# WPCLab/OpenSeg3D

Hardware: AMD Instinct MI355X
Metric: points/sec fwd+bwd, Waymo 1-sweep ~180k pts @0.1m voxel; logit parity (higher is better)
Workload: dtype f32 storage/accumulate, bf16x3 products; 1 GPU; waymo_one_sweep (BASELINE configs[1]): synthetic scene, 174633 pts/step/GPU, voxel [0.1, 0.1, 0.1], grid [1440, 1440, 64], fwd (attention dropout p=0.1, DropPath) + criterion (ohem_ce+lovasz on 3 heads) + bwd + SGD step; mode=fwdbwd, segmentor=segformer, voxels=108690, parallelism=dp1

## Files before the change

### include/seg3d_hip.h

```cpp
#ifndef SEG3D_HIP_H
#define SEG3D_HIP_H

#include <stddef.h>
#include <stdint.h>

#ifdef __cplusplus
extern "C" {
#endif

#define SEG3D_OK 0
#define SEG3D_EINVAL (-1)
#define SEG3D_EWORKSPACE (-2)
#define SEG3D_ELAUNCH (-3)

#define SEG3D_REDUCE_SUM 0
#define SEG3D_REDUCE_MEAN 1
#define SEG3D_REDUCE_MAX 2

int seg3d_abi_version(void);

const char* seg3d_last_error(void);

int seg3d_grid_size(const float* voxel_size, const float* range, int32_t* grid_xyz);

// ... 107 lines not shown
int seg3d_linear_fwd_f32(const float* x, int64_t m, const void* w_packed, const float* bias ,
                         int32_t cin, int32_t cout, float* y, void* stream);
size_t seg3d_linear_packed_bytes_x6(int32_t cin, int32_t cout);
int seg3d_linear_pack_weight_x6(const float* weight, int32_t cin, int32_t cout, int32_t transpose, void* w_packed,
                                void* stream);
int seg3d_linear_fwd_x6(const float* x, int64_t m, const void* w_packed, const float* bias ,
                        const float* scale , const float* shift , int32_t relu, int32_t cin,
                        int32_t cout, float* y, void* stream);

typedef struct {
  const float* src;
  void* dst;
  int32_t cin, cout;
  int32_t kk, transpose, flip, reserved;
  int64_t first_block;
} seg3d_pack_job;
int seg3d_pack_weights_batched(const void* jobs, int32_t n_jobs, int64_t total_blocks, void* stream);

size_t seg3d_linear_packed_bytes(int32_t cin, int32_t cout, int32_t transpose);
int seg3d_linear_pack_weight(const float* weight, int32_t cin, int32_t cout, int32_t transpose,
                             void* w_packed, void* stream);
int seg3d_linear_fwd(const float* x, int64_t m, const void* w_packed, const float* bias ,
                     const float* addend , int32_t cin, int32_t cout,
                     float* y, void* stream);
int seg3d_linear_fwd_sum(const float* x, const float* x_add, int64_t m, const void* w_packed, const float* bias,
                         int32_t cin, int32_t cout, float* y, void* stream);
int seg3d_linear_layernorm_fwd(const float* x, int64_t m, const void* w_packed, const float* bias, const float* res,
                               const float* gamma, const float* beta, float eps, int32_t cin, int32_t cout, float* y,
                               void* stream);
int seg3d_linear_fwd_mul(const float* x, int64_t m, const void* w_packed, const float* factor, int32_t cin, int32_t cout,
                         float* y, void* stream);

size_t seg3d_window_partition_workspace_bytes(int64_t m, int32_t batch_size, const int32_t* nwin_xyz);
int seg3d_window_partition(const int32_t* coords, int64_t m, int32_t batch_size,
                           const int32_t* win_xyz, const int32_t* nwin_xyz, const int32_t* shift_xyz,
                           int32_t n_levels, const int32_t* level_lo, const int32_t* level_hi,
                           const int32_t* level_cap, int32_t* win_id, int32_t* in_win, int32_t* rank,
                           int32_t* level, int32_t* slot, int32_t* tok, int32_t* win_start,
                           int32_t* win_count, int32_t* win_tile0, int32_t* tile_item,
                           int32_t* qg_item, int32_t* counts, void* workspace,
                           size_t workspace_bytes, void* stream);

int seg3d_pos_embed(const int32_t* in_win, int64_t m, const int32_t* win_xyz ,
                    const float* inv_freq, int32_t c, float* pos, void* stream);

int seg3d_window_attn_supported(int32_t heads, int32_t dh);
size_t seg3d_window_attn_workspace_bytes(int64_t m, int32_t n_tiles, int32_t heads, int32_t dh);
int seg3d_window_attn_schedule(int32_t n_tiles, int32_t n_chunks, int32_t heads, int32_t dh, float dropout_p, int32_t* out);
int seg3d_window_attn_fwd(const float* q, const float* k, const float* v, int32_t ldq, int32_t ldk,
                          int32_t ldv, const int32_t* tok, const int32_t* win_start,
                          const int32_t* win_count, const int32_t* win_tile0,
                          const int32_t* tile_item, int32_t n_tiles, const int32_t* qg_item,
                          int32_t n_qgroups, int64_t m, int32_t n_windows, int32_t heads, int32_t dh,
                          const float* tau, float tau_min, float dropout_p, uint64_t dropout_seed, float* out,
                          float* lse, void* workspace, size_t workspace_bytes, void* stream);
int seg3d_window_attn_bwd(const float* q, const float* k, const float* v, int32_t ldq, int32_t ldk,
                          int32_t ldv, const float* out, const float* dout, const float* lse,
                          const int32_t* tok, const int32_t* win_start, const int32_t* win_count,
                          const int32_t* win_tile0, const int32_t* tile_item, int32_t n_tiles,
                          const int32_t* qg_item, int32_t n_qgroups, int64_t m, int32_t n_windows,
                          int32_t heads, int32_t dh, const float* tau,
                          float tau_min, float dropout_p, uint64_t dropout_seed, float* dq, float* dk,
                          float* dv, int32_t lddq, int32_t lddk,
                          int32_t lddv, float* dtau, void* workspace, size_t workspace_bytes,
                          void* stream);

int seg3d_layernorm_fwd(const float* x, const float* res, const float* gamma, const float* beta,
                        const float* rowscale, float eps, int64_t m, int32_t c, float* y, float* mean,
                        float* rstd, void* stream);
size_t seg3d_layernorm_bwd_workspace_bytes(int64_t m, int32_t c);
int seg3d_layernorm_bwd(const float* dy, const float* x, const float* mean, const float* rstd,
                        const float* gamma, const float* rowscale, int64_t m, int32_t c, float* dx,
                        float* dgamma, float* dbeta, void* workspace, size_t workspace_bytes, void* stream);
int seg3d_layernorm_bwd_partials(const float* dy, const float* x, const float* mean, const float* rstd,
                                 const float* gamma, const float* rowscale, int64_t m, int32_t c, float* dx,
                                 void* workspace, size_t workspace_bytes, int32_t* nblocks, void* stream);
size_t seg3d_batchnorm_workspace_bytes(int64_t m, int32_t c);
int seg3d_colstats(const float* x, int64_t m, int32_t c, float* sums, void* workspace, size_t workspace_bytes,
                   void* stream);
int seg3d_batchnorm_stats(const float* x, int64_t m, int32_t c, float eps, const float* gamma, const float* beta,
                          float momentum, float* running_mean, float* running_var, float* stats, void* workspace,
                          size_t workspace_bytes, void* stream);
int seg3d_gelu_fwd(const float* h, int64_t n, float* g, float* gp, void* stream);
int seg3d_affine_act(const float* x, const float* res, const float* scale, const float* shift, int32_t relu,
                     int64_t m, int32_t c, float* y, void* stream);
int seg3d_batchnorm_bwd(const float* dy, const float* y, const float* x, const float* mean, const float* rstd,
                        const float* gamma, int32_t relu, int64_t m, int32_t c, float* dx, float* dres,
                        float* sums, void* workspace, size_t workspace_bytes, void* stream);
int seg3d_batchnorm_bwd_reduce(const float* dy, const float* y, const float* x, const float* mean,
                               const float* rstd, int32_t relu, int64_t m, int32_t c, float* sums,
                               void* workspace, size_t workspace_bytes, void* stream);
int seg3d_batchnorm_bwd_apply(const float* dy, const float* y, const float* x, const float* mean,
                              const float* rstd, const float* gamma, const float* sums, const float* inv_count,
                              int32_t relu, int64_t m, int32_t c, float* dx, float* dres, void* stream);

int seg3d_segment_reduce_fwd(const float* x, int32_t c, const int32_t* order, const int32_t* offsets,
                             int64_t n_seg, int32_t mode, float* out, int32_t* argmax, void* stream);
int seg3d_segment_reduce_bwd(const float* dout, int32_t c, const int32_t* seg_of_row, int64_t n,
                             const int32_t* offsets, const int32_t* argmax, int64_t n_seg,
                             int32_t mode, float* dx, void* stream);

int seg3d_knn_attention_fwd(const float* q, const float* k, const float* v, const int32_t* idx,
                            const uint8_t* invalid, const float* keep, int64_t n, int64_t n_src,
                            int32_t n_neighbors, int32_t d, float scale, float* out, float* prob, void* stream);
int seg3d_knn_attention_bwd(const float* q, const float* k, const float* v, const int32_t* idx, const float* keep,
                            const float* prob, const float* dout, const int32_t* pair_order,
                            const int32_t* pair_offsets, int64_t n, int64_t n_src, int32_t n_neighbors, int32_t d,
                            float scale, float* dq, float* dk, float* dv, float* scratch, void* stream);

int seg3d_class_context_fwd(const float* feats, const float* probs, const int32_t* offsets, const int32_t* chunks,
                            const int32_t* chunk_offsets, int32_t n_chunks, int32_t batch, int64_t m,
                            int32_t classes, int32_t c, float scale, float* weights, float* partials, float* stats,
                            float* context, void* stream);
int seg3d_class_context_bwd(const float* feats, const float* weights, const float* dcontext,
                            const int32_t* offsets, const int32_t* chunks, const int32_t* chunk_offsets,
                            int32_t n_chunks, int32_t batch, int64_t m, int32_t classes, int32_t c, float scale,
                            float* dfeats, float* dprobs, float* scratch, void* stream);

int seg3d_gather_rows(const float* feats, const int32_t* ids, int64_t n, int32_t c, float* out,
                      void* stream);

int seg3d_knn_query(const float* xyz, int64_t n, const float* new_xyz, int64_t m, const int32_t* offset,
                    const int32_t* new_offset, int32_t batch_size, int32_t k, int32_t* idx, float* dist2,
                    void* stream);

size_t seg3d_knn_level_workspace_bytes(int64_t n);
int seg3d_knn_level_build(const float* xyz, int64_t n, const int32_t* offset, int32_t batch_size, float cell,
                          float* sorted_xyz, int32_t* src_index, int32_t* cell_end, void* table_keys, int32_t* table_vals,
                          int64_t capacity, void* workspace, size_t workspace_bytes, void* stream);
int seg3d_knn_query_order(const float* new_xyz, int64_t m, const int32_t* new_offset, int32_t batch_size, float cell,
                          int32_t* order, void* workspace, size_t workspace_bytes, void* stream);
int seg3d_parity_order(const int32_t* coords, int64_t m, int32_t* order, void* workspace, size_t workspace_bytes,
                       void* stream);
typedef struct {
  const float* sorted_xyz;
  const int32_t* src_index;
  const int32_t* cell_end;
  const void* table_keys;
  const int32_t* table_vals;
  int64_t capacity;
  float cell;
  int32_t max_ring;
} seg3d_knn_level;
int seg3d_knn_grid_query(const seg3d_knn_level* levels, int32_t n_levels, const float* new_xyz,
                         const int32_t* query_order , int64_t m,
                         const int32_t* offset, const int32_t* new_offset, int32_t batch_size, int32_t k,
                         int32_t* idx, float* dist2, void* stream);

size_t seg3d_furthest_sampling_workspace_bytes(int64_t n);
int seg3d_furthest_sampling(const float* xyz, int64_t n, const int32_t* order, const int32_t* offset,
                            const int32_t* new_offset, int32_t n_segments, int32_t* idx, void* workspace,
                            size_t workspace_bytes, void* stream);
int seg3d_furthest_sampling_host(const float* xyz, int64_t n, const int32_t* order, const int32_t* offset,
                                 const int32_t* new_offset, int32_t n_segments, int32_t* idx);
int seg3d_sector_angles(const float* xyz, int64_t n, const int32_t* offset, int32_t batch_size, float* angle,
                        float* minmax, void* stream);
int seg3d_sector_angles_host(const float* xyz, int64_t n, const int32_t* offset, int32_t batch_size, float* angle,
                             float* minmax);
int seg3d_sector_assign(const float* angle, int64_t n, const int32_t* offset, int32_t batch_size, const float* edges,
                        const int32_t* sector_offset, int32_t* sector_id, void* stream);
int seg3d_sector_assign_host(const float* angle, int64_t n, const int32_t* offset, int32_t batch_size,
                             const float* edges, const int32_t* sector_offset, int32_t* sector_id);

#define SEG3D_POINTOPS_CHUNK 512
size_t seg3d_pointops_scratch_bytes(int64_t m, int32_t k, int32_t width);
int seg3d_group_points_fwd(const float* xyz, const float* new_xyz, const float* feat, const int32_t* idx, int64_t n,
// ... 218 lines not shown
```

### openseg3d_amd/_lib.py

```python
import ctypes
import os
import re

_HERE = os.path.dirname(os.path.abspath(__file__))
LIB_PATH = os.path.join(_HERE, "csrc", "libseg3d_hip.so")
HEADER_PATH = os.path.join(os.path.dirname(_HERE), "include", "seg3d_hip.h")

OK, EINVAL, EWORKSPACE, ELAUNCH = 0, -1, -2, -3
REDUCE_SUM, REDUCE_MEAN, REDUCE_MAX = 0, 1, 2
ABI_VERSION = 49

_p, _i32, _i64, _sz, _f = ctypes.c_void_p, ctypes.c_int32, ctypes.c_int64, ctypes.c_size_t, ctypes.c_float
_u64 = ctypes.c_uint64
_d = ctypes.c_double

SIGNATURES = {
    "seg3d_abi_version": (ctypes.c_int, []),
    "seg3d_last_error": (ctypes.c_char_p, []),
    "seg3d_grid_size": (ctypes.c_int, [_p, _p, _p]),
    "seg3d_voxelize_workspace_bytes": (_sz, [_i64]),
    "seg3d_voxelize_f32": (ctypes.c_int, [_p, _i64, _i32, _i32, _i32, _p, _p, _p, _p, _p, _p, _sz, _p]),
    "seg3d_voxelize_f64": (ctypes.c_int, [_p, _i64, _i32, _i32, _i32, _p, _p, _p, _p, _p, _p, _sz, _p]),
    "seg3d_voxelize_host_workspace_bytes": (_sz, [_i64]),
    "seg3d_voxelize_host_f32": (ctypes.c_int, [_p, _i64, _i32, _i32, _i32, _p, _p, _p, _p, _p, _p, _sz]),
    "seg3d_voxelize_host_f64": (ctypes.c_int, [_p, _i64, _i32, _i32, _i32, _p, _p, _p, _p, _p, _p, _sz]),
    "seg3d_cart2polar_f32": (ctypes.c_int, [_p, _i64, _i32, _i32, _p, _p]),
    "seg3d_cart2polar_f64": (ctypes.c_int, [_p, _i64, _i32, _i32, _p, _p]),
    "seg3d_group_index_workspace_bytes": (_sz, [_i64, _i64]),
    "seg3d_group_index": (ctypes.c_int, [_p, _i64, _i64, _p, _p, _p, _p, _sz, _p]),
    "seg3d_coord_hash_bytes": (_sz, [_i64]),
    "seg3d_coord_hash_build": (ctypes.c_int, [_p, _i64, _p, _p, _sz, _p]),
    "seg3d_rulebook_subm": (ctypes.c_int, [_p, _i64, _p, _p, _sz, _p, _p]),
    "seg3d_downsample_workspace_bytes": (_sz, [_i32, _p]),
    "seg3d_downsample_coords": (ctypes.c_int, [_p, _i64, _p, _i32, _p, _p, _i64, _p, _p, _sz, _p]),
    "seg3d_rulebook_strided": (ctypes.c_int, [_p, _i64, _i64, _p, _p, _sz, _p, _p, _p]),
    "seg3d_spconv_packed_bytes": (_sz, [_i32, _i32, _i32]),
    "seg3d_spconv_pack_weight": (ctypes.c_int, [_p, _i32, _i32, _i32, _p, _p]),
    "seg3d_spconv_fwd": (ctypes.c_int, [_p, _p, _i64, _i64, _p, _i32, _p, _i32, _i32, _p, _p, _p]),
    "seg3d_spconv_fwd_act": (ctypes.c_int, [_p, _p, _i64, _i64, _p, _i32, _p, _p, _i32, _i32, _i32, _p, _p, _p]),
    "seg3d_spconv_fwd_act_bf16": (ctypes.c_int, [_p, _i32, _p, _i64, _i64, _p, _i32, _p, _p, _i32, _i32, _i32, _p, _p, _p]),
    "seg3d_spconv_presplit_bytes": (_sz, [_i64, _i32]),
    "seg3d_spconv_presplit": (ctypes.c_int, [_p, _i64, _i32, _p, _p]),
    "seg3d_spconv_fwd_presplit": (ctypes.c_int, [_p, _p, _i64, _i64, _p, _i32, _p, _p, _i32, _i32, _i32, _p, _p, _p]),
    "seg3d_conv_plan_bytes": (_sz, [_i64]),
    "seg3d_conv_plan_workspace_bytes": (_sz, [_i64]),
    "seg3d_conv_plan_build": (ctypes.c_int, [_p, _p, _i64, _p, _p, _sz, _p]),
    "seg3d_spconv_tiled_supported": (_i32, [_i32, _i32]),
    "seg3d_spconv_fwd_tiled": (ctypes.c_int, [_p, _p, _p, _i64, _i64, _p, _i32, _p, _p, _i32, _i32, _i32, _p, _p]),
    "seg3d_spconv_fwd_tiled_bf16": (ctypes.c_int, [_p, _i32, _p, _p, _i64, _i64, _p, _i32, _p, _p, _i32, _i32, _i32, _p, _p]),
    "seg3d_debug_set_conv_nbt": (ctypes.c_int, [_i32]),
    "seg3d_debug_set_linear_stream": (ctypes.c_int, [_i32]),
    "seg3d_spconv_wgrad_workspace_bytes": (_sz, [_i64, _i32, _i32]),
    "seg3d_spconv_wgrad": (ctypes.c_int, [_p, _p, _p, _i64, _i64, _i32, _i32, _i32, _p, _p, _sz, _p]),
    "seg3d_spconv_wgrad_partials": (ctypes.c_int, [_p, _p, _p, _i64, _i64, _i32, _i32, _p, _sz, _p, _p]),
    "seg3d_spconv_wgrad_partials_xbf16": (ctypes.c_int, [_p, _p, _p, _i64, _i64, _i32, _i32, _p, _sz, _p, _p]),
    "seg3d_linear_wgrad_partials_xbf16": (ctypes.c_int, [_p, _p, _i64, _i32, _i32, _i32, _p, ctypes.c_size_t, _p, _p]),
    "seg3d_linear_packed_bytes_f32": (ctypes.c_size_t, [_i32, _i32]),
    "seg3d_linear_pack_weight_f32": (ctypes.c_int, [_p, _i32, _i32, _i32, _p, _p]),
    "seg3d_linear_fwd_f32": (ctypes.c_int, [_p, _i64, _p, _p, _i32, _i32, _p, _p]),
    "seg3d_debug_set_wgrad_lds": (ctypes.c_int, [_i32]),
    "seg3d_linear_packed_bytes_x6": (ctypes.c_size_t, [_i32, _i32]),
    "seg3d_linear_pack_weight_x6": (ctypes.c_int, [_p, _i32, _i32, _i32, _p, _p]),
    "seg3d_linear_fwd_x6": (ctypes.c_int, [_p, _i64, _p, _p, _p, _p, _i32, _i32, _i32, _p, _p]),
    "seg3d_pack_weights_batched": (ctypes.c_int, [_p, _i32, _i64, _p]),
    "seg3d_linear_wgrad_workspace_bytes": (ctypes.c_size_t, [_i64, _i32, _i32]),
    "seg3d_linear_wgrad": (ctypes.c_int, [_p, _p, _i64, _i32, _i32, _p, _p, _p, ctypes.c_size_t, _p]),
    "seg3d_linear_wgrad_partials": (ctypes.c_int, [_p, _p, _i64, _i32, _i32, _i32, _p, ctypes.c_size_t, _p, _p]),
    "seg3d_reduce_partials": (ctypes.c_int, [_p, _i32, _i64, _i64, _p, _p, _p]),
    "seg3d_reduce_partials_batched": (ctypes.c_int, [_p, _i32, _i64, _p]),
    "seg3d_linear_packed_bytes": (_sz, [_i32, _i32, _i32]),
    "seg3d_linear_pack_weight": (ctypes.c_int, [_p, _i32, _i32, _i32, _p, _p]),
    "seg3d_linear_fwd": (ctypes.c_int, [_p, _i64, _p, _p, _p, _i32, _i32, _p, _p]),
    "seg3d_linear_fwd_sum": (ctypes.c_int, [_p, _p, _i64, _p, _p, _i32, _i32, _p, _p]),
    "seg3d_linear_fwd_mul": (ctypes.c_int, [_p, _i64, _p, _p, _i32, _i32, _p, _p]),
    "seg3d_linear_layernorm_fwd": (ctypes.c_int, [_p, _i64, _p, _p, _p, _p, _p, ctypes.c_float, _i32, _i32, _p, _p]),
    "seg3d_window_partition_workspace_bytes": (_sz, [_i64, _i32, _p]),
    "seg3d_window_partition": (ctypes.c_int, [_p, _i64, _i32, _p, _p, _p, _i32, _p, _p, _p,
                                              _p, _p, _p, _p, _p, _p, _p, _p, _p, _p, _p, _p, _p, _sz, _p]),
    "seg3d_pos_embed": (ctypes.c_int, [_p, _i64, _p, _p, _i32, _p, _p]),
    "seg3d_window_attn_supported": (ctypes.c_int, [_i32, _i32]),
    "seg3d_window_attn_workspace_bytes": (_sz, [_i64, _i32, _i32, _i32]),
    "seg3d_window_attn_schedule": (ctypes.c_int, [_i32, _i32, _i32, _i32, _f, _p]),
    "seg3d_window_attn_fwd": (ctypes.c_int, [_p, _p, _p, _i32, _i32, _i32, _p, _p, _p, _p, _p, _i32, _p, _i32,
                                             _i64, _i32, _i32, _i32, _p, _f, _f, _u64, _p, _p, _p, _sz, _p]),
    "seg3d_window_attn_bwd": (ctypes.c_int, [_p, _p, _p, _i32, _i32, _i32, _p, _p, _p, _p, _p, _p, _p, _p, _i32, _p,
                                             _i32, _i64, _i32, _i32, _i32, _p, _f, _f, _u64, _p, _p, _p, _i32, _i32, _i32,
                                             _p, _p, _sz, _p]),
    "seg3d_layernorm_fwd": (ctypes.c_int, [_p, _p, _p, _p, _p, _f, _i64, _i32, _p, _p, _p, _p]),
    "seg3d_layernorm_bwd_workspace_bytes": (ctypes.c_size_t, [_i64, _i32]),
    "seg3d_layernorm_bwd": (ctypes.c_int, [_p, _p, _p, _p, _p, _p, _i64, _i32, _p, _p, _p, _p, ctypes.c_size_t, _p]),
    "seg3d_layernorm_bwd_partials": (ctypes.c_int, [_p, _p, _p, _p, _p, _p, _i64, _i32, _p, _p, ctypes.c_size_t, _p, _p]),
    "seg3d_batchnorm_workspace_bytes": (ctypes.c_size_t, [_i64, _i32]),
    "seg3d_colstats": (ctypes.c_int, [_p, _i64, _i32, _p, _p, ctypes.c_size_t, _p]),
    "seg3d_batchnorm_stats": (ctypes.c_int, [_p, _i64, _i32, _f, _p, _p, _f, _p, _p, _p, _p, ctypes.c_size_t, _p]),
    "seg3d_affine_act": (ctypes.c_int, [_p, _p, _p, _p, _i32, _i64, _i32, _p, _p]),
    "seg3d_gelu_fwd": (ctypes.c_int, [_p, _i64, _p, _p, _p]),
    "seg3d_batchnorm_bwd": (ctypes.c_int, [_p, _p, _p, _p, _p, _p, _i32, _i64, _i32, _p, _p, _p, _p, ctypes.c_size_t, _p]),
    "seg3d_batchnorm_bwd_reduce": (ctypes.c_int, [_p, _p, _p, _p, _p, _i32, _i64, _i32, _p, _p, ctypes.c_size_t, _p]),
    "seg3d_batchnorm_bwd_apply": (ctypes.c_int, [_p, _p, _p, _p, _p, _p, _p, _p, _i32, _i64, _i32, _p, _p, _p]),
    "seg3d_segment_reduce_fwd": (ctypes.c_int, [_p, _i32, _p, _p, _i64, _i32, _p, _p, _p]),
    "seg3d_segment_reduce_bwd": (ctypes.c_int, [_p, _i32, _p, _i64, _p, _p, _i64, _i32, _p, _p]),
    "seg3d_voxel_majority_labels": (ctypes.c_int, [_p, _p, _p, _i64, _i32, _p, _p]),
    "seg3d_cross_entropy_workspace_bytes": (ctypes.c_size_t, [_i64]),
    "seg3d_cross_entropy_fwd": (ctypes.c_int, [_p, _p, _i64, _i32, _i64, _f, _p, _p, _p, ctypes.c_size_t, _p]),
    "seg3d_cross_entropy_bwd": (ctypes.c_int, [_p, _p, _p, _p, _p, _i64, _i32, _p, _p]),
    "seg3d_lovasz_workspace_bytes": (ctypes.c_size_t, [_i64, _i32]),
    "seg3d_lovasz_softmax_fwd": (ctypes.c_int, [_p, _p, _i64, _i32, _i64, _i32, _p, _p, _p, _p, _p, ctypes.c_size_t, _p]),
    "seg3d_lovasz_softmax_bwd": (ctypes.c_int, [_p, _p, _p, _p, _i64, _i32, _p, _p]),
    "seg3d_pointwise_loss_workspace_bytes": (ctypes.c_size_t, [_i64]),
    "seg3d_focal_loss_fwd": (ctypes.c_int, [_p, _p, _i64, _i32, _i64, _f, _f, _p, _i32, _p, _p, ctypes.c_size_t, _p]),
    "seg3d_focal_loss_bwd": (ctypes.c_int, [_p, _p, _p, _p, _i64, _i32, _i64, _f, _f, _p, _i32, _p, _p]),
    "seg3d_dice_loss_fwd": (ctypes.c_int, [_p, _p, _i64, _i32, _i64, _f, _f, _p, _f, _f, _p, _p, ctypes.c_size_t, _p]),
    "seg3d_dice_loss_bwd": (ctypes.c_int, [_p, _p, _p, _i64, _i32, _i64, _f, _f, _p, _f, _f, _p, _p]),
    "seg3d_knn_level_workspace_bytes": (ctypes.c_size_t, [_i64]),
    "seg3d_knn_level_build": (ctypes.c_int, [_p, _i64, _p, _i32, _f, _p, _p, _p, _p, _p, _i64, _p, ctypes.c_size_t, _p]),
    "seg3d_parity_order": (ctypes.c_int, [_p, _i64, _p, _p, ctypes.c_size_t, _p]),
    "seg3d_knn_query_order": (ctypes.c_int, [_p, _i64, _p, _i32, _f, _p, _p, ctypes.c_size_t, _p]),
    "seg3d_knn_grid_query": (ctypes.c_int, [_p, _i32, _p, _p, _i64, _p, _p, _i32, _i32, _p, _p, _p]),
    "seg3d_knn_query": (ctypes.c_int, [_p, _i64, _p, _i64, _p, _p, _i32, _i32, _p, _p, _p]),
    "seg3d_furthest_sampling_workspace_bytes": (_sz, [_i64]),
    "seg3d_furthest_sampling": (ctypes.c_int, [_p, _i64, _p, _p, _p, _i32, _p, _p, _sz, _p]),
    "seg3d_furthest_sampling_host": (ctypes.c_int, [_p, _i64, _p, _p, _p, _i32, _p]),
    "seg3d_sector_angles": (ctypes.c_int, [_p, _i64, _p, _i32, _p, _p, _p]),
    "seg3d_sector_angles_host": (ctypes.c_int, [_p, _i64, _p, _i32, _p, _p]),
    "seg3d_sector_assign": (ctypes.c_int, [_p, _i64, _p, _i32, _p, _p, _p, _p]),
    "seg3d_sector_assign_host": (ctypes.c_int, [_p, _i64, _p, _i32, _p, _p, _p]),
    "seg3d_pointops_scratch_bytes": (_sz, [_i64, _i32, _i32]),
    "seg3d_group_points_fwd": (ctypes.c_int, [_p, _p, _p, _p, _i64, _i64, _i32, _i32, _p, _p]),
    "seg3d_group_points_fwd_host": (ctypes.c_int, [_p, _p, _p, _p, _i64, _i64, _i32, _i32, _p]),
    "seg3d_group_points_bwd": (ctypes.c_int, [_p, _p, _p, _p, _i64, _i64, _i32, _i32, _i32, _p, _p, _p, _p, _sz, _p]),
    "seg3d_group_points_bwd_host": (ctypes.c_int, [_p, _p, _p, _p, _i64, _i64, _i32, _i32, _i32, _p, _p, _p]),
    "seg3d_knn_interpolate_fwd": (ctypes.c_int, [_p, _p, _p, _i64, _i64, _i32, _i32, _p, _p, _p]),
    "seg3d_knn_interpolate_fwd_host": (ctypes.c_int, [_p, _p, _p, _i64, _i64, _i32, _i32, _p, _p]),
    "seg3d_knn_interpolate_bwd": (ctypes.c_int, [_p, _p, _p, _p, _p, _i64, _i64, _i32, _i32, _p, _p, _sz, _p]),
    "seg3d_knn_interpolate_bwd_host": (ctypes.c_int, [_p, _p, _p, _p, _p, _i64, _i64, _i32, _i32, _p]),
    "seg3d_gather_rows": (ctypes.c_int, [_p, _p, _i64, _i32, _p, _p]),
    "seg3d_class_context_fwd": (ctypes.c_int, [_p, _p, _p, _p, _p, _i32, _i32, _i64, _i32, _i32, _f, _p, _p, _p, _p, _p]),
    "seg3d_class_context_bwd": (ctypes.c_int, [_p, _p, _p, _p, _p, _p, _i32, _i32, _i64, _i32, _i32, _f, _p, _p, _p, _p]),
    "seg3d_knn_attention_fwd": (ctypes.c_int, [_p, _p, _p, _p, _p, _p, _i64, _i64, _i32, _i32, _f, _p, _p, _p]),
    "seg3d_knn_attention_bwd": (ctypes.c_int, [_p, _p, _p, _p, _p, _p, _p, _p, _p, _i64, _i64, _i32, _i32, _f, _p, _p, _p, _p, _p]),
    "seg3d_tta_views_f32": (ctypes.c_int, [_p, _i64, _i32, _p, _p, _p]),
    "seg3d_tta_views_host_f32": (ctypes.c_int, [_p, _i64, _i32, _p, _p]),
    "seg3d_softmax_accumulate_f32": (ctypes.c_int, [_p, _i64, _i32, _i32, _i32, _p, _p]),
    "seg3d_argmax_confusion": (ctypes.c_int, [_p, _p, _i64, _i32, _i32, _p, _i32, _p, _p, _p]),
    "seg3d_aug_polarmix_workspace_bytes": (_sz, [_i64, _i64]),
    "seg3d_aug_polarmix_map": (ctypes.c_int, [_p, _i64, _p, _i64, _i32, _i32, _p, _i32, _i32, _d, _d, _p, _i32, _i32, _i64,
                                              _p, _p, _p, _p, _sz, _p]),
    "seg3d_aug_polarmix_map_host": (ctypes.c_int, [_p, _i64, _p, _i64, _i32, _i32, _p, _i32, _i32, _d, _d, _p, _i32, _i32,
                                                   _i64, _p, _p, _p]),
    "seg3d_aug_far_near_workspace_bytes": (_sz, [_i64]),
    "seg3d_aug_far_near": (ctypes.c_int, [_p, _i64, _p, _i64, _i32, _i32, _p, _p, _i64, _p, _i64, _p, _f, _p, _p, _p, _p,
                                          _p, _sz, _p]),
    "seg3d_aug_far_near_host": (ctypes.c_int, [_p, _i64, _p, _i64, _i32, _i32, _p, _p, _i64, _p, _i64, _p, _f, _p, _p, _p,
                                               _p]),
    "seg3d_aug_sample_workspace_bytes": (_sz, [_i64]),
    "seg3d_aug_sample_device": (ctypes.c_int, [_p, _i64, _i64, _u64, _p, _p, _sz, _p]),
    "seg3d_aug_sample_host": (ctypes.c_int, [_p, _i64, _i64, _u64, _p]),
    "seg3d_aug_cur_map_workspace_bytes": (_sz, [_i64, _i64]),
    "seg3d_aug_cur_map": (ctypes.c_int, [_p, _i64, _p, _i64, _i64, _p, _p, _p, _p, _sz, _p]),
    "seg3d_aug_cur_map_host": (ctypes.c_int, [_p, _i64, _p, _i64, _i64, _p, _p, _p]),
    "seg3d_aug_apply_f32": (ctypes.c_int, [_p, _i64, _p, _i64, _i32, _p, _p, _i64, _p, _p, _p]),
    "seg3d_aug_apply_f64in": (ctypes.c_int, [_p, _i64, _p, _i64, _i32, _p, _p, _i64, _p, _p, _p]),
    "seg3d_aug_apply_host_f32": (ctypes.c_int, [_p, _i64, _p, _i64, _i32, _p, _p, _i64, _p, _p]),
    "seg3d_aug_apply_host_f64in": (ctypes.c_int, [_p, _i64, _p, _i64, _i32, _p, _p, _i64, _p, _p]),
    "seg3d_aug_gather": (ctypes.c_int, [_p, _i64, _p, _i64, _i64, _p, _i64, _p, _p]),
    "seg3d_aug_gather_host": (ctypes.c_int, [_p, _i64, _p, _i64, _i64, _p, _i64, _p]),
    "seg3d_aug_instance_workspace_bytes": (_sz, [_i64, _i64, _i32]),
    "seg3d_aug_instance_paste": (ctypes.c_int, [_p, _i64, _i32, _i32, _p, _i32, _p, _i32, _p, _i64, _p, _i32, _i64, _p, _p,
                                                _p, _p, _p, _sz, _p]),
    "seg3d_aug_instance_paste_host": (ctypes.c_int, [_p, _i64, _i32, _i32, _p, _i32, _p, _i32, _p, _i64, _p, _i32, _i64, _p,
                                                     _p, _p, _p]),
    "seg3d_instance_extract_workspace_bytes": (_sz, [_i64, _i32]),
    "seg3d_instance_extract": (ctypes.c_int, [_p, _i64, _i32, _i32, _p, _i32, _p, _p, _i32, _p, _i32, _d, _i32, _p, _p, _p, _p,
                                              _p, _sz, _p]),
    "seg3d_instance_extract_host": (ctypes.c_int, [_p, _i64, _i32, _i32, _p, _i32, _p, _p, _i32, _p, _i32, _d, _i32, _p, _p, _p,
                                                   _p]),
    "seg3d_frame_assemble": (ctypes.c_int, [_p, _i32, _i32, _p, _p, _p, _f, _p]),
    "seg3d_frame_assemble_host": (ctypes.c_int, [_p, _i32, _i32, _p, _p, _p, _f]),
    "seg3d_range_image_workspace_bytes": (_sz, [_i32, _i32]),
# ... 55 lines not shown
```

### openseg3d_amd/csrc/rownorm.hip

```cpp
#include "common.hpp"

namespace {

constexpr int kThreads = 256;
constexpr int kMaxBlocks = 2048;
constexpr int kLnBwdMaxBlocks = 1024;

struct RowMap {
    int quads;
    int p;
    int items;
};

inline RowMap row_map(int c) {
    RowMap m;
    m.quads = c / 4;
    m.items = (m.quads + 63) / 64;
    int need = (m.quads + m.items - 1) / m.items;
    m.p = 8;
    while (m.p < need) m.p <<= 1;
    return m;
}

__device__ __forceinline__ float group_sum(float v, int p) {
    for (int off = 1; off < p; off <<= 1) v += __shfl_xor(v, off, SEG3D_WAVE);
    return v;
}

template <int ITEMS>
__global__ __launch_bounds__(kThreads) void ln_fwd_kernel(const float* __restrict__ x, const float* __restrict__ res,
                                                          const float* __restrict__ gamma, const float* __restrict__ beta,
                                                          const float* __restrict__ rowscale, float eps, int64_t m, int c,
                                                          RowMap rm, float* __restrict__ y, float* __restrict__ mean,
                                                          float* __restrict__ rstd) {
    const int lane = threadIdx.x & 63, wave = threadIdx.x >> 6;
    const int rows_per_wave = 64 / rm.p;
    const int lr = lane / rm.p, lq = lane % rm.p;
    const float inv_c = 1.0f / (float)c;
    for (int64_t base = ((int64_t)blockIdx.x * 4 + wave) * rows_per_wave; base < m;
         base += (int64_t)gridDim.x * 4 * rows_per_wave) {
        const int64_t row = base + lr;
        const bool rok = row < m;
        float4 v[ITEMS];
        float s = 0.f;
#pragma unroll
        for (int i = 0; i < ITEMS; ++i) {
            const int q = lq + i * rm.p;
            v[i] = make_float4(0.f, 0.f, 0.f, 0.f);
            if (rok && q < rm.quads) v[i] = *reinterpret_cast<const float4*>(x + row * c + 4 * q);
            s += (v[i].x + v[i].y) + (v[i].z + v[i].w);
        }
        const float mu = group_sum(s, rm.p) * inv_c;
        float ss = 0.f;
#pragma unroll
        for (int i = 0; i < ITEMS; ++i) {
            const int q = lq + i * rm.p;
            if (q < rm.quads) {
                const float a = v[i].x - mu, b = v[i].y - mu, cc = v[i].z - mu, d = v[i].w - mu;
                ss += (a * a + b * b) + (cc * cc + d * d);
            }
        }
        const float rs = rsqrtf(group_sum(ss, rm.p) * inv_c + eps);
        const float sc = rowscale && rok ? rowscale[row] : 1.0f;
#pragma unroll
        for (int i = 0; i < ITEMS; ++i) {
            const int q = lq + i * rm.p;
            if (rok && q < rm.quads) {
                const float4 g = *reinterpret_cast<const float4*>(gamma + 4 * q);
                const float4 b = *reinterpret_cast<const float4*>(beta + 4 * q);
                float4 o;
                o.x = ((v[i].x - mu) * rs * g.x + b.x) * sc;
                o.y = ((v[i].y - mu) * rs * g.y + b.y) * sc;
                o.z = ((v[i].z - mu) * rs * g.z + b.z) * sc;
                o.w = ((v[i].w - mu) * rs * g.w + b.w) * sc;
                if (res) {
                    const float4 r4 = *reinterpret_cast<const float4*>(res + row * c + 4 * q);
                    o.x += r4.x; o.y += r4.y; o.z += r4.z; o.w += r4.w;
                }
                *reinterpret_cast<float4*>(y + row * c + 4 * q) = o;
            }
        }
        if (rok && lq == 0 && mean) {
            mean[row] = mu;
            rstd[row] = rs;
        }
    }
}

template <int ITEMS>
__global__ __launch_bounds__(kThreads) void ln_bwd_kernel(const float* __restrict__ dy, const float* __restrict__ x,
                                                          const float* __restrict__ mean, const float* __restrict__ rstd,
                                                          const float* __restrict__ gamma, const float* __restrict__ rowscale,
                                                          int64_t m, int c, RowMap rm, float* __restrict__ dx,
                                                          float* __restrict__ part ) {
    extern __shared__ float red[];
    const int lane = threadIdx.x & 63, wave = threadIdx.x >> 6;
    const int rows_per_wave = 64 / rm.p;
    const int lr = lane / rm.p, lq = lane % rm.p;
    const float inv_c = 1.0f / (float)c;
    float4 ag[ITEMS], ab[ITEMS];
#pragma unroll
    for (int i = 0; i < ITEMS; ++i) ag[i] = ab[i] = make_float4(0.f, 0.f, 0.f, 0.f);

    for (int64_t base = ((int64_t)blockIdx.x * 4 + wave) * rows_per_wave; base < m;
         base += (int64_t)gridDim.x * 4 * rows_per_wave) {
        const int64_t row = base + lr;
        const bool rok = row < m;
        const float mu = rok ? mean[row] : 0.f, rs = rok ? rstd[row] : 0.f;
        const float sc = rowscale && rok ? rowscale[row] : 1.0f;
        float4 xh[ITEMS], gy[ITEMS];
        float s1 = 0.f, s2 = 0.f;
#pragma unroll
        for (int i = 0; i < ITEMS; ++i) {
            const int q = lq + i * rm.p;
            xh[i] = gy[i] = make_float4(0.f, 0.f, 0.f, 0.f);
            if (rok && q < rm.quads) {
                const float4 xv = *reinterpret_cast<const float4*>(x + row * c + 4 * q);
                float4 dv = *reinterpret_cast<const float4*>(dy + row * c + 4 * q);
                dv.x *= sc; dv.y *= sc; dv.z *= sc; dv.w *= sc;
                const float4 g = *reinterpret_cast<const float4*>(gamma + 4 * q);
                xh[i] = make_float4((xv.x - mu) * rs, (xv.y - mu) * rs, (xv.z - mu) * rs, (xv.w - mu) * rs);
                gy[i] = make_float4(dv.x * g.x, dv.y * g.y, dv.z * g.z, dv.w * g.w);
                ag[i].x += dv.x * xh[i].x; ag[i].y += dv.y * xh[i].y; ag[i].z += dv.z * xh[i].z; ag[i].w += dv.w * xh[i].w;
                ab[i].x += dv.x; ab[i].y += dv.y; ab[i].z += dv.z; ab[i].w += dv.w;
                s1 += (gy[i].x + gy[i].y) + (gy[i].z + gy[i].w);
                s2 += (gy[i].x * xh[i].x + gy[i].y * xh[i].y) + (gy[i].z * xh[i].z + gy[i].w * xh[i].w);
            }
        }
        const float c1 = group_sum(s1, rm.p) * inv_c, c2 = group_sum(s2, rm.p) * inv_c;
#pragma unroll
        for (int i = 0; i < ITEMS; ++i) {
            const int q = lq + i * rm.p;
            if (rok && q < rm.quads) {
                float4 o;
                o.x = rs * (gy[i].x - c1 - xh[i].x * c2);
                o.y = rs * (gy[i].y - c1 - xh[i].y * c2);
                o.z = rs * (gy[i].z - c1 - xh[i].z * c2);
                o.w = rs * (gy[i].w - c1 - xh[i].w * c2);
                *reinterpret_cast<float4*>(dx + row * c + 4 * q) = o;
            }
        }
    }
    const int slots = 4 * rows_per_wave;
    float* mine = red + (size_t)(wave * rows_per_wave + lr) * 2 * c;
#pragma unroll
    for (int i = 0; i < ITEMS; ++i) {
        const int q = lq + i * rm.p;
        if (q < rm.quads) {
            *reinterpret_cast<float4*>(mine + 4 * q) = ag[i];
            *reinterpret_cast<float4*>(mine + c + 4 * q) = ab[i];
        }
    }
    __syncthreads();
    for (int i = threadIdx.x; i < 2 * c; i += kThreads) {
        float t = red[i];
        for (int l = 1; l < slots; ++l) t += red[(size_t)l * 2 * c + i];
        part[(int64_t)blockIdx.x * 2 * c + i] = t;
    }
}

__global__ __launch_bounds__(1024) void ln_bwd_reduce(const float* __restrict__ part, int nblocks, int c,
                                                      float* __restrict__ dgamma, float* __restrict__ dbeta) {
    __shared__ float red[32][33];
    const int col = threadIdx.x & 31, q = threadIdx.x >> 5;
    const int i = blockIdx.x * 32 + col;
    float s = 0.f;
    if (i < 2 * c) {
        float s0 = 0.f, s1 = 0.f, s2 = 0.f, s3 = 0.f;
        int b = q;
        for (; b + 96 < nblocks; b += 128) {
            s0 += part[(int64_t)b * 2 * c + i];
            s1 += part[(int64_t)(b + 32) * 2 * c + i];
            s2 += part[(int64_t)(b + 64) * 2 * c + i];
            s3 += part[(int64_t)(b + 96) * 2 * c + i];
        }
        for (; b < nblocks; b += 32) s0 += part[(int64_t)b * 2 * c + i];
        s = (s0 + s1) + (s2 + s3);
    }
    red[q][col] = s;
    __syncthreads();
    if (q == 0 && i < 2 * c) {
        float t = red[0][col];
#pragma unroll
        for (int k = 1; k < 32; ++k) t += red[k][col];
        if (i < c) dgamma[i] = t;
        else dbeta[i - c] = t;
    }
}

template <int MODE>
__global__ __launch_bounds__(kThreads) void col_reduce_kernel(const float* __restrict__ x, const float* __restrict__ dy,
                                                              const float* __restrict__ y, const float* __restrict__ mean,
                                                              const float* __restrict__ rstd, int relu, int64_t m, int c,
                                                              float* __restrict__ part ) {
    extern __shared__ float red[];
    const int quads = c / 4;
    const int lanes = kThreads / quads;
    const int q = threadIdx.x % quads, rl = threadIdx.x / quads;
    if (rl < lanes) {
        float4 a = make_float4(0.f, 0.f, 0.f, 0.f), b = a;
        float4 p0 = a, p1 = a;
        if (MODE == 0) p0 = *reinterpret_cast<const float4*>(x + 4 * q);
        if (MODE == 1) {
            p0 = *reinterpret_cast<const float4*>(mean + 4 * q);
            p1 = *reinterpret_cast<const float4*>(rstd + 4 * q);
        }
        for (int64_t row = (int64_t)blockIdx.x * lanes + rl; row < m; row += (int64_t)gridDim.x * lanes) {
            const float4 xv = *reinterpret_cast<const float4*>(x + row * c + 4 * q);
            if (MODE == 0) {
                const float dx_ = xv.x - p0.x, dy_ = xv.y - p0.y, dz_ = xv.z - p0.z, dw_ = xv.w - p0.w;
                a.x += dx_; a.y += dy_; a.z += dz_; a.w += dw_;
                b.x += dx_ * dx_; b.y += dy_ * dy_; b.z += dz_ * dz_; b.w += dw_ * dw_;
            } else {
                float4 g = *reinterpret_cast<const float4*>(dy + row * c + 4 * q);
                if (relu) {
                    const float4 yv = *reinterpret_cast<const float4*>(y + row * c + 4 * q);
                    g.x = yv.x > 0.f ? g.x : 0.f; g.y = yv.y > 0.f ? g.y : 0.f;
                    g.z = yv.z > 0.f ? g.z : 0.f; g.w = yv.w > 0.f ? g.w : 0.f;
                }
                a.x += g.x; a.y += g.y; a.z += g.z; a.w += g.w;
                b.x += g.x * (xv.x - p0.x) * p1.x; b.y += g.y * (xv.y - p0.y) * p1.y;
                b.z += g.z * (xv.z - p0.z) * p1.z; b.w += g.w * (xv.w - p0.w) * p1.w;
            }
        }
        *reinterpret_cast<float4*>(red + (size_t)rl * 2 * c + 4 * q) = a;
        *reinterpret_cast<float4*>(red + (size_t)rl * 2 * c + c + 4 * q) = b;
    }
    __syncthreads();
    for (int i = threadIdx.x; i < 2 * c; i += kThreads) {
        float t = red[i];
        for (int l = 1; l < lanes; ++l) t += red[(size_t)l * 2 * c + i];
        part[(size_t)blockIdx.x * 2 * c + i] = t;
    }
}

__device__ __forceinline__ float col_partial_sum(const float* __restrict__ part, int nblocks, int c2, int i, float (*red)[33]) {
    const int col = threadIdx.x & 31, q = threadIdx.x >> 5;
    float s = 0.f;
    if (i < c2) {
        float s0 = 0.f, s1 = 0.f, s2 = 0.f, s3 = 0.f;
        int b = q;
        for (; b + 96 < nblocks; b += 128) {
            s0 += part[(int64_t)b * c2 + i];
            s1 += part[(int64_t)(b + 32) * c2 + i];
            s2 += part[(int64_t)(b + 64) * c2 + i];
            s3 += part[(int64_t)(b + 96) * c2 + i];
        }
        for (; b < nblocks; b += 32) s0 += part[(int64_t)b * c2 + i];
        s = (s0 + s1) + (s2 + s3);
    }
    red[q][col] = s;
    __syncthreads();
    float t = red[0][col];
#pragma unroll
    for (int k = 1; k < 32; ++k) t += red[k][col];
    __syncthreads();
    return t;
}

__global__ __launch_bounds__(1024) void col_sums_finish(const float* __restrict__ part, int nblocks, int c,
                                                        float* __restrict__ sums ) {
    __shared__ float red[32][33];
    const int i = blockIdx.x * 32 + (threadIdx.x & 31);
    const float t = col_partial_sum(part, nblocks, 2 * c, i, red);
    if ((threadIdx.x >> 5) == 0 && i < 2 * c) sums[i] = t;
}

__global__ __launch_bounds__(kThreads) void gelu_fwd_kernel(const float* __restrict__ h, int64_t quads, float* __restrict__ g,
                                                            float* __restrict__ gp) {
    for (int64_t t = (int64_t)blockIdx.x * kThreads + threadIdx.x; t < quads; t += (int64_t)gridDim.x * kThreads) {
        const float4 v = reinterpret_cast<const float4*>(h)[t];
        const float in[4] = {v.x, v.y, v.z, v.w};
        float o[4], d[4];
#pragma unroll
        for (int i = 0; i < 4; ++i) {
            const float cdf = 0.5f * (1.0f + erff(in[i] * 0.70710678118654752440f));
            o[i] = in[i] * cdf;
            d[i] = cdf + in[i] * (0.39894228040143267794f * __expf(-0.5f * in[i] * in[i]));
        }
        reinterpret_cast<float4*>(g)[t] = make_float4(o[0], o[1], o[2], o[3]);
        if (gp) reinterpret_cast<float4*>(gp)[t] = make_float4(d[0], d[1], d[2], d[3]);
    }
}

__global__ __launch_bounds__(kThreads) void affine_act_kernel(const float* __restrict__ x, const float* __restrict__ res,
                                                              const float* __restrict__ scale, const float* __restrict__ shift,
                                                              int relu, int64_t total_quads, int quads, float* __restrict__ y) {
    for (int64_t t = (int64_t)blockIdx.x * kThreads + threadIdx.x; t < total_quads; t += (int64_t)gridDim.x * kThreads) {
        const int q = (int)(t % quads);
        const float4 xv = reinterpret_cast<const float4*>(x)[t];
        const float4 s = *reinterpret_cast<const float4*>(scale + 4 * q);
        const float4 b = *reinterpret_cast<const float4*>(shift + 4 * q);
        float4 o = make_float4(xv.x * s.x + b.x, xv.y * s.y + b.y, xv.z * s.z + b.z, xv.w * s.w + b.w);
        if (res) {
            const float4 r = reinterpret_cast<const float4*>(res)[t];
            o.x += r.x; o.y += r.y; o.z += r.z; o.w += r.w;
        }
        if (relu) {
            o.x = fmaxf(o.x, 0.f); o.y = fmaxf(o.y, 0.f); o.z = fmaxf(o.z, 0.f); o.w = fmaxf(o.w, 0.f);
        }
        reinterpret_cast<float4*>(y)[t] = o;
    }
}

__global__ __launch_bounds__(kThreads) void bn_bwd_apply_kernel(const float* __restrict__ dy, const float* __restrict__ y,
                                                                const float* __restrict__ x, const float* __restrict__ mean,
                                                                const float* __restrict__ rstd, const float* __restrict__ gamma,
                                                                const float* __restrict__ sums , int relu,
                                                                float inv_m, const float* __restrict__ inv_m_dev,
                                                                int64_t total_quads, int quads,
                                                                float* __restrict__ dx, float* __restrict__ dres) {
    const int c = quads * 4;
    if (inv_m_dev) inv_m = inv_m_dev[0];
    for (int64_t t = (int64_t)blockIdx.x * kThreads + threadIdx.x; t < total_quads; t += (int64_t)gridDim.x * kThreads) {
        const int q = (int)(t % quads);
        float4 g = reinterpret_cast<const float4*>(dy)[t];
        if (relu) {
            const float4 yv = reinterpret_cast<const float4*>(y)[t];
            g.x = yv.x > 0.f ? g.x : 0.f; g.y = yv.y > 0.f ? g.y : 0.f;
            g.z = yv.z > 0.f ? g.z : 0.f; g.w = yv.w > 0.f ? g.w : 0.f;
        }
        if (dres) reinterpret_cast<float4*>(dres)[t] = g;
        const float4 xv = reinterpret_cast<const float4*>(x)[t];
        const float4 mu = *reinterpret_cast<const float4*>(mean + 4 * q);
        const float4 rs = *reinterpret_cast<const float4*>(rstd + 4 * q);
        const float4 ga = *reinterpret_cast<const float4*>(gamma + 4 * q);
        const float4 s1 = *reinterpret_cast<const float4*>(sums + 4 * q);
        const float4 s2 = *reinterpret_cast<const float4*>(sums + c + 4 * q);
        float4 o;
        o.x = ga.x * rs.x * (g.x - s1.x * inv_m - (xv.x - mu.x) * rs.x * s2.x * inv_m);
        o.y = ga.y * rs.y * (g.y - s1.y * inv_m - (xv.y - mu.y) * rs.y * s2.y * inv_m);
        o.z = ga.z * rs.z * (g.z - s1.z * inv_m - (xv.z - mu.z) * rs.z * s2.z * inv_m);
        o.w = ga.w * rs.w * (g.w - s1.w * inv_m - (xv.w - mu.w) * rs.w * s2.w * inv_m);
        reinterpret_cast<float4*>(dx)[t] = o;
    }
}

__global__ __launch_bounds__(1024) void bn_finalize_kernel(const float* __restrict__ x, const float* __restrict__ part,
                                                           int nblocks, int64_t m, int c, float eps,
                                                           const float* __restrict__ gamma, const float* __restrict__ beta,
                                                           float momentum, float* __restrict__ running_mean,
                                                           float* __restrict__ running_var, float* __restrict__ stats) {
    __shared__ float red[32][33];
    const int i = blockIdx.x * 32 + (threadIdx.x & 31);
    const float s1 = col_partial_sum(part, nblocks, 2 * c, i < c ? i : 2 * c, red);
    const float s2 = col_partial_sum(part, nblocks, 2 * c, i < c ? c + i : 2 * c, red);
    if ((threadIdx.x >> 5) != 0 || i >= c) return;
    stats[i] = s1;
    stats[c + i] = s2;
    const float inv_m = 1.0f / (float)m;
    const float d = s1 * inv_m;
    const float mean = x[i] + d;
    const float var = fmaxf(s2 * inv_m - d * d, 0.0f);
    const float rstd = 1.0f / sqrtf(var + eps);
    const float scale = gamma[i] * rstd;
    stats[2 * c + i] = mean;
    stats[3 * c + i] = rstd;
    stats[4 * c + i] = scale;
    stats[5 * c + i] = beta[i] - mean * scale;
    if (running_mean) {
        running_mean[i] = running_mean[i] * (1.0f - momentum) + mean * momentum;
        const float unbiased = m > 1 ? var * ((float)m / (float)(m - 1)) : var;
        running_var[i] = running_var[i] * (1.0f - momentum) + unbiased * momentum;
    }
}

constexpr int kColMaxBlocks = 1024;
constexpr size_t kColSmem = 8192;

inline unsigned blocks_for(int64_t work_items, int per_block) {
    int64_t b = ceil_div64(work_items, per_block);
    if (b > kMaxBlocks) b = kMaxBlocks;
    if (b < 1) b = 1;
    return (unsigned)b;
}

inline bool bad_c(int c) { return c <= 0 || (c & 3) || c > 1024; }

}

extern "C" {

int seg3d_layernorm_fwd(const float* x, const float* res, const float* gamma, const float* beta, const float* rowscale,
                        float eps, int64_t m, int32_t c, float* y, float* mean, float* rstd, void* stream) {
    if (m < 0 || bad_c(c) || c > 512) return SEG3D_EINVAL;
    if (m == 0) return SEG3D_OK;
    if (!x || !gamma || !beta || !y) return SEG3D_EINVAL;
    const RowMap rm = row_map(c);
    const unsigned nb = blocks_for(m, 4 * (64 / rm.p));
    if (rm.items == 1)
        hipLaunchKernelGGL(ln_fwd_kernel<1>, dim3(nb), dim3(kThreads), 0, as_stream(stream), x, res, gamma, beta, rowscale,
                           eps, m, c, rm, y, mean, rstd);
    else
        hipLaunchKernelGGL(ln_fwd_kernel<2>, dim3(nb), dim3(kThreads), 0, as_stream(stream), x, res, gamma, beta, rowscale,
                           eps, m, c, rm, y, mean, rstd);
    SEG3D_CHECK_LAUNCH();
    return SEG3D_OK;
}

size_t seg3d_layernorm_bwd_workspace_bytes(int64_t m, int32_t c) {
    if (m < 0 || bad_c(c)) return 0;
    return (size_t)kLnBwdMaxBlocks * 2 * c * sizeof(float);
}

int seg3d_layernorm_bwd_partials(const float* dy, const float* x, const float* mean, const float* rstd, const float* gamma,
                                 const float* rowscale, int64_t m, int32_t c, float* dx, void* workspace,
                                 size_t workspace_bytes, int32_t* nblocks, void* stream) {
    if (m < 0 || bad_c(c) || c > 512 || !nblocks) return SEG3D_EINVAL;
    if (workspace_bytes < seg3d_layernorm_bwd_workspace_bytes(m, c) || !workspace) return SEG3D_EWORKSPACE;
    *nblocks = 0;
    if (m == 0) return SEG3D_OK;
    if (!dy || !x || !mean || !rstd || !gamma || !dx) return SEG3D_EINVAL;
    hipStream_t st = as_stream(stream);
    float* part = static_cast<float*>(workspace);
    const RowMap rm = row_map(c);
    unsigned nb = blocks_for(m, 4 * (64 / rm.p) * 4);
    if (nb > (unsigned)kLnBwdMaxBlocks) nb = kLnBwdMaxBlocks;
    const size_t smem = (size_t)4 * (64 / rm.p) * 2 * c * sizeof(float);
    if (rm.items == 1)
        hipLaunchKernelGGL(ln_bwd_kernel<1>, dim3(nb), dim3(kThreads), smem, st, dy, x, mean, rstd, gamma, rowscale, m, c, rm,
                           dx, part);
    else
        hipLaunchKernelGGL(ln_bwd_kernel<2>, dim3(nb), dim3(kThreads), smem, st, dy, x, mean, rstd, gamma, rowscale, m, c, rm,
                           dx, part);
    SEG3D_CHECK_LAUNCH();
    *nblocks = (int32_t)nb;
    return SEG3D_OK;
}

int seg3d_layernorm_bwd(const float* dy, const float* x, const float* mean, const float* rstd, const float* gamma,
                        const float* rowscale, int64_t m, int32_t c, float* dx, float* dgamma, float* dbeta,
                        void* workspace, size_t workspace_bytes, void* stream) {
    if (m < 0 || bad_c(c) || c > 512 || !dgamma || !dbeta) return SEG3D_EINVAL;
    if (workspace_bytes < seg3d_layernorm_bwd_workspace_bytes(m, c) || !workspace) return SEG3D_EWORKSPACE;
    hipStream_t st = as_stream(stream);
    float* part = static_cast<float*>(workspace);
    unsigned nb = 0;
    if (m > 0) {
        if (!dy || !x || !mean || !rstd || !gamma || !dx) return SEG3D_EINVAL;
        const RowMap rm = row_map(c);
        nb = blocks_for(m, 4 * (64 / rm.p) * 4);
        if (nb > (unsigned)kLnBwdMaxBlocks) nb = kLnBwdMaxBlocks;
        const size_t smem = (size_t)4 * (64 / rm.p) * 2 * c * sizeof(float);
        if (rm.items == 1)
            hipLaunchKernelGGL(ln_bwd_kernel<1>, dim3(nb), dim3(kThreads), smem, st, dy, x, mean, rstd, gamma, rowscale, m, c,
                               rm, dx, part);
        else
            hipLaunchKernelGGL(ln_bwd_kernel<2>, dim3(nb), dim3(kThreads), smem, st, dy, x, mean, rstd, gamma, rowscale, m, c,
                               rm, dx, part);
        SEG3D_CHECK_LAUNCH();
    }
    hipLaunchKernelGGL(ln_bwd_reduce, dim3((unsigned)((2 * c + 31) / 32)), dim3(1024), 0, st, part, (int)nb, c, dgamma,
                       dbeta);
    SEG3D_CHECK_LAUNCH();
    return SEG3D_OK;
}

size_t seg3d_batchnorm_workspace_bytes(int64_t m, int32_t c) {
    if (m < 0 || bad_c(c)) return 0;
    return (size_t)kColMaxBlocks * 2 * c * sizeof(float);
}

static unsigned col_blocks(int64_t m, int c) {
    const int lanes = kThreads / (c / 4);
    unsigned nb = blocks_for(m, lanes * 16);
    return nb > (unsigned)kColMaxBlocks ? (unsigned)kColMaxBlocks : nb;
}

int seg3d_colstats(const float* x, int64_t m, int32_t c, float* sums ,
                   void* workspace, size_t workspace_bytes, void* stream) {
    if (m <= 0 || bad_c(c) || !sums || !x) return SEG3D_EINVAL;
    if (!workspace || workspace_bytes < seg3d_batchnorm_workspace_bytes(m, c)) return SEG3D_EWORKSPACE;
    hipStream_t st = as_stream(stream);
    float* part = static_cast<float*>(workspace);
    const unsigned nb = col_blocks(m, c);
    hipLaunchKernelGGL(col_reduce_kernel<0>, dim3(nb), dim3(kThreads), kColSmem, st, x, nullptr, nullptr, nullptr, nullptr, 0, m,
                       c, part);
    SEG3D_CHECK_LAUNCH();
    hipLaunchKernelGGL(col_sums_finish, dim3((unsigned)((2 * c + 31) / 32)), dim3(1024), 0, st, part, (int)nb, c, sums);
    SEG3D_CHECK_LAUNCH();
    return SEG3D_OK;
}

int seg3d_batchnorm_stats(const float* x, int64_t m, int32_t c, float eps, const float* gamma, const float* beta,
                          float momentum, float* running_mean, float* running_var, float* stats ,
                          void* workspace, size_t workspace_bytes, void* stream) {
    if (m <= 0 || bad_c(c) || !x || !gamma || !beta || !stats || (running_mean && !running_var)) return SEG3D_EINVAL;
    if (!workspace || workspace_bytes < seg3d_batchnorm_workspace_bytes(m, c)) return SEG3D_EWORKSPACE;
    hipStream_t st = as_stream(stream);
    float* part = static_cast<float*>(workspace);
    const unsigned nb = col_blocks(m, c);
    hipLaunchKernelGGL(col_reduce_kernel<0>, dim3(nb), dim3(kThreads), kColSmem, st, x, nullptr, nullptr, nullptr, nullptr, 0, m,
                       c, part);
    SEG3D_CHECK_LAUNCH();
    hipLaunchKernelGGL(bn_finalize_kernel, dim3((unsigned)((c + 31) / 32)), dim3(1024), 0, st, x, part, (int)nb, m, c, eps, gamma,
                       beta, momentum, running_mean, running_var, stats);
    SEG3D_CHECK_LAUNCH();
    return SEG3D_OK;
}

int seg3d_gelu_fwd(const float* h, int64_t n, float* g, float* gp, void* stream) {
    if (n < 0 || (n & 3)) return SEG3D_EINVAL;
    if (n == 0) return SEG3D_OK;
    if (!h || !g) return SEG3D_EINVAL;
    hipLaunchKernelGGL(gelu_fwd_kernel, dim3(blocks_for(n / 4, kThreads * 4)), dim3(kThreads), 0, as_stream(stream), h, n / 4, g,
                       gp);
    SEG3D_CHECK_LAUNCH();
    return SEG3D_OK;
}

int seg3d_affine_act(const float* x, const float* res, const float* scale, const float* shift, int32_t relu, int64_t m,
                     int32_t c, float* y, void* stream) {
    if (m < 0 || bad_c(c)) return SEG3D_EINVAL;
    if (m == 0) return SEG3D_OK;
    if (!x || !scale || !shift || !y) return SEG3D_EINVAL;
    const int64_t tq = m * (c / 4);
    hipLaunchKernelGGL(affine_act_kernel, dim3(blocks_for(tq, kThreads * 4)), dim3(kThreads), 0, as_stream(stream), x, res,
                       scale, shift, relu, tq, c / 4, y);
    SEG3D_CHECK_LAUNCH();
    return SEG3D_OK;
}

int seg3d_batchnorm_bwd(const float* dy, const float* y, const float* x, const float* mean, const float* rstd,
                        const float* gamma, int32_t relu, int64_t m, int32_t c, float* dx, float* dres,
                        float* sums , void* workspace, size_t workspace_bytes, void* stream) {
    if (m <= 0 || bad_c(c) || !sums) return SEG3D_EINVAL;
    if (!workspace || workspace_bytes < seg3d_batchnorm_workspace_bytes(m, c)) return SEG3D_EWORKSPACE;
    if (!dy || !x || !mean || !rstd || !gamma || !dx || (relu && !y)) return SEG3D_EINVAL;
    hipStream_t st = as_stream(stream);
    float* part = static_cast<float*>(workspace);
    const unsigned nb = col_blocks(m, c);
    hipLaunchKernelGGL(col_reduce_kernel<1>, dim3(nb), dim3(kThreads), kColSmem, st, x, dy, y, mean, rstd, relu, m, c, part);
    SEG3D_CHECK_LAUNCH();
    hipLaunchKernelGGL(col_sums_finish, dim3((unsigned)((2 * c + 31) / 32)), dim3(1024), 0, st, part, (int)nb, c, sums);
    SEG3D_CHECK_LAUNCH();
    const int64_t tq = m * (c / 4);
    hipLaunchKernelGGL(bn_bwd_apply_kernel, dim3(blocks_for(tq, kThreads * 4)), dim3(kThreads), 0, st, dy, y, x, mean, rstd,
                       gamma, sums, relu, 1.0f / (float)m, nullptr, tq, c / 4, dx, dres);
    SEG3D_CHECK_LAUNCH();
    return SEG3D_OK;
}

int seg3d_batchnorm_bwd_reduce(const float* dy, const float* y, const float* x, const float* mean, const float* rstd,
                               int32_t relu, int64_t m, int32_t c, float* sums, void* workspace, size_t workspace_bytes,
                               void* stream) {
    if (m <= 0 || bad_c(c) || !sums) return SEG3D_EINVAL;
    if (!workspace || workspace_bytes < seg3d_batchnorm_workspace_bytes(m, c)) return SEG3D_EWORKSPACE;
    if (!dy || !x || !mean || !rstd || (relu && !y)) return SEG3D_EINVAL;
    hipStream_t st = as_stream(stream);
    float* part = static_cast<float*>(workspace);
    const unsigned nb = col_blocks(m, c);
    hipLaunchKernelGGL(col_reduce_kernel<1>, dim3(nb), dim3(kThreads), kColSmem, st, x, dy, y, mean, rstd, relu, m, c, part);
    SEG3D_CHECK_LAUNCH();
    hipLaunchKernelGGL(col_sums_finish, dim3((unsigned)((2 * c + 31) / 32)), dim3(1024), 0, st, part, (int)nb, c, sums);
    SEG3D_CHECK_LAUNCH();
    return SEG3D_OK;
}

int seg3d_batchnorm_bwd_apply(const float* dy, const float* y, const float* x, const float* mean, const float* rstd,
                              const float* gamma, const float* sums, const float* inv_count, int32_t relu, int64_t m,
                              int32_t c, float* dx, float* dres, void* stream) {
    if (m <= 0 || bad_c(c) || !sums || !inv_count) return SEG3D_EINVAL;
    if (!dy || !x || !mean || !rstd || !gamma || !dx || (relu && !y)) return SEG3D_EINVAL;
    const int64_t tq = m * (c / 4);
    hipLaunchKernelGGL(bn_bwd_apply_kernel, dim3(blocks_for(tq, kThreads * 4)), dim3(kThreads), 0, as_stream(stream), dy, y, x,
                       mean, rstd, gamma, sums, relu, 0.0f, inv_count, tq, c / 4, dx, dres);
    SEG3D_CHECK_LAUNCH();
    return SEG3D_OK;
}

}
```

### openseg3d_amd/csrc/scan.hip

```cpp
#include "common.hpp"

namespace {

constexpr int kThreads = 256;
constexpr int kItems = 8;
constexpr int kChunk = kThreads * kItems;

__device__ __forceinline__ uint32_t add(uint32_t a, uint32_t b) { return a + b; }
__device__ __forceinline__ uint4 add(uint4 a, uint4 b) {
    return make_uint4(a.x + b.x, a.y + b.y, a.z + b.z, a.w + b.w);
}
__device__ __forceinline__ uint32_t zero_of(uint32_t) { return 0u; }
__device__ __forceinline__ uint4 zero_of(uint4) { return make_uint4(0, 0, 0, 0); }

__device__ __forceinline__ uint32_t shfl_up_t(uint32_t v, int d) { return __shfl_up(v, d, SEG3D_WAVE); }
__device__ __forceinline__ uint4 shfl_up_t(uint4 v, int d) {
    return make_uint4(__shfl_up(v.x, d, SEG3D_WAVE), __shfl_up(v.y, d, SEG3D_WAVE),
                      __shfl_up(v.z, d, SEG3D_WAVE), __shfl_up(v.w, d, SEG3D_WAVE));
}

template <typename T>
__device__ T block_inclusive(T v, T* lds , T* total) {
    const int lane = threadIdx.x & 63, wave = threadIdx.x >> 6;
    for (int d = 1; d < 64; d <<= 1) {
        T o = shfl_up_t(v, d);
        if (lane >= d) v = add(v, o);
    }
    if (lane == 63) lds[wave] = v;
    __syncthreads();
    T base = zero_of(v), tot = zero_of(v);
    for (int w = 0; w < kThreads / 64; ++w) {
        if (w < wave) base = add(base, lds[w]);
        tot = add(tot, lds[w]);
    }
    __syncthreads();
    *total = tot;
    return add(v, base);
}

template <typename T>
__global__ __launch_bounds__(kThreads) void chunk_totals(const T* __restrict__ in, int64_t n, T* __restrict__ sums) {
    __shared__ T lds[4];
    const int64_t base = (int64_t)blockIdx.x * kChunk + (int64_t)threadIdx.x * kItems;
    T acc = zero_of(T());
#pragma unroll
    for (int i = 0; i < kItems; ++i)
        if (base + i < n) acc = add(acc, in[base + i]);
    T tot;
    block_inclusive(acc, lds, &tot);
    if (threadIdx.x == 0) sums[blockIdx.x] = tot;
}

template <typename T>
__global__ __launch_bounds__(kThreads) void chunk_scan(const T* __restrict__ in, T* __restrict__ out, int64_t n,
                                                       const T* __restrict__ sums, T* __restrict__ total) {
    __shared__ T lds[4];
    T part = zero_of(T());
    for (int j = threadIdx.x; j < (int)blockIdx.x; j += kThreads) part = add(part, sums[j]);
    T chunk_base;
    block_inclusive(part, lds, &chunk_base);

    const int64_t base = (int64_t)blockIdx.x * kChunk + (int64_t)threadIdx.x * kItems;
    T v[kItems];
    T acc = zero_of(T());
#pragma unroll
    for (int i = 0; i < kItems; ++i) {
        v[i] = (base + i < n) ? in[base + i] : zero_of(T());
        acc = add(acc, v[i]);
    }
    T tot;
    T incl = block_inclusive(acc, lds, &tot);
    T run;
    if constexpr (sizeof(T) == 4) {
        run = add(chunk_base, incl - acc);
    } else {
        run = add(chunk_base, make_uint4(incl.x - acc.x, incl.y - acc.y, incl.z - acc.z, incl.w - acc.w));
    }
#pragma unroll
    for (int i = 0; i < kItems; ++i) {
        if (base + i < n) out[base + i] = run;
        run = add(run, v[i]);
    }
    if (total != nullptr && blockIdx.x == gridDim.x - 1 && threadIdx.x == 0) *total = add(chunk_base, tot);
}

template <typename T>
int scan_impl(const T* in, T* out, int64_t n, T* total, T* tmp, hipStream_t st) {
    if (n < 0) return SEG3D_EINVAL;
    const int64_t nb = ceil_div64(n > 0 ? n : 1, kChunk);
    if (nb > 1) {
        hipLaunchKernelGGL(chunk_totals<T>, dim3((unsigned)nb), dim3(kThreads), 0, st, in, n, tmp);
        SEG3D_CHECK_LAUNCH();
    }
    hipLaunchKernelGGL(chunk_scan<T>, dim3((unsigned)nb), dim3(kThreads), 0, st, in, out, n, tmp, total);
    SEG3D_CHECK_LAUNCH();
    return SEG3D_OK;
}

}

int scan_exclusive_u32(const uint32_t* in, uint32_t* out, int64_t n, uint32_t* total, uint32_t* tmp,
                       hipStream_t st) {
    return scan_impl<uint32_t>(in, out, n, total, tmp, st);
}

int scan_exclusive_u32x4(const uint4* in, uint4* out, int64_t n, uint4* total, uint4* tmp, hipStream_t st) {
    return scan_impl<uint4>(in, out, n, total, tmp, st);
}
```

### openseg3d_amd/csrc/spconv_split.hip

```cpp
#include <atomic>
#include <cstdlib>
#include <type_traits>

#include "common.hpp"

#ifdef SEG3D_CONV_STAMP
__device__ unsigned long long* g_stamp_buf = nullptr;
extern "C" int seg3d_debug_conv_stamps(void* buf) {
    unsigned long long* p = static_cast<unsigned long long*>(buf);
    return hipMemcpyToSymbol(HIP_SYMBOL(g_stamp_buf), &p, sizeof(p)) == hipSuccess ? 0 : 2;
}
#define STAMP(i)                                                     \
    do {                                                             \
        __builtin_amdgcn_sched_barrier(0);                           \
        const unsigned long long t_ = __builtin_amdgcn_s_memtime();  \
        __builtin_amdgcn_sched_barrier(0);                           \
        st_acc[i] += t_ - st_last;                                   \
        st_last = t_;                                                \
    } while (0)
#else
#define STAMP(i) do {} while (0)
#endif

namespace {
// ... 7 lines not shown
__device__ __forceinline__ uint32_t pack_bf16(float a, float b) {
    f32x2 v = {a, b};
    return __builtin_bit_cast(uint32_t, __builtin_convertvector(v, bf16x2));
}

__device__ __forceinline__ void split8(const f32x4& p, const f32x4& q, bf16x8* hi, bf16x8* lo) {
    u32x4 h, l;
    const float v[8] = {p[0], p[1], p[2], p[3], q[0], q[1], q[2], q[3]};
#pragma unroll
    for (int i = 0; i < 4; ++i) {
        const uint32_t ph = pack_bf16(v[2 * i], v[2 * i + 1]);
        const float h0 = __builtin_bit_cast(float, ph << 16);
        const float h1 = __builtin_bit_cast(float, ph & 0xFFFF0000u);
        h[i] = ph;
        l[i] = pack_bf16(v[2 * i] - h0, v[2 * i + 1] - h1);
    }
    *hi = __builtin_bit_cast(bf16x8, h);
    *lo = __builtin_bit_cast(bf16x8, l);
}

__device__ __forceinline__ void pack_item(const float* __restrict__ w, int cin_src, int cout_src, int kk, int transpose,
                                          int flip, int64_t item, __bf16* __restrict__ wp) {
    const int cin_op = transpose ? cout_src : cin_src;
    const int cout_op = transpose ? cin_src : cout_src;
    const int cb_n = (cin_op + 31) / 32, nb_n = cout_op / 16;
    int64_t r = item;
    const int lane = (int)(r & 63); r >>= 6;
    const int nb = (int)(r % nb_n); r /= nb_n;
    const int cb = (int)(r % cb_n); r /= cb_n;
    const int kp = (int)r;
    const int k = flip ? kk - 1 - kp : kp;
    const int ci0 = cb * 32 + (lane >> 4) * 8;
    const int co_op = nb * 16 + (lane & 15);
    float v[8];
#pragma unroll
    for (int j = 0; j < 8; ++j) {
        const int ci_op = ci0 + j;
        const int ci = transpose ? co_op : ci_op;
        const int co = transpose ? ci_op : co_op;
        v[j] = ci_op < cin_op ? w[((int64_t)co * kk + k) * cin_src + ci] : 0.f;
    }
    bf16x8 hi, lo;
    split8((f32x4){v[0], v[1], v[2], v[3]}, (f32x4){v[4], v[5], v[6], v[7]}, &hi, &lo);
    const int64_t base = ((item >> 6) * 2) * 512 + (int64_t)lane * 8;
    *reinterpret_cast<bf16x8*>(wp + base) = hi;
    *reinterpret_cast<bf16x8*>(wp + base + 512) = lo;
}

__global__ __launch_bounds__(256) void pack_weight_split(const float* __restrict__ w, int cin_src, int cout_src, int kk,
                                                         int transpose, int flip, int64_t items, __bf16* __restrict__ wp) {
    const int64_t t = (int64_t)blockIdx.x * 256 + threadIdx.x;
    if (t < items) pack_item(w, cin_src, cout_src, kk, transpose, flip, t, wp);
}

struct PackJob {
    const float* src;
    __bf16* dst;
    int32_t cin_src, cout_src, kk, transpose, flip, reserved;
    int64_t first_block;
};
static_assert(sizeof(PackJob) == 48, "PackJob layout is part of the C ABI (seg3d_pack_weights_batched)");

__global__ __launch_bounds__(256) void pack_weights_batched(const PackJob* __restrict__ jobs, int n_jobs) {
    int lo = 0, hi = n_jobs - 1;
    while (lo < hi) {
        const int mid = (lo + hi + 1) >> 1;
        if (jobs[mid].first_block <= (int64_t)blockIdx.x) lo = mid;
        else hi = mid - 1;
    }
    const PackJob jb = jobs[lo];
    const int cin_op = jb.transpose ? jb.cout_src : jb.cin_src;
    const int cout_op = jb.transpose ? jb.cin_src : jb.cout_src;
    const int64_t items = (int64_t)jb.kk * ((cin_op + 31) / 32) * (cout_op / 16) * 64;
    const int64_t t = ((int64_t)blockIdx.x - jb.first_block) * 256 + threadIdx.x;
    if (t < items) pack_item(jb.src, jb.cin_src, jb.cout_src, jb.kk, jb.transpose, jb.flip, t, jb.dst);
}

struct LnEpilogue {
    const float* gamma;
    const float* beta;
    float eps;
};

template <int NBT, int RB, bool DENSE, int IO = 0, int DEPTH = 1>
__global__ __launch_bounds__(256, 2) void spconv_split_kernel(const void* __restrict__ x_v, const int32_t* __restrict__ nbr,
                                                              int64_t m_out, const uint4* __restrict__ wp,
                                                              const float* __restrict__ bias,
                                                              const void* __restrict__ addend_v,
                                                              const int32_t* __restrict__ row_order, int cin, int cout,
                                                              void* __restrict__ y_v, int relu_flags,
                                                              const float* __restrict__ x_add, LnEpilogue ln) {
    const int relu = relu_flags & 1;
    const float* __restrict__ x = static_cast<const float*>(x_v);
    const float* __restrict__ addend = static_cast<const float*>(addend_v);
    float* __restrict__ y = static_cast<float*>(y_v);
    constexpr int kW = 4;
    constexpr int kSlot = NBT * 128;
    constexpr int kPieces = NBT * 2;
    __shared__ __attribute__((aligned(16))) uint4 wlds[2 * kSlot];
    __shared__ uint32_t wave_mask[kW];
    constexpr int kRowsW = RB * 16;
    __shared__ int32_t idx_lds[DENSE ? 1 : kW * 27 * kRowsW];

    const int tid = threadIdx.x, lane = tid & 63, wave = tid >> 6;
    const int g = lane >> 4, c16 = lane & 15;
#ifdef SEG3D_CONV_STAMP
    unsigned long long st_acc[8] = {0, 0, 0, 0, 0, 0, 0, 0};
    unsigned long long st_last = __builtin_amdgcn_s_memtime();
    const unsigned long long st_begin = st_last;
#endif
    int64_t tile_id = blockIdx.x;
    int col_group = blockIdx.y;
    if (relu_flags & 4) {
        const int ny = (cout >> 4) / NBT;
        const int64_t n_tiles = (m_out + kW * RB * 16 - 1) / (kW * RB * 16);
        const int64_t id = blockIdx.x;
        const int64_t grp = id / (8 * ny);
        const int t = (int)(id - grp * 8 * ny);
        tile_id = grp * 8 + (t & 7);
        col_group = t >> 3;
        if (tile_id >= n_tiles) return;
    }
    if (relu_flags & 2) {
        const int64_t n_tiles = (m_out + kW * RB * 16 - 1) / (kW * RB * 16);
        const int64_t per = (n_tiles + 7) >> 3;
        tile_id = (int64_t)(blockIdx.x & 7) * per + (blockIdx.x >> 3);
        if (tile_id >= n_tiles) return;
    }
    const int64_t row0 = tile_id * (kW * RB * 16) + wave * (RB * 16);
    const int nb0 = col_group * NBT;
    const int cb_n = (cin + 31) >> 5, nb_n = cout >> 4;
    const int64_t last_row = m_out - 1;

    uint32_t my_mask = 0;
    {
        const int64_t pos = row0 + (lane & (kRowsW - 1));
        const bool ok = pos < m_out;
        const int64_t rc = ok ? (row_order ? (int64_t)row_order[pos] : pos) : last_row;
        if (DENSE) {
            my_mask = 1u;
        } else {
            int32_t v[27];
#pragma unroll
            for (int k = 0; k < 27; ++k) v[k] = nbr[(int64_t)k * m_out + rc];
#pragma unroll
            for (int k = 0; k < 27; ++k) {
                v[k] = ok ? v[k] : -1;
                if (__ballot(v[k] >= 0) != 0ull) my_mask |= 1u << k;
                if (lane < kRowsW) idx_lds[(wave * 27 + k) * kRowsW + lane] = v[k];
            }
        }
    }
    if (lane == 0) wave_mask[wave] = my_mask;
    __syncthreads();
    const uint32_t todo_all = wave_mask[0] | wave_mask[1] | wave_mask[2] | wave_mask[3];

    f32x4 acc[RB][NBT];
#pragma unroll
    for (int n = 0; n < NBT; ++n) {
        const float b = bias ? bias[(nb0 + n) * 16 + c16] : 0.0f;
#pragma unroll
        for (int rb = 0; rb < RB; ++rb) acc[rb][n] = (f32x4){b, b, b, b};
    }

    if (todo_all != 0u) {
        int64_t grow[RB];
        bool grow_ok[RB];
#pragma unroll
        for (int rb = 0; rb < RB; ++rb) {
            const int64_t pos = row0 + rb * 16 + c16;
            grow_ok[rb] = pos < m_out;
            grow[rb] = grow_ok[rb] ? pos : last_row;
        }
        auto fetch_idx = [&](int k, int32_t* idx) {
#pragma unroll
            for (int rb = 0; rb < RB; ++rb)
                idx[rb] = DENSE ? (grow_ok[rb] ? (int32_t)grow[rb] : -1) : idx_lds[(wave * 27 + k) * kRowsW + rb * 16 + c16];
        };
        constexpr int kMine = (kPieces + kW - 1) / kW;
        u32x4 wreg[DEPTH][kMine];
        auto stage_w = [&](auto S, int k, int cb) {
            const uint4* src = wp + (((int64_t)k * cb_n + cb) * nb_n + nb0) * 128;
#pragma unroll
            for (int j = 0; j < kMine; ++j) {
                const int piece = j * kW + wave;
                wreg[S][j] = *reinterpret_cast<const u32x4*>(src + (kPieces % kW == 0 || piece < kPieces ? piece : 0) * 64 + lane);
            }
        };
        auto commit_w = [&](auto S, int buf) {
#pragma unroll
            for (int j = 0; j < kMine; ++j) {
                const int piece = j * kW + wave;
                if (kPieces % kW == 0 || piece < kPieces)
                    *reinterpret_cast<u32x4*>(wlds + buf * kSlot + piece * 64 + lane) = wreg[S][j];
            }
        };
        f32x4 areg[DEPTH][RB][2];
        constexpr bool XADD = DENSE && IO == 3;
        f32x4 areg2[XADD ? RB : 1][2];
        bool aval[DEPTH][RB];
        auto issue_a = [&](auto S, const int32_t* idx, int cb, bool on) {
            const bool in_range = cb * 32 + g * 8 < cin;
            const int col = in_range ? cb * 32 + g * 8 : 0;
#pragma unroll
            for (int rb = 0; rb < RB; ++rb) {
                aval[S][rb] = on && in_range && idx[rb] >= 0;
                const int64_t src_row = idx[rb] >= 0 ? idx[rb] : 0;
                if constexpr (IO == 2) {
                    areg[S][rb][0] = *reinterpret_cast<const f32x4*>(static_cast<const __bf16*>(x_v) + src_row * cin + col);
                } else {
                    const f32x4* p = reinterpret_cast<const f32x4*>(x + src_row * cin + col);
                    areg[S][rb][0] = p[0];
                    areg[S][rb][1] = p[1];
                    if constexpr (XADD) {
                        const f32x4* p2 = reinterpret_cast<const f32x4*>(x_add + src_row * cin + col);
                        areg2[rb][0] = p2[0];
                        areg2[rb][1] = p2[1];
                    }
                }
            }
        };
        bf16x8 a_hi[RB], a_lo[RB];
        auto land_a = [&](auto S) {
#pragma unroll
            for (int rb = 0; rb < RB; ++rb) {
                const f32x4 z = (f32x4){0.f, 0.f, 0.f, 0.f};
                if constexpr (IO == 2) {
                    a_hi[rb] = __builtin_bit_cast(bf16x8, aval[S][rb] ? areg[S][rb][0] : z);
                } else {
                    f32x4 r0 = areg[S][rb][0], r1 = areg[S][rb][1];
                    if constexpr (XADD) {
                        r0 = r0 + areg2[rb][0];
                        r1 = r1 + areg2[rb][1];
                    }
                    split8(aval[S][rb] ? r0 : z, aval[S][rb] ? r1 : z, &a_hi[rb], &a_lo[rb]);
                }
            }
        };

        using S0 = std::integral_constant<int, 0>;
        using S1 = std::integral_constant<int, DEPTH - 1>;
        struct Chunk {
            int k, cb;
            bool on, have;
        };
        uint32_t it_todo = todo_all;
        int it_cb = 0;
        auto next_chunk = [&]() {
            Chunk c;
            c.have = true;
            if (it_todo == 0u) {
                it_cb += 1;
                it_todo = todo_all;
                c.have = it_cb < cb_n;
// ... 57 lines not shown
                STAMP(5);
                buf ^= 1;
                cur = nxt;
            }
        } else {
            Chunk n1 = next_chunk();
            if (n1.have) issue(S1{}, n1);
            for (;;) {
                Chunk n2 = n1;
                if (n1.have) {
                    n2 = next_chunk();
                    if (n2.have) issue(S0{}, n2);
                }
                multiply(cur.on, buf);
                if (!n1.have) break;
                land_a(S1{});
                commit_w(S1{}, buf ^ 1);
                __syncthreads();
                buf ^= 1;
                Chunk n3 = n2;
                if (n2.have) {
                    n3 = next_chunk();
                    if (n3.have) issue(S1{}, n3);
                }
                multiply(n1.on, buf);
                if (!n2.have) break;
                land_a(S0{});
                commit_w(S0{}, buf ^ 1);
                __syncthreads();
                buf ^= 1;
                cur = n2;
                n1 = n3;
            }
        }
    }

    if constexpr (IO == 5) {
        float gm[NBT], bt[NBT];
#pragma unroll
        for (int n = 0; n < NBT; ++n) {
            gm[n] = ln.gamma[n * 16 + c16];
            bt[n] = ln.beta[n * 16 + c16];
        }
        const float inv_c = 1.0f / (float)cout;
#pragma unroll
        for (int rb = 0; rb < RB; ++rb)
#pragma unroll
            for (int r = 0; r < 4; ++r) {
                float sum = 0.f;
#pragma unroll
                for (int n = 0; n < NBT; ++n) sum += acc[rb][n][r];
#pragma unroll
                for (int d = 1; d < 16; d <<= 1) sum += __shfl_xor(sum, d, 64);
                const float mu = sum * inv_c;
                float ss = 0.f;
#pragma unroll
                for (int n = 0; n < NBT; ++n) {
                    const float dlt = acc[rb][n][r] - mu;
                    ss = fmaf(dlt, dlt, ss);
                }
#pragma unroll
                for (int d = 1; d < 16; d <<= 1) ss += __shfl_xor(ss, d, 64);
                const float rs = rsqrtf(ss * inv_c + ln.eps);
                const int64_t opos = row0 + rb * 16 + g * 4 + r;
                if (opos < m_out) {
                    float* yr = y + opos * cout + c16;
                    const float* rr = addend ? addend + opos * cout + c16 : nullptr;
#pragma unroll
                    for (int n = 0; n < NBT; ++n) {
                        float o = (acc[rb][n][r] - mu) * rs * gm[n] + bt[n];
                        if (rr) o += rr[n * 16];
                        yr[n * 16] = o;
                    }
                }
            }
        return;
    }

#pragma unroll
    for (int rb = 0; rb < RB; ++rb)
#pragma unroll
        for (int r = 0; r < 4; ++r) {
            const int64_t opos = row0 + rb * 16 + g * 4 + r;
            if (opos < m_out) {
                const int64_t orow = row_order ? (int64_t)row_order[opos] : opos;
                if constexpr (IO == 1 || IO == 2) {
                    __bf16* yb = static_cast<__bf16*>(y_v) + orow * cout + nb0 * 16 + c16;
                    const __bf16* ab = addend_v ? static_cast<const __bf16*>(addend_v) + orow * cout + nb0 * 16 + c16 : nullptr;
#pragma unroll
                    for (int n = 0; n < NBT; ++n) {
                        const float v = acc[rb][n][r] + (ab ? (float)ab[n * 16] : 0.0f);
                        yb[n * 16] = (__bf16)(relu ? (v < 0.0f ? 0.0f : v) : v);
                    }
                    continue;
                }
                float* yr = y + orow * cout + nb0 * 16 + c16;
                if (addend) {
                    const float* ar = addend + orow * cout + nb0 * 16 + c16;
#pragma unroll
                    for (int n = 0; n < NBT; ++n) {
                        const float v = IO == 4 ? acc[rb][n][r] * ar[n * 16] : acc[rb][n][r] + ar[n * 16];
                        yr[n * 16] = relu ? (v < 0.0f ? 0.0f : v) : v;
                    }
                } else {
#pragma unroll
                    for (int n = 0; n < NBT; ++n) {
                        const float v = acc[rb][n][r];
                        yr[n * 16] = relu ? (v < 0.0f ? 0.0f : v) : v;
                    }
                }
            }
        }
#ifdef SEG3D_CONV_STAMP
    asm volatile("s_waitcnt vmcnt(0)" ::: "memory");
    if (g_stamp_buf && lane == 0) {
        unsigned long long* o = g_stamp_buf + (((size_t)blockIdx.y * gridDim.x + blockIdx.x) * 4 + wave) * 8;
        st_acc[6] = __builtin_amdgcn_s_memtime() - st_begin;
        for (int i = 0; i < 8; ++i) o[i] = st_acc[i];
    }
#endif
}

constexpr int kDeepMaxNbt = 6;
static bool conv_depth2() {
    static const bool on = [] {
        const char* e = getenv("SEG3D_CONV_DEPTH");
        return e && atoi(e) == 2;
    }();
    return on;
}

template <int NBT, int RB>
int launch_split(const void* x, const int32_t* nbr, int64_t m_out, const void* wp, const float* bias, const void* addend,
                 const int32_t* row_order, int cin, int cout, void* y, int relu, int io, hipStream_t st,
                 const float* x_add = nullptr, LnEpilogue ln = LnEpilogue{nullptr, nullptr, 0.f}) {
    dim3 grid((unsigned)ceil_div64(m_out, 4 * RB * 16), (unsigned)((cout / 16) / NBT));
    static const int xcd_run = [] {
        const char* e = getenv("SEG3D_CONV_XCD_RUN");
        return (e && atoi(e) == 1) ? 1 : 0;
    }();
    if (xcd_run && nbr != nullptr && io == 0 && grid.x >= 64) {
        grid.x = (grid.x + 7) / 8 * 8;
        relu |= 2;
    }
    static const int col_adjacent = [] {
        const char* e = getenv("SEG3D_LINEAR_COLGROUPS");
        return (e && atoi(e) == 0) ? 0 : 1;
    }();
    if (col_adjacent && nbr == nullptr && grid.y > 1 && (io == 0 || io == 3 || io == 4)) {
        grid.x = (grid.x + 7) / 8 * 8 * grid.y;
        grid.y = 1;
        relu |= 4;
    }
    if (io == 5) {
        if (nbr != nullptr || NBT * 16 != cout || !ln.gamma || !ln.beta) return SEG3D_EINVAL;
        hipLaunchKernelGGL((spconv_split_kernel<NBT, RB, true, 5>), grid, dim3(256), 0, st, x, nbr, m_out,
                           reinterpret_cast<const uint4*>(wp), bias, addend, nullptr, cin, cout, y, 0, nullptr, ln);
        SEG3D_CHECK_LAUNCH();
        return SEG3D_OK;
    }
    if (io == 1 || io == 2) {
        if (nbr == nullptr) return SEG3D_EINVAL;
        if (io == 1)
            hipLaunchKernelGGL((spconv_split_kernel<NBT, RB, false, 1>), grid, dim3(256), 0, st, x, nbr, m_out,
                               reinterpret_cast<const uint4*>(wp), bias, addend, row_order, cin, cout, y, relu, nullptr, LnEpilogue{nullptr, nullptr, 0.f});
        else
            hipLaunchKernelGGL((spconv_split_kernel<NBT, RB, false, 2>), grid, dim3(256), 0, st, x, nbr, m_out,
                               reinterpret_cast<const uint4*>(wp), bias, addend, row_order, cin, cout, y, relu, nullptr, LnEpilogue{nullptr, nullptr, 0.f});
        SEG3D_CHECK_LAUNCH();
        return SEG3D_OK;
    }
    if (nbr == nullptr && io == 4)
        hipLaunchKernelGGL((spconv_split_kernel<NBT, RB, true, 4>), grid, dim3(256), 0, st, x, nbr, m_out,
                           reinterpret_cast<const uint4*>(wp), bias, addend, nullptr, cin, cout, y, relu, nullptr, LnEpilogue{nullptr, nullptr, 0.f});
    else if (nbr == nullptr && x_add)
        hipLaunchKernelGGL((spconv_split_kernel<NBT, RB, true, 3>), grid, dim3(256), 0, st, x, nbr, m_out,
                           reinterpret_cast<const uint4*>(wp), bias, addend, nullptr, cin, cout, y, relu, x_add, LnEpilogue{nullptr, nullptr, 0.f});
    else if (nbr == nullptr)
        hipLaunchKernelGGL((spconv_split_kernel<NBT, RB, true>), grid, dim3(256), 0, st, x, nbr, m_out,
                           reinterpret_cast<const uint4*>(wp), bias, addend, nullptr, cin, cout, y, relu, nullptr, LnEpilogue{nullptr, nullptr, 0.f});
    else if (NBT <= kDeepMaxNbt && conv_depth2())
        hipLaunchKernelGGL((spconv_split_kernel<NBT, RB, false, 0, (NBT <= kDeepMaxNbt ? 2 : 1)>), grid, dim3(256), 0, st, x, nbr,
                           m_out, reinterpret_cast<const uint4*>(wp), bias, addend, row_order, cin, cout, y, relu, nullptr, LnEpilogue{nullptr, nullptr, 0.f});
    else
        hipLaunchKernelGGL((spconv_split_kernel<NBT, RB, false>), grid, dim3(256), 0, st, x, nbr, m_out,
                           reinterpret_cast<const uint4*>(wp), bias, addend, row_order, cin, cout, y, relu, nullptr, LnEpilogue{nullptr, nullptr, 0.f});
    SEG3D_CHECK_LAUNCH();
    return SEG3D_OK;
}

}

size_t spconv_split_packed_bytes(int cin_op, int cout_op, int kk) {
    return (size_t)kk * ((cin_op + 31) / 32) * (cout_op / 16) * 1024 * sizeof(__bf16);
}

int spconv_split_pack(const float* weight, int cin, int cout, int kk, int transpose, int flip, void* w_packed,
                      hipStream_t st) {
    const int cin_op = transpose ? cout : cin, cout_op = transpose ? cin : cout;
    const int64_t items = (int64_t)kk * ((cin_op + 31) / 32) * (cout_op / 16) * 64;
    hipLaunchKernelGGL(pack_weight_split, dim3((unsigned)ceil_div64(items, 256)), dim3(256), 0, st, weight, cin, cout, kk,
                       transpose, flip, items, reinterpret_cast<__bf16*>(w_packed));
    SEG3D_CHECK_LAUNCH();
    return SEG3D_OK;
}

static std::atomic<int> g_forced_nbt{[] {
    const char* e = getenv("SEG3D_CONV_NBT");
    return e ? atoi(e) : 0;
}()};

extern "C" int seg3d_debug_set_conv_nbt(int32_t nbt) {
    if (nbt != 0 && nbt != 1 && nbt != 2 && nbt != 3 && nbt != 4 && nbt != 6 && nbt != 8 && nbt != 12) return SEG3D_EINVAL;
    g_forced_nbt.store(nbt, std::memory_order_relaxed);
    return SEG3D_OK;
}

int linear_stream_fwd(const float* x, int64_t m, const void* wp, const float* bias, const float* addend, int cin, int cout,
                      float* y, int io, hipStream_t st);

static int split_fwd_impl(const void* x, const int32_t* nbr, int64_t m_out, const void* wp, const float* bias,
                          const void* addend, const int32_t* row_order, int cin, int cout, void* y, int relu, int io,
                          hipStream_t st, const float* x_add, LnEpilogue ln) {
    if (x_add && (nbr || io != 0)) return SEG3D_EINVAL;
    if (io == 4 && (nbr || !addend)) return SEG3D_EINVAL;
    if (!nbr && !row_order && !relu && !x_add && (io == 0 || io == 4) && g_forced_nbt.load(std::memory_order_relaxed) == 0) {
        const int rc = linear_stream_fwd(static_cast<const float*>(x), m_out, wp, bias, static_cast<const float*>(addend), cin,
                                         cout, static_cast<float*>(y), io, st);
        if (rc != 1) return rc;
    }
    const int nb = cout / 16;
    const int64_t row_tiles = ceil_div64(m_out, 4 * 2 * 16);
    int pick = 1;
    if (nb % 12 == 0) pick = row_tiles >= 400 ? 12 : (nb % 8 == 0 ? 8 : 6);
    else if (nb % 6 == 0) pick = 6;
    else if (nb % 4 == 0) pick = 4;
    else if (nb % 3 == 0) pick = 3;
    else if (nb % 2 == 0) pick = 2;
    if (const int w = g_forced_nbt.load(std::memory_order_relaxed); w > 0 && nb % w == 0) pick = w;
    if (io == 5) {
        if (nb != 1 && nb != 2 && nb != 3 && nb != 4 && nb != 6 && nb != 8 && nb != 12) return SEG3D_EINVAL;
        pick = nb;
    }
    switch (pick) {
        case 12: return launch_split<12, 2>(x, nbr, m_out, wp, bias, addend, row_order, cin, cout, y, relu, io, st, x_add, ln);
        case 8: return launch_split<8, 2>(x, nbr, m_out, wp, bias, addend, row_order, cin, cout, y, relu, io, st, x_add, ln);
        case 6: return launch_split<6, 2>(x, nbr, m_out, wp, bias, addend, row_order, cin, cout, y, relu, io, st, x_add, ln);
        case 4: return launch_split<4, 2>(x, nbr, m_out, wp, bias, addend, row_order, cin, cout, y, relu, io, st, x_add, ln);
        case 3: return launch_split<3, 2>(x, nbr, m_out, wp, bias, addend, row_order, cin, cout, y, relu, io, st, x_add, ln);
        case 2: return launch_split<2, 2>(x, nbr, m_out, wp, bias, addend, row_order, cin, cout, y, relu, io, st, x_add, ln);
        default: return launch_split<1, 2>(x, nbr, m_out, wp, bias, addend, row_order, cin, cout, y, relu, io, st, x_add, ln);
    }
}

int spconv_split_fwd_io(const void* x, const int32_t* nbr, int64_t m_out, const void* wp, const float* bias,
                        const void* addend, const int32_t* row_order, int cin, int cout, void* y, int relu, int io,
                        hipStream_t st, const float* x_add) {
    return split_fwd_impl(x, nbr, m_out, wp, bias, addend, row_order, cin, cout, y, relu, io, st, x_add,
                          LnEpilogue{nullptr, nullptr, 0.f});
}

int spconv_split_fwd(const float* x, const int32_t* nbr, int64_t m_out, const void* wp, const float* bias,
                     const float* addend, const int32_t* row_order, int cin, int cout, float* y, int relu, hipStream_t st) {
    return spconv_split_fwd_io(x, nbr, m_out, wp, bias, addend, row_order, cin, cout, y, relu, 0, st, nullptr);
}

extern "C" {

int seg3d_pack_weights_batched(const void* jobs, int32_t n_jobs, int64_t total_blocks, void* stream) {
    if (n_jobs < 0 || total_blocks < 0 || total_blocks > 0x7FFFFFFF || (n_jobs > 0 && !jobs)) return SEG3D_EINVAL;
    if (n_jobs == 0 || total_blocks == 0) return SEG3D_OK;
    hipLaunchKernelGGL(pack_weights_batched, dim3((unsigned)total_blocks), dim3(256), 0, as_stream(stream),
                       static_cast<const PackJob*>(jobs), (int)n_jobs);
    SEG3D_CHECK_LAUNCH();
    return SEG3D_OK;
}

size_t seg3d_linear_packed_bytes(int32_t cin, int32_t cout, int32_t transpose) {
    if (cin <= 0 || cout <= 0) return 0;
    return spconv_split_packed_bytes(transpose ? cout : cin, transpose ? cin : cout, 1);
}

int seg3d_linear_pack_weight(const float* weight, int32_t cin, int32_t cout, int32_t transpose, void* w_packed,
                             void* stream) {
    const int cin_op = transpose ? cout : cin, cout_op = transpose ? cin : cout;
    if (!weight || !w_packed || cin <= 0 || cout <= 0 || (cin_op & 7) || (cout_op & 15)) return SEG3D_EINVAL;
    return spconv_split_pack(weight, cin, cout, 1, transpose ? 1 : 0, 0, w_packed, as_stream(stream));
}

int seg3d_linear_fwd(const float* x, int64_t m, const void* w_packed, const float* bias, const float* addend, int32_t cin,
                     int32_t cout, float* y, void* stream) {
    if (m < 0 || cin <= 0 || cout <= 0 || (cin & 7) || (cout & 15) || !w_packed) return SEG3D_EINVAL;
    if (m == 0) return SEG3D_OK;
    if (!x || !y) return SEG3D_EINVAL;
    return spconv_split_fwd(x, nullptr, m, w_packed, bias, addend, nullptr, cin, cout, y, 0, as_stream(stream));
}

int seg3d_linear_layernorm_fwd(const float* x, int64_t m, const void* w_packed, const float* bias, const float* res,
                               const float* gamma, const float* beta, float eps, int32_t cin, int32_t cout, float* y,
                               void* stream) {
    if (m < 0 || cin <= 0 || cout <= 0 || (cin & 7) || (cout & 15) || !w_packed || !gamma || !beta) return SEG3D_EINVAL;
    const int nb = cout / 16;
    if (nb != 1 && nb != 2 && nb != 3 && nb != 4 && nb != 6 && nb != 8 && nb != 12) return SEG3D_EINVAL;
    if (m == 0) return SEG3D_OK;
    if (!x || !y) return SEG3D_EINVAL;
    return split_fwd_impl(x, nullptr, m, w_packed, bias, res, nullptr, cin, cout, y, 0, 5, as_stream(stream), nullptr,
                          LnEpilogue{gamma, beta, eps});
}

int seg3d_linear_fwd_mul(const float* x, int64_t m, const void* w_packed, const float* factor, int32_t cin, int32_t cout,
                         float* y, void* stream) {
    if (m < 0 || cin <= 0 || cout <= 0 || (cin & 7) || (cout & 15) || !w_packed) return SEG3D_EINVAL;
    if (m == 0) return SEG3D_OK;
    if (!x || !factor || !y) return SEG3D_EINVAL;
    return spconv_split_fwd_io(x, nullptr, m, w_packed, nullptr, factor, nullptr, cin, cout, y, 0, 4, as_stream(stream), nullptr);
}

int seg3d_linear_fwd_sum(const float* x, const float* x_add, int64_t m, const void* w_packed, const float* bias, int32_t cin,
                         int32_t cout, float* y, void* stream) {
    if (m < 0 || cin <= 0 || cout <= 0 || (cin & 7) || (cout & 15) || !w_packed) return SEG3D_EINVAL;
    if (m == 0) return SEG3D_OK;
    if (!x || !x_add || !y) return SEG3D_EINVAL;
    return spconv_split_fwd_io(x, nullptr, m, w_packed, bias, nullptr, nullptr, cin, cout, y, 0, 0, as_stream(stream), x_add);
}

}
```

### openseg3d_amd/csrc/voxelize.hip

```cpp
#include <cstdio>

#include "common.hpp"

namespace {

constexpr int kThreads = 256;

struct VoxParams {
    int32_t grid[3];
    int32_t row_stride, xyz_col, batch_col;
};

template <typename T>
struct VoxConst {
    T lo[3];
    T vs[3];
};

__device__ __forceinline__ float floor_t(float v) { return floorf(v); }
__device__ __forceinline__ double floor_t(double v) { return floor(v); }

template <typename T>
__global__ __launch_bounds__(kThreads) void vox_insert(const T* __restrict__ pts, int64_t n, VoxParams p,
                                                       VoxConst<T> c, HashView h, uint32_t* __restrict__ slot_of) {
// ... 167 lines not shown


inline float floor_h(float v) { return __builtin_floorf(v); }
inline double floor_h(double v) { return __builtin_floor(v); }

inline uint64_t host_capacity(int64_t n) {
    uint64_t cap = 64;
    while (cap < (uint64_t)(2 * n + 2)) cap <<= 1;
    return cap;
}

template <typename T>
int voxelize_host_impl(const T* points, int64_t n, int32_t row_stride, int32_t xyz_col, int32_t batch_col,
                       const float* voxel_size, const float* range, int32_t* voxel_coords, int32_t* point_voxel_ids,
                       int32_t* n_voxels, void* workspace, size_t workspace_bytes) {
    if (n < 0 || n >= (int64_t)0x7F000000 || !voxel_size || !range || !n_voxels || row_stride < 3 || xyz_col < 0 ||
        xyz_col + 3 > row_stride || batch_col >= row_stride)
        return SEG3D_EINVAL;
    if (n > 0 && (!points || !point_voxel_ids || !voxel_coords || !workspace)) return SEG3D_EINVAL;
    const uint64_t cap = host_capacity(n);
    if (n > 0 && workspace_bytes < cap * 12) return SEG3D_EWORKSPACE;
    int32_t grid[3];
    if (seg3d_grid_size(voxel_size, range, grid) != SEG3D_OK) return SEG3D_EINVAL;
    *n_voxels = 0;
    if (n == 0) return SEG3D_OK;
    uint64_t* keys = static_cast<uint64_t*>(workspace);
    int32_t* vals = reinterpret_cast<int32_t*>(keys + cap);
    for (uint64_t s = 0; s < cap; ++s) keys[s] = ~0ull;
    T lo[3], vs[3];
    for (int j = 0; j < 3; ++j) {
        lo[j] = (T)range[j];
        vs[j] = (T)voxel_size[j];
    }
    int32_t count = 0;
    for (int64_t i = 0; i < n; ++i) {
        const T* row = points + i * row_stride;
        int32_t cc[3];
        bool ok = true;
        for (int j = 0; j < 3 && ok; ++j) {
            volatile T d = row[xyz_col + j] - lo[j];
            volatile T q = d / vs[j];
            const T v = floor_h((T)q);
            if (!(v >= (T)0) || v >= (T)grid[j]) ok = false;
            else cc[j] = (int32_t)v;
        }
        if (!ok) {
            point_voxel_ids[i] = -1;
            continue;
        }
        const int64_t b = batch_col >= 0 ? (int64_t)row[batch_col] : 0;
        const uint64_t key = (uint64_t)(((b * grid[2] + cc[2]) * grid[1] + cc[1]) * (int64_t)grid[0] + cc[0]);
        uint64_t h = key * 0x9E3779B97F4A7C15ull;
        uint64_t s = (h ^ (h >> 29)) & (cap - 1);
        while (keys[s] != key && keys[s] != ~0ull) s = (s + 1) & (cap - 1);
        if (keys[s] == ~0ull) {
            keys[s] = key;
            vals[s] = count;
            int32_t* o = voxel_coords + 4 * (int64_t)count;
            o[0] = (int32_t)b;
            o[1] = cc[2];
            o[2] = cc[1];
            o[3] = cc[0];
            ++count;
        }
        point_voxel_ids[i] = vals[s];
    }
    *n_voxels = count;
    return SEG3D_OK;
}

}

extern "C" {

int seg3d_cart2polar_f32(const float* points, int64_t n_points, int32_t row_stride, int32_t xyz_col, float* out, void* stream) {
    return cart2polar_impl<float>(points, n_points, row_stride, xyz_col, out, stream);
}

int seg3d_cart2polar_f64(const double* points, int64_t n_points, int32_t row_stride, int32_t xyz_col, double* out,
                         void* stream) {
    return cart2polar_impl<double>(points, n_points, row_stride, xyz_col, out, stream);
}

int seg3d_abi_version(void) { return 49; }

namespace {
thread_local char g_last_error[320] = "";
}

const char* seg3d_last_error(void) { return g_last_error; }

int seg3d_grid_size(const float* voxel_size, const float* range, int32_t* grid_xyz) {
    if (!voxel_size || !range || !grid_xyz) return SEG3D_EINVAL;
    for (int j = 0; j < 3; ++j) {
        volatile float span = range[3 + j] - range[j];
        volatile float g = span / voxel_size[j];
        grid_xyz[j] = (int32_t)__builtin_rintf(g);
        if (grid_xyz[j] <= 0) return SEG3D_EINVAL;
    }
    return SEG3D_OK;
}

size_t seg3d_voxelize_workspace_bytes(int64_t n_points) { return ws_bytes(n_points < 0 ? 0 : n_points); }

int seg3d_voxelize_f32(const float* points, int64_t n_points, int32_t row_stride, int32_t xyz_col, int32_t batch_col,
                       const float* voxel_size, const float* range, int32_t* voxel_coords, int32_t* point_voxel_ids,
                       int32_t* n_voxels, void* workspace, size_t workspace_bytes, void* stream) {
    return voxelize_impl<float>(points, n_points, row_stride, xyz_col, batch_col, voxel_size, range, voxel_coords,
                                point_voxel_ids, n_voxels, workspace, workspace_bytes, stream);
}

int seg3d_voxelize_f64(const double* points, int64_t n_points, int32_t row_stride, int32_t xyz_col, int32_t batch_col,
                       const float* voxel_size, const float* range, int32_t* voxel_coords, int32_t* point_voxel_ids,
                       int32_t* n_voxels, void* workspace, size_t workspace_bytes, void* stream) {
    return voxelize_impl<double>(points, n_points, row_stride, xyz_col, batch_col, voxel_size, range, voxel_coords,
                                 point_voxel_ids, n_voxels, workspace, workspace_bytes, stream);
}

size_t seg3d_voxelize_host_workspace_bytes(int64_t n_points) { return (size_t)host_capacity(n_points < 0 ? 0 : n_points) * 12; }

int seg3d_voxelize_host_f32(const float* points, int64_t n_points, int32_t row_stride, int32_t xyz_col, int32_t batch_col,
                            const float* voxel_size, const float* range, int32_t* voxel_coords, int32_t* point_voxel_ids,
                            int32_t* n_voxels, void* workspace, size_t workspace_bytes) {
    return voxelize_host_impl<float>(points, n_points, row_stride, xyz_col, batch_col, voxel_size, range, voxel_coords,
                                     point_voxel_ids, n_voxels, workspace, workspace_bytes);
}

int seg3d_voxelize_host_f64(const double* points, int64_t n_points, int32_t row_stride, int32_t xyz_col, int32_t batch_col,
                            const float* voxel_size, const float* range, int32_t* voxel_coords, int32_t* point_voxel_ids,
                            int32_t* n_voxels, void* workspace, size_t workspace_bytes) {
    return voxelize_host_impl<double>(points, n_points, row_stride, xyz_col, batch_col, voxel_size, range, voxel_coords,
                                      point_voxel_ids, n_voxels, workspace, workspace_bytes);
}

}

void seg3d_note_hip_error(int code, const char* file, int line) {
    const char* base = file;
    for (const char* p = file; *p; ++p)
        if (*p == '/') base = p + 1;
    snprintf(g_last_error, sizeof(g_last_error), "%s (%s) at %s:%d", hipGetErrorString((hipError_t)code),
             hipGetErrorName((hipError_t)code), base, line);
}
```

### openseg3d_amd/csrc/wgrad_dense.hip

```cpp
#include <cstdlib>
#include <type_traits>

#include "attn_common.hpp"

int wgrad_dense_lds_plan(int64_t m, int cin, int cout, int* chunks, int64_t* rows);
int wgrad_dense_lds_launch(const float* x, const float* dy, int64_t m, int cin, int cout, int chunks, int64_t rows, float* part,
                           int want_bias, hipStream_t st);

namespace {

using namespace attn;

constexpr int kWaves = 4;
constexpr int kThreads = 64 * kWaves;

struct Plan {
    int nbo, nbi;
    int chunks;
    int64_t rows;
    int group;
    int lds;
};

static const bool g_wgrad_group = [] {
    const char* e = getenv("SEG3D_WGRAD_GROUP");
    return e && atoi(e) == 1;
}();

Plan plan(int64_t m, int cin, int cout, bool allow_lds = false) {
    Plan p{(cout + 63) / 64, (cin + 63) / 64, 0, 32, 0, 0};
    if (m <= 0) return p;
    if (allow_lds) {
        int c = 0;
        int64_t r = 0;
        if (wgrad_dense_lds_plan(m, cin, cout, &c, &r)) {
            p.chunks = c;
            p.rows = r;
            p.lds = 1;
            return p;
        }
    }
    if (g_wgrad_group && p.nbo * p.nbi >= 4 && m >= 8192) {
        int best_b = 0, best_c = 0;
        float best = 1e9f;
        for (int qb = 1; qb <= 4; ++qb)
            for (int qc = 1; qb * qc <= 4; ++qc) {
                if (p.nbo % qb || p.nbi % qc || qb * qc < 3) continue;
                const float slabs = (float)(qb + qc) / (float)(qb * qc) - 0.01f * (float)(qb * qc);
                if (slabs < best) best = slabs, best_b = qb, best_c = qc;
            }
        if (best_b) {
            p.group = best_b << 4 | best_c;
            const int groups = (p.nbo / best_b) * (p.nbi / best_c);
            int64_t chunks = 512 / groups / 8 * 8;
            if (chunks < 8) chunks = 8;
            int64_t rows = (m + chunks - 1) / chunks;
            if (rows < 32 * 8) rows = 32 * 8;
            rows = (rows + 31) / 32 * 32;
            p.rows = rows;
            p.chunks = (int)((m + rows - 1) / rows);
            return p;
        }
    }
    const int tiles = p.nbo * p.nbi;
    int target = tiles >= 16 ? 1024 : 512;
    if (const char* e = getenv("SEG3D_WGRAD_TARGET")) target = atoi(e);
    int64_t chunks = target / tiles / 8 * 8;
    if (chunks < 8) chunks = 8;
    int64_t rows = (m + chunks - 1) / chunks;
    if (rows < 32 * kWaves * 4) rows = 32 * kWaves * 4;
    rows = (rows + 31) / 32 * 32;
    p.rows = rows;
    p.chunks = (int)((m + rows - 1) / rows);
    return p;
}

__device__ __forceinline__ bf16x8 frag_from_bf16_rows(const uint2* q, int comp) {
    u32x4 h;
#pragma unroll
    for (int j = 0; j < 4; ++j) {
        const uint32_t a = (comp & 2) ? q[2 * j].y : q[2 * j].x, b = (comp & 2) ? q[2 * j + 1].y : q[2 * j + 1].x;
        h[j] = (comp & 1) ? ((a >> 16) | (b & 0xFFFF0000u)) : ((a & 0xFFFFu) | (b << 16));
    }
    return __builtin_bit_cast(bf16x8, h);
}

__device__ __forceinline__ f32x4 mfma2(const bf16x8& a_hi, const bf16x8& a_lo, const bf16x8& b, f32x4 acc) {
    acc = __builtin_amdgcn_mfma_f32_16x16x32_bf16(a_lo, b, acc, 0, 0, 0);
    acc = __builtin_amdgcn_mfma_f32_16x16x32_bf16(a_hi, b, acc, 0, 0, 0);
    return acc;
}

template <bool XB, bool GROUP, int DEPTH = 1>
__global__ __launch_bounds__(kThreads, (DEPTH > 1 ? 1 : 2)) void wgrad_dense_kernel(const void* __restrict__ x_v, const float* __restrict__ dy,
                                                               int64_t m_rows, int cin, int cout, int rows_per_chunk,
                                                               int nbi, int tiles, float* __restrict__ part,
                                                               int want_bias, int group) {
    const float* x = static_cast<const float*>(x_v);
    __shared__ __attribute__((aligned(16))) float red[GROUP ? 4 : 64 * 64];
    __shared__ float red_b[GROUP ? 1 : kWaves][64];
    const int lane = threadIdx.x & 63, wave = threadIdx.x >> 6;
    const int cq = lane & 15, rg = lane >> 4;
    const int xcd = blockIdx.x & 7, k = blockIdx.x >> 3;
    const int chunk = (k / tiles) * 8 + xcd, tile = k % tiles;
    int bi = tile % nbi, bo = tile / nbi;
    if constexpr (GROUP) {
        const int qb = group >> 4, qc = group & 15;
        if (wave >= qb * qc) return;
        bo = bo * qb + wave / qc;
        bi = bi * qc + wave % qc;
    }
    const int ci0 = bi * 64, co0 = bo * 64;
    const int64_t r_begin = (int64_t)chunk * rows_per_chunk;
    if (r_begin >= m_rows) return;
    const int64_t r_end = r_begin + rows_per_chunk < m_rows ? r_begin + rows_per_chunk : m_rows;
    const bool a_ok = co0 + 4 * cq < cout, b_ok = ci0 + 4 * cq < cin;
    const uint32_t yoff = (uint32_t)((8 * rg * cout + (a_ok ? co0 + 4 * cq : 0)) * 4);
    const uint32_t xoff = (uint32_t)((8 * rg * cin + (b_ok ? ci0 + 4 * cq : 0)) * (XB ? 2 : 4));
    const bool want_db = want_bias && bi == 0;

    f32x4 acc[4][4];
#pragma unroll
    for (int a = 0; a < 4; ++a)
#pragma unroll
        for (int b = 0; b < 4; ++b) acc[a][b] = (f32x4){0.f, 0.f, 0.f, 0.f};
    f32x4 db_acc = {0.f, 0.f, 0.f, 0.f};

    f32x4 xr[XB ? 1 : 8], yr[8];
    f32x4 xd[DEPTH > 1 ? DEPTH : 1][8], yd[DEPTH > 1 ? DEPTH : 1][8];
    uint2 xq[XB ? 8 : 1];
    bf16x8 b_hi[4], b_lo[XB ? 1 : 4];
    auto load_rows = [&](const float* src, int ld, uint32_t off, int step, f32x4(&dst)[8]) {
        const char* base = reinterpret_cast<const char*>(src + (r_begin + 32 * (int64_t)step) * ld);
#pragma unroll
        for (int i = 0; i < 8; ++i) dst[i] = *reinterpret_cast<const f32x4*>(base + (size_t)i * ld * 4 + off);
    };
    auto load_x = [&](int step, auto& xs) {
        if constexpr (XB) {
            const char* base = static_cast<const char*>(x_v) + (r_begin + 32 * (int64_t)step) * cin * 2;
#pragma unroll
            for (int i = 0; i < 8; ++i) xq[i] = *reinterpret_cast<const uint2*>(base + (size_t)i * cin * 2 + xoff);
        } else {
            const char* base = reinterpret_cast<const char*>(x + (r_begin + 32 * (int64_t)step) * cin);
#pragma unroll
            for (int i = 0; i < 8; ++i) xs[i] = *reinterpret_cast<const f32x4*>(base + (size_t)i * cin * 4 + xoff);
        }
    };
    auto make_b = [&](auto& xs) {
#pragma unroll
        for (int b = 0; b < 4; ++b) {
            if constexpr (XB) {
                b_hi[b] = frag_from_bf16_rows(xq, b);
            } else {
                float v[8];
#pragma unroll
                for (int i = 0; i < 8; ++i) v[i] = xs[i][b];
                split_frag(v, &b_hi[b], &b_lo[b]);
            }
        }
    };
    auto multiply = [&](auto& ys) {
        if (want_db) {
#pragma unroll
            for (int i = 0; i < 8; ++i) db_acc += ys[i];
        }
#pragma unroll
        for (int a = 0; a < 4; ++a) {
            float v[8];
#pragma unroll
            for (int i = 0; i < 8; ++i) v[i] = ys[i][a];
            bf16x8 a_hi, a_lo;
            split_frag(v, &a_hi, &a_lo);
#pragma unroll
            for (int b = 0; b < 4; ++b) {
                if constexpr (XB) acc[a][b] = mfma2(a_hi, a_lo, b_hi[b], acc[a][b]);
                else acc[a][b] = mfma3(a_hi, a_lo, b_hi[b], b_lo[b], acc[a][b]);
            }
        }
    };
    const int n_full = (int)((r_end - r_begin) / 32);
    constexpr int kStride = GROUP ? 1 : kWaves;
    int s = GROUP ? 0 : wave;
    if constexpr (DEPTH > 1) {
        static_assert(!XB && !GROUP, "the deep form is the fp32 split-K form's");
#pragma unroll
        for (int d = 0; d < DEPTH; ++d)
            if (s + d * kStride < n_full) {
                load_x(s + d * kStride, xd[d]);
                load_rows(dy, cout, yoff, s + d * kStride, yd[d]);
            }
        for (; s < n_full; s += DEPTH * kStride) {
#pragma unroll
            for (int d = 0; d < DEPTH; ++d) {
                const int cur = s + d * kStride;
                if (cur < n_full) {
                    const bool more = cur + DEPTH * kStride < n_full;
                    make_b(xd[d]);
                    if (more) load_x(cur + DEPTH * kStride, xd[d]);
// ... 109 lines not shown
#pragma unroll
            for (int u = 0; u < 4; ++u) {
                const float4 v = *reinterpret_cast<const float4*>(part + (int64_t)(c + 4 * u) * n + i);
                acc[u].x += v.x; acc[u].y += v.y; acc[u].z += v.z; acc[u].w += v.w;
            }
        }
        for (; c < chunks; c += 4) {
            const float4 v = *reinterpret_cast<const float4*>(part + (int64_t)c * n + i);
            acc[0].x += v.x; acc[0].y += v.y; acc[0].z += v.z; acc[0].w += v.w;
        }
    }
    float4 s;
    s.x = (acc[0].x + acc[1].x) + (acc[2].x + acc[3].x);
    s.y = (acc[0].y + acc[1].y) + (acc[2].y + acc[3].y);
    s.z = (acc[0].z + acc[1].z) + (acc[2].z + acc[3].z);
    s.w = (acc[0].w + acc[1].w) + (acc[2].w + acc[3].w);
    red[q][cq] = s;
    __syncthreads();
    if (q == 0 && i < n) {
        float4 t = red[0][cq];
#pragma unroll
        for (int k = 1; k < 4; ++k) {
            const float4 v = red[k][cq];
            t.x += v.x; t.y += v.y; t.z += v.z; t.w += v.w;
        }
        if (i < nw) *reinterpret_cast<float4*>(dw + i) = t;
        else if (db) *reinterpret_cast<float4*>(db + (i - nw)) = t;
    }
}

__global__ __launch_bounds__(256) void wgrad_dense_reduce(const float* __restrict__ part, int chunks, int64_t n,
                                                          int64_t nw, float* __restrict__ dw,
                                                          float* __restrict__ db) {
    reduce_block(part, chunks, n, nw, dw, db, (int64_t)blockIdx.x);
}

struct ReduceJob {
    const float* part;
    float* dw;
    float* db;
    int64_t n, nw;
    int32_t chunks, reserved;
    int64_t first_block;
};
static_assert(sizeof(ReduceJob) == 56, "ReduceJob layout is part of the C ABI (seg3d_reduce_partials_batched)");

__global__ __launch_bounds__(256) void reduce_partials_batched(const ReduceJob* __restrict__ jobs, int n_jobs) {
    int lo = 0, hi = n_jobs - 1;
    while (lo < hi) {
        const int mid = (lo + hi + 1) >> 1;
        if (jobs[mid].first_block <= (int64_t)blockIdx.x) lo = mid;
        else hi = mid - 1;
    }
    const ReduceJob jb = jobs[lo];
    reduce_block(jb.part, jb.chunks, jb.n, jb.nw, jb.dw, jb.db, (int64_t)blockIdx.x - jb.first_block);
}

}

int wgrad_chunk_reduce(const float* part, int chunks, int64_t n, int64_t nw, float* dw, float* db, hipStream_t st) {
    hipLaunchKernelGGL(wgrad_dense_reduce, dim3((unsigned)ceil_div64(n, 256)), dim3(256), 0, st, part, chunks, n, nw, dw, db);
    SEG3D_CHECK_LAUNCH();
    return SEG3D_OK;
}

extern "C" size_t seg3d_linear_wgrad_workspace_bytes(int64_t m, int32_t cin, int32_t cout) {
    if (m < 0 || cin <= 0 || cout <= 0) return 0;
    const Plan p = plan(m, cin, cout), q = plan(m, cin, cout, true);
    return ((size_t)(p.chunks > q.chunks ? p.chunks : q.chunks) * ((size_t)cin * cout + cout) + 64) * sizeof(float);
}

static void launch_dense(const Plan& p, const void* x, bool x_bf16, const float* dy, int64_t m, int cin, int cout, float* part,
                         int want_bias, hipStream_t st) {
    if (p.lds) {
        wgrad_dense_lds_launch(static_cast<const float*>(x), dy, m, cin, cout, p.chunks, p.rows, part, want_bias, st);
        return;
    }
    if (p.group) {
        const int qb = p.group >> 4, qc = p.group & 15;
        const int nbi_g = p.nbi / qc, groups = (p.nbo / qb) * nbi_g;
        const unsigned blocks = (unsigned)((p.chunks + 7) / 8 * 8) * (unsigned)groups;
        if (x_bf16)
            hipLaunchKernelGGL((wgrad_dense_kernel<true, true>), dim3(blocks), dim3(kThreads), 0, st, x, dy, m, cin, cout, (int)p.rows,
                               nbi_g, groups, part, want_bias, p.group);
        else
            hipLaunchKernelGGL((wgrad_dense_kernel<false, true>), dim3(blocks), dim3(kThreads), 0, st, x, dy, m, cin, cout, (int)p.rows,
                               nbi_g, groups, part, want_bias, p.group);
        return;
    }
    const int tiles = p.nbo * p.nbi;
    const unsigned blocks = (unsigned)((p.chunks + 7) / 8 * 8) * (unsigned)tiles;
    static const int depth = [] {
        const char* e = getenv("SEG3D_WGRAD_DENSE_DEPTH");
        return (e && atoi(e) == 3) ? 3 : 1;
    }();
    if (!x_bf16 && depth == 3) {
        hipLaunchKernelGGL((wgrad_dense_kernel<false, false, 3>), dim3(blocks), dim3(kThreads), 0, st, x, dy, m, cin, cout, (int)p.rows,
                           p.nbi, tiles, part, want_bias, 0);
        return;
    }
    if (x_bf16)
        hipLaunchKernelGGL((wgrad_dense_kernel<true, false>), dim3(blocks), dim3(kThreads), 0, st, x, dy, m, cin, cout, (int)p.rows,
                           p.nbi, tiles, part, want_bias, 0);
    else
        hipLaunchKernelGGL((wgrad_dense_kernel<false, false>), dim3(blocks), dim3(kThreads), 0, st, x, dy, m, cin, cout, (int)p.rows,
                           p.nbi, tiles, part, want_bias, 0);
}

static int linear_wgrad_partials(const void* x, bool x_bf16, const float* dy, int64_t m, int32_t cin, int32_t cout,
                                 int32_t with_bias, void* workspace, size_t workspace_bytes, int32_t* chunks, void* stream) {
    if (m < 0 || cin <= 0 || cout <= 0 || (cin & 3) || (cout & 3) || !chunks) return SEG3D_EINVAL;
    if (m > 0 && (!x || !dy)) return SEG3D_EINVAL;
    if (workspace_bytes < seg3d_linear_wgrad_workspace_bytes(m, cin, cout) || (m > 0 && !workspace)) return SEG3D_EINVAL;
    *chunks = 0;
    if (m == 0) return SEG3D_OK;
    const Plan p = plan(m, cin, cout, !x_bf16);
    launch_dense(p, x, x_bf16, dy, m, cin, cout, static_cast<float*>(workspace), with_bias ? 1 : 0, as_stream(stream));
    SEG3D_CHECK_LAUNCH();
    *chunks = p.chunks;
    return SEG3D_OK;
}

extern "C" int seg3d_linear_wgrad_partials(const float* x, const float* dy, int64_t m, int32_t cin, int32_t cout,
                                           int32_t with_bias, void* workspace, size_t workspace_bytes, int32_t* chunks,
                                           void* stream) {
    return linear_wgrad_partials(x, false, dy, m, cin, cout, with_bias, workspace, workspace_bytes, chunks, stream);
}

extern "C" int seg3d_linear_wgrad_partials_xbf16(const uint16_t* x_bf16, const float* dy, int64_t m, int32_t cin, int32_t cout,
                                                 int32_t with_bias, void* workspace, size_t workspace_bytes, int32_t* chunks,
                                                 void* stream) {
    return linear_wgrad_partials(x_bf16, true, dy, m, cin, cout, with_bias, workspace, workspace_bytes, chunks, stream);
}

extern "C" int seg3d_reduce_partials(const float* part, int32_t chunks, int64_t n, int64_t nw, float* dw, float* db,
                                     void* stream) {
    if (chunks < 0 || n <= 0 || nw < 0 || nw > n || (n & 3) || (nw & 3) || !dw || (chunks > 0 && !part)) return SEG3D_EINVAL;
    return wgrad_chunk_reduce(part, chunks, n, nw, dw, db, as_stream(stream));
}

extern "C" int seg3d_reduce_partials_batched(const void* jobs, int32_t n_jobs, int64_t total_blocks, void* stream) {
    if (n_jobs < 0 || total_blocks < 0 || total_blocks > 0x7FFFFFFF || (n_jobs > 0 && !jobs)) return SEG3D_EINVAL;
    if (n_jobs == 0 || total_blocks == 0) return SEG3D_OK;
    hipLaunchKernelGGL(reduce_partials_batched, dim3((unsigned)total_blocks), dim3(256), 0, as_stream(stream),
                       static_cast<const ReduceJob*>(jobs), (int)n_jobs);
    SEG3D_CHECK_LAUNCH();
    return SEG3D_OK;
}

extern "C" int seg3d_linear_wgrad(const float* x, const float* dy, int64_t m, int32_t cin, int32_t cout, float* dw,
                                  float* db, void* workspace, size_t workspace_bytes, void* stream) {
    if (m < 0 || cin <= 0 || cout <= 0 || (cin & 3) || (cout & 3) || !dw) return SEG3D_EINVAL;
    if (m > 0 && (!x || !dy)) return SEG3D_EINVAL;
    if (workspace_bytes < seg3d_linear_wgrad_workspace_bytes(m, cin, cout) || (m > 0 && !workspace)) return SEG3D_EINVAL;
    hipStream_t st = as_stream(stream);
    const Plan p = plan(m, cin, cout, true);
    float* part = static_cast<float*>(workspace);
    if (m > 0) {
        launch_dense(p, x, false, dy, m, cin, cout, part, db ? 1 : 0, st);
        SEG3D_CHECK_LAUNCH();
    }
    const int64_t nw = (int64_t)cin * cout;
    return wgrad_chunk_reduce(part, p.chunks, nw + cout, nw, dw, db, st);
}
```

### openseg3d_amd/ops.py

```python
import ctypes
import weakref
import os

import numpy as np
import torch

from . import _lib
from ._lib import REDUCE_MAX, REDUCE_MEAN, REDUCE_SUM

_F3 = ctypes.c_float * 3
_F6 = ctypes.c_float * 6
_I3 = ctypes.c_int32 * 3


def _need_gpu(*tensors):
    for t in tensors:
        if t is not None and not t.is_cuda:
            raise _lib.Seg3dError("openseg3d_amd ops run on the GPU only (no CPU fallback); got a CPU tensor")


def _ptr(t):
    return None if t is None else ctypes.c_void_p(t.data_ptr())


# ... 1411 lines not shown
            f"window attention: {heads} heads on {v.shape[1]} channels is not a head geometry of this path (head widths "
            "6 with 4 / 8 / 16 heads, 12 with 4 / 8 / 12 / 16 heads, 24 / 48 with up to 16 heads; the reference builds 8 heads "
            "on 48 / 96 / 192 / 384 channels, pointtransformer.py:143-155)")
    return _WindowAttnPackedFn.apply(qk, v, tau, tau_min, heads, wi, float(drop_p), int(drop_seed))


INPROJ_SUM = os.environ.get("SEG3D_INPROJ_SUM", "1") != "0"


class _AttnInProjFn(torch.autograd.Function):

    @staticmethod
    def forward(ctx, x, pos, w_in, b_in):
        x = _f32c(x)
        c = x.shape[1]
        if (INPROJ_SUM and not any(ctx.needs_input_grad) and pos.shape == x.shape and pos.dtype == torch.float32
                and pos.is_contiguous()):
            qk = torch.empty((x.shape[0], 2 * c), dtype=torch.float32, device=x.device)
            _lib.call("seg3d_linear_fwd_sum", _ptr(x), _ptr(pos), x.shape[0], _ptr(_linear_pack(w_in[: 2 * c], 0)),
                      _ptr(b_in[: 2 * c]), c, 2 * c, _ptr(qk), _stream())
            return qk, _linear_apply(x, _linear_pack(w_in[2 * c:], 0), b_in[2 * c:], c, c)
        xp = x + pos
        qk = _linear_apply(xp, _linear_pack(w_in[: 2 * c], 0), b_in[: 2 * c], c, 2 * c)
        v = _linear_apply(x, _linear_pack(w_in[2 * c:], 0), b_in[2 * c:], c, c)
        keep = ctx.needs_input_grad[2]
        ctx.save_for_backward(_saved_rows(x) if keep else x, _saved_rows(xp) if keep else xp, w_in)
        ctx.b_in = b_in
        return qk, v

    @staticmethod
    def backward(ctx, dqk, dv):
        x, xp, w_in = ctx.saved_tensors
        c = x.shape[1]
        m = x.shape[0]
        dqk, dv = _f32c(dqk), _f32c(dv)
        dx = dpos = dw = db = None
        fk = _WgradFork(x.device)
        if ctx.needs_input_grad[2]:
            dw = torch.empty((3 * c, c), dtype=torch.float32, device=x.device)
            db = torch.empty((3 * c,), dtype=torch.float32, device=x.device)
            for src, dy, r0, rows in ((xp, dqk, 0, 2 * c), (x, dv, 2 * c, c)):
                _linear_wgrad_into(fk, src, dy, c, rows, dw.data_ptr() + 4 * r0 * c, db.data_ptr() + 4 * r0)
        if ctx.needs_input_grad[0] or ctx.needs_input_grad[1]:
            extra = None if ctx.needs_input_grad[1] else getattr(ctx, "dx_addend", None)
            d_xp = _linear_apply(dqk, _linear_pack(w_in[: 2 * c], 1), None, 2 * c, c, addend=extra)
            if ctx.needs_input_grad[1]:
                dpos = d_xp
            if ctx.needs_input_grad[0]:
                dx = _linear_apply(dv, _linear_pack(w_in[2 * c:], 1), None, c, c, addend=d_xp)
        fk.join((w_in, dw), (ctx.b_in, db if ctx.needs_input_grad[3] else None))
        return dx, dpos, dw, (db if ctx.needs_input_grad[3] else None)


def attn_in_proj(x, pos, w_in, b_in):
    c = x.shape[1]
    fits = (x.is_cuda and x.dim() == 2 and x.dtype == torch.float32 and c % 16 == 0 and CONV_PRECISION == "bf16x3"
            and w_in.is_contiguous() and b_in is not None)
    if not fits:
        return linear(x + pos, w_in[: 2 * c], None if b_in is None else b_in[: 2 * c]), \
            linear(x, w_in[2 * c:], None if b_in is None else b_in[2 * c:])
    return _AttnInProjFn.apply(x, pos, w_in, b_in)


def window_attention(q, k, v, tau, tau_min, heads, wi):
    _need_gpu(q, k, v, tau)
    for t in (q, k, v):
        if t.dtype != torch.float32 or t.stride(1) != 1:
            raise _lib.Seg3dError("q/k/v must be float32 with a contiguous last dimension")
    return _WindowAttnFn.apply(q, k, v, tau, tau_min, heads, wi)


def _linear_wgrad(x, dy, cin, cout, want_db=True, fork=None):
    dw = torch.empty((cout, cin), dtype=torch.float32, device=dy.device)
    db = torch.empty((cout,), dtype=torch.float32, device=dy.device) if want_db else None
    if fork is not None:
        _linear_wgrad_into(fork, x, dy, cin, cout, dw.data_ptr(), db.data_ptr() if want_db else 0)
        return dw, db
    ws_bytes = _lib.query("seg3d_linear_wgrad_workspace_bytes", x.shape[0], cin, cout)
    ws = _workspace(ws_bytes, dy.device)
    _lib.call("seg3d_linear_wgrad", _ptr(x), _ptr(dy), x.shape[0], cin, cout, _ptr(dw), _ptr(db), _ptr(ws), ws_bytes, _stream())
    return dw, db


def _linear_wgrad_into(fk, x, dy, cin, cout, dw_ptr, db_ptr, *keep):
    m = x.shape[0]
    ws_bytes = _lib.query("seg3d_linear_wgrad_workspace_bytes", m, cin, cout)
    ws = _workspace(ws_bytes, dy.device)
    chunks = ctypes.c_int32(0)
    _lib.call("seg3d_linear_wgrad_partials_xbf16" if x.dtype == torch.bfloat16 else "seg3d_linear_wgrad_partials",
              _ptr(x), _ptr(dy), m, cin, cout, 1 if db_ptr else 0, _ptr(ws), ws_bytes,
              ctypes.byref(chunks), fk.fork(ws, x, dy, *keep))
    fk.add_reduce(ws, chunks.value, cin * cout + cout, cin * cout, dw_ptr, db_ptr, *keep)


class _Ctx:

    def __init__(self, *needs):
        self.needs_input_grad = needs
        self.saved_tensors = ()

    def save_for_backward(self, *tensors):
        self.saved_tensors = tensors


GELU_SAVED_GRAD = os.environ.get("SEG3D_GELU_SAVED_GRAD", "1") != "0"


class _EncoderLayerFn(torch.autograd.Function):

    @staticmethod
    def forward(ctx, x, pos, w_in, b_in, tau, w_out, b_out, g1, be1, w1, b1, w2, b2, g2, be2, meta):
        heads, tau_min, wi, eps1, eps2, s1, s2, drop_p, drop_seed = meta
        x = _f32c(x)
        c = x.shape[1]
        live = any(ctx.needs_input_grad)
        c_in = _Ctx(live, False, live, live)
        qk, v = _AttnInProjFn.forward(c_in, x, pos, w_in, b_in)
        c_at = _Ctx(True, True, True, False, False, False)
        o = _WindowAttnPackedFn.forward(c_at, qk, v, tau, tau_min, heads, wi, drop_p, drop_seed)
        fuse_ln = (LINEAR_LN_FUSED and not live and s1 is None and s2 is None and (c // 16) in (1, 2, 3, 4, 6, 8, 12)
                   and b_out is not None and b2 is not None)
        c_n1 = _Ctx(True, True, True, True, False, False)
        if fuse_ln:
            x1 = _linear_layernorm(o, _linear_pack(w_out, 0), b_out, x, g1, be1, eps1, c, c)
        else:
            a = _linear_apply(o, _linear_pack(w_out, 0), b_out, c, c)
            x1 = _LayerNormResidualFn.forward(c_n1, a, x, g1, be1, eps1, s1)
        hid = w1.shape[0]
        h = _linear_apply(x1, _linear_pack(w1, 0), b1, c, hid)
        if live and GELU_SAVED_GRAD:
            g, gp = torch.empty_like(h), torch.empty_like(h)
            _lib.call("seg3d_gelu_fwd", _ptr(h), h.numel(), _ptr(g), _ptr(gp), _stream())
            h = gp
        else:
            g = torch.nn.functional.gelu(h)
        c_n2 = _Ctx(True, True, True, True, False, False)
        if fuse_ln:
            x2 = _linear_layernorm(g, _linear_pack(w2, 0), b2, x1, g2, be2, eps2, hid, c)
        else:
            m = _linear_apply(g, _linear_pack(w2, 0), b2, hid, c)
            x2 = _LayerNormResidualFn.forward(c_n2, m, x1, g2, be2, eps2, s2)
        ctx.parts = (c_in, c_at, c_n1, c_n2)
        ctx.save_for_backward(_saved_rows(o), _saved_rows(x1), h, _saved_rows(g), w_out, w1, w2)
        ctx.bias_params = (b_out, b1, b2)
        ctx.norm_params = (g1, be1, g2, be2)
        return x2

    @staticmethod
    def backward(ctx, dx2):
        c_in, c_at, c_n1, c_n2 = ctx.parts
        o, x1, h, g, w_out, w1, w2 = ctx.saved_tensors
        dx2 = _f32c(dx2)
        c, hid = x1.shape[1], w1.shape[0]
        fk = _WgradFork(dx2.device)
        c_n1.fork = c_n2.fork = fk
        dm, _, dg2, dbe2, _, _ = _LayerNormResidualFn.backward(c_n2, dx2)
        dw2, db2 = _linear_wgrad(g, dm, hid, c, fork=fk)
        if GELU_SAVED_GRAD:
            dh = torch.empty((dm.shape[0], hid), dtype=torch.float32, device=dm.device)
            _lib.call("seg3d_linear_fwd_mul", _ptr(dm), dm.shape[0], _ptr(_linear_pack(w2, 1)), _ptr(h), c, hid, _ptr(dh),
                      _stream())
        else:
            dh = torch.ops.aten.gelu_backward(_linear_apply(dm, _linear_pack(w2, 1), None, c, hid), h)
        dw1, db1 = _linear_wgrad(x1, dh, c, hid, fork=fk)
        d_x1 = _linear_apply(dh, _linear_pack(w1, 1), None, hid, c, addend=dx2)
        da, _, dg1, dbe1, _, _ = _LayerNormResidualFn.backward(c_n1, d_x1)
        dw_out, db_out = _linear_wgrad(o, da, c, c, fork=fk)
        do = _linear_apply(da, _linear_pack(w_out, 1), None, c, c)
        dqk, dv, dtau = _WindowAttnPackedFn.backward(c_at, do)[:3]
        c_in.dx_addend = d_x1
        dx, _, dw_in, db_in = _AttnInProjFn.backward(c_in, dqk, dv)
        b_out, b1, b2 = ctx.bias_params
        g1, be1, g2, be2 = ctx.norm_params
        fk.join((w_out, dw_out), (w1, dw1), (w2, dw2), (b_out, db_out), (b1, db1), (b2, db2), (g1, dg1), (be1, dbe1),
                (g2, dg2), (be2, dbe2))
        c_n1.fork = c_n2.fork = None
        ctx.parts = None
        return dx, None, dw_in, db_in, dtau, dw_out, db_out, dg1, dbe1, dw1, db1, dw2, db2, dg2, dbe2, None


def encoder_layer_fits(x, c, hid, heads):
    return (x.is_cuda and x.dim() == 2 and x.dtype == torch.float32 and c % 16 == 0 and hid % 16 == 0 and c <= 512
            and c % heads == 0 and CONV_PRECISION == "bf16x3")


class _SegmentReduceFn(torch.autograd.Function):
    @staticmethod
    def forward(ctx, x, seg, mode):
        x = _f32c(x)
        n, c = x.shape
        out = torch.empty((seg.n_segments, c), dtype=torch.float32, device=x.device)
        arg = torch.empty((seg.n_segments, c), dtype=torch.int32, device=x.device) if mode == REDUCE_MAX else None
        _lib.call("seg3d_segment_reduce_fwd", _ptr(x), c, _ptr(seg.order), _ptr(seg.offsets), seg.n_segments, mode,
                  _ptr(out), _ptr(arg), _stream())
        ctx.seg, ctx.mode, ctx.arg, ctx.n = seg, mode, arg, n
        return out

    @staticmethod
    def backward(ctx, dout):
        dout = _f32c(dout)
        c = dout.shape[1]
        seg = ctx.seg
        if ctx.mode == REDUCE_MAX:
            dx = torch.zeros((ctx.n, c), dtype=torch.float32, device=dout.device)
        else:
            dx = torch.empty((ctx.n, c), dtype=torch.float32, device=dout.device)
        _lib.call("seg3d_segment_reduce_bwd", _ptr(dout), c, _ptr(seg.ids), ctx.n, _ptr(seg.offsets), _ptr(ctx.arg),
                  seg.n_segments, ctx.mode, _ptr(dx), _stream())
        return dx, None, None


def segment_reduce(x, seg, mode):
    _need_gpu(x)
    return _SegmentReduceFn.apply(x, seg, mode)


_MODES = {"sum": REDUCE_SUM, "add": REDUCE_SUM, "mean": REDUCE_MEAN, "max": REDUCE_MAX}


def scatter(src, index, dim=0, reduce="sum", dim_size=None):
    if dim != 0 or src.dim() != 2:
        raise _lib.Seg3dError("scatter: only dim=0 on [N, C] tensors is on this path")
    _need_gpu(src, index)
    n_seg = int(index.max().item()) + 1 if dim_size is None else int(dim_size)
    return segment_reduce(src, SegmentIndex(index, n_seg), _MODES[reduce])


class _GatherRowsFn(torch.autograd.Function):
    @staticmethod
    def forward(ctx, feats, ids, seg):
        feats = _f32c(feats)
        n, c = ids.shape[0], feats.shape[1]
        out = torch.empty((n, c), dtype=torch.float32, device=feats.device)
        _lib.call("seg3d_gather_rows", _ptr(feats), _ptr(ids), n, c, _ptr(out), _stream())
        ctx.ids, ctx.seg, ctx.m = ids, seg, feats.shape[0]
        return out

    @staticmethod
    def backward(ctx, dout):
        dout = _f32c(dout)
        seg = ctx.seg if ctx.seg is not None else SegmentIndex(ctx.ids, ctx.m)
        c = dout.shape[1]
        dfeat = torch.empty((ctx.m, c), dtype=torch.float32, device=dout.device)
        _lib.call("seg3d_segment_reduce_fwd", _ptr(dout), c, _ptr(seg.order), _ptr(seg.offsets), ctx.m, REDUCE_SUM,
                  _ptr(dfeat), None, _stream())
        return dfeat, None, None


def gather_rows(feats, ids, seg=None):
    _need_gpu(feats, ids)
    return _GatherRowsFn.apply(feats, _i32c(ids), seg)


def voxel_to_point(feats, coords):
    return gather_rows(feats, coords)


def voxel_max_pooling(feats, coords):
    return scatter(feats, coords, reduce="max")
# ... 1319 lines not shown
```

### openseg3d_amd/swformer.py

```python
import math
import os

import numpy as np

import torch
import torch.nn as nn
import torch.nn.functional as F

from . import ops


def window_geometry(sparse_shape_xyz, window_shape, do_shift):
    win = [int(w) for w in window_shape]
    if len(win) != 3:
        raise NotImplementedError("3-D windows only (config.py:68 WINDOW_SHAPE)")
    s = [float(v) for v in sparse_shape_xyz]
    nwin = [int(np.ceil(s[i] / win[i]) + 1) for i in range(3)]
    shift = [w // 2 for w in win] if do_shift else list(win)
    if s[2] == win[2]:
        shift[2] = 0
    return win, nwin, shift


class WindowPlan:
# ... 70 lines not shown
class CosineMultiheadAttention(nn.Module):

    def __init__(self, embed_dim, num_heads, dropout=0.0, tau_min=0.01):
        super().__init__()
        if embed_dim % num_heads:
            raise ValueError("embed_dim must be divisible by num_heads")
        self.embed_dim, self.num_heads, self.tau_min, self.dropout = embed_dim, num_heads, tau_min, dropout
        self.in_proj_weight = nn.Parameter(torch.empty(3 * embed_dim, embed_dim))
        self.in_proj_bias = nn.Parameter(torch.zeros(3 * embed_dim))
        self.out_proj = nn.Linear(embed_dim, embed_dim)
        self.tau = nn.Parameter(torch.ones(1, 1, 1))
        nn.init.xavier_uniform_(self.in_proj_weight)
        nn.init.constant_(self.out_proj.bias, 0.0)

    def drop_args(self, seed):
        if self.training and self.dropout > 0.0:
            return float(self.dropout), int(seed)
        return 0.0, 0

    def forward(self, x, pos, wi, seed=0):
        qk, v = ops.attn_in_proj(x, pos, self.in_proj_weight, self.in_proj_bias)
        drop_p, drop_seed = self.drop_args(seed)
        o = ops.window_attention_packed(qk, v, self.tau, self.tau_min, self.num_heads, wi, drop_p, drop_seed)
        return ops.linear(o, self.out_proj.weight, self.out_proj.bias)


class WindowAttention(nn.Module):
    def __init__(self, d_model, nhead, attn_drop, tau_min=0.01):
        super().__init__()
        self.self_attn = CosineMultiheadAttention(d_model, nhead, dropout=attn_drop, tau_min=tau_min)

    def forward(self, feat_2d, pos, wi, seed=0):
        return self.self_attn(feat_2d, pos, wi, seed)


class MLP(nn.Module):
    def __init__(self, in_features, hidden_features, drop=0.0):
        super().__init__()
        self.fc1 = nn.Linear(in_features, hidden_features)
        self.fc2 = nn.Linear(hidden_features, in_features)
        self.drop = drop

    def forward(self, x):
        x = F.gelu(ops.linear(x, self.fc1.weight, self.fc1.bias))
        if self.drop and self.training:
            x = F.dropout(x, self.drop)
        x = ops.linear(x, self.fc2.weight, self.fc2.bias)
        if self.drop and self.training:
            x = F.dropout(x, self.drop)
        return x


def attention_dropout_seed():
    return int(torch.randint(0, 2 ** 62, (1,), dtype=torch.int64).item())


def drop_path_scale(x, p):
    keep = 1.0 - p
    mask = x.new_empty((x.shape[0],)).bernoulli_(keep)
    if keep > 0.0:
        mask.div_(keep)
    return mask


def drop_path(x, p, training):
    if p == 0.0 or not training:
        return x
    return x * drop_path_scale(x, p).reshape((x.shape[0],) + (1,) * (x.dim() - 1))


FUSED_LAYER = os.environ.get("SEG3D_FUSED_LAYER", "1") != "0"


class EncoderLayer(nn.Module):

    def __init__(self, d_model, nhead, mlp_hidden_dim, drop=0.0, attn_drop=0.1, drop_path_rate=0.0):
        super().__init__()
        self.win_attn = WindowAttention(d_model, nhead, attn_drop)
        self.norm1 = nn.LayerNorm(d_model)
        self.norm2 = nn.LayerNorm(d_model)
        self.mlp = MLP(d_model, mlp_hidden_dim, drop=drop)
        self.drop_path_rate = float(drop_path_rate)

    def forward(self, x, pos, wi, scales=None, seed=None):
        at, mlp = self.win_attn.self_attn, self.mlp
        if seed is None:
            seed = attention_dropout_seed() if self.training and at.dropout > 0.0 else 0
        drop = self.training and self.drop_path_rate > 0.0
        s1 = s2 = None
        if drop:
            s1, s2 = scales if scales is not None else (drop_path_scale(x, self.drop_path_rate),
                                                        drop_path_scale(x, self.drop_path_rate))
        if (FUSED_LAYER and torch.is_grad_enabled() and x.requires_grad and not mlp.drop and at.in_proj_bias is not None
                and ops.encoder_layer_fits(x, at.embed_dim, mlp.fc1.out_features, at.num_heads)):
            meta = (at.num_heads, at.tau_min, wi, self.norm1.eps, self.norm2.eps, s1, s2) + at.drop_args(seed)
            return ops._EncoderLayerFn.apply(x, pos, at.in_proj_weight, at.in_proj_bias, at.tau, at.out_proj.weight,
                                             at.out_proj.bias, self.norm1.weight, self.norm1.bias, mlp.fc1.weight,
                                             mlp.fc1.bias, mlp.fc2.weight, mlp.fc2.bias, self.norm2.weight,
                                             self.norm2.bias, meta)
        a = self.win_attn(x, pos, wi, seed)
        x = ops.layer_norm_residual(a, x, self.norm1, rowscale=s1)
        return ops.layer_norm_residual(self.mlp(x), x, self.norm2, rowscale=s2)


class SWFormerBlock(nn.Module):
    def __init__(self, d_model, nhead, depth=4, mlp_ratio=2.0, attn_drop=0.1, drop=0.0, drop_path=0.0):
        super().__init__()
        self.depth = depth
        rates = drop_path if isinstance(drop_path, (list, tuple)) else [drop_path] * depth
        self.layers = nn.ModuleList(
            EncoderLayer(d_model, nhead, int(d_model * mlp_ratio), drop=drop, attn_drop=attn_drop,
                         drop_path_rate=rates[i]) for i in range(depth))
        self._keep = None

    def forward(self, voxel_info):
        x, plan = voxel_info["voxel_features"], voxel_info["plan"]
        if x.dtype == torch.bfloat16:
            x = x.float()
        half = int(self.depth / 2)
        scales = self.drop_path_scales(x) if self.training else None
        seed = attention_dropout_seed() if self.training else 0
        for i, layer in enumerate(self.layers):
            s = 0 if i < half else 1
            x = layer(x, plan.pos[s], plan.index[s], None if scales is None else (scales[2 * i], scales[2 * i + 1]), seed + i)
        return x

    def drop_path_scales(self, x):
        rates = [layer.drop_path_rate for layer in self.layers]
        if not any(r > 0.0 for r in rates):
            return None
        if self._keep is None or self._keep.device != x.device:
            self._keep = torch.tensor([1.0 - r for r in rates for _ in (0, 1)], dtype=torch.float32, device=x.device)[:, None]
        u = torch.rand((2 * self.depth, x.shape[0]), dtype=torch.float32, device=x.device)
        return (u < self._keep).to(torch.float32).div_(self._keep)
```

Baseline: 4.166 million points/s.

## Skip MLP compute for DropPath-dropped rows via row partitioning in fused encoder layer

```diff
diff --git a/include/seg3d_hip.h b/include/seg3d_hip.h
--- a/include/seg3d_hip.h
+++ b/include/seg3d_hip.h
@@ -213,6 +213,23 @@
                           float momentum, float* running_mean, float* running_var, float* stats, void* workspace,
                           size_t workspace_bytes, void* stream);
 int seg3d_gelu_fwd(const float* h, int64_t n, float* g, float* gp, void* stream);
+size_t seg3d_row_partition_workspace_bytes(int32_t n_masks, int64_t m);
+int seg3d_row_partition(const float* scale, int32_t n_masks, int64_t m, uint64_t skip_bits, int32_t* order, int32_t* inv,
+                        int32_t* gather, int32_t* n_keep, void* workspace, size_t workspace_bytes, void* stream);
+int seg3d_linear_fwd_rows(const float* x, int64_t m, const int32_t* n_live, const int32_t* row_out, const void* w_packed,
+                          const float* bias, const float* addend, int32_t mul, int32_t cin, int32_t cout, float* y,
+                          void* stream);
+int seg3d_gelu_fwd_rows(const float* h, int64_t m, int32_t c, const int32_t* n_live, float* g, float* gp, void* stream);
+int seg3d_layernorm_fwd_rows(const float* x, const float* res, const float* gamma, const float* beta, const float* rowscale,
+                             const int32_t* x_row, const int32_t* copy_row, float* y_copy, float eps, int64_t m, int32_t c,
+                             float* y, float* mean, float* rstd, void* stream);
+int seg3d_layernorm_bwd_partials_rows(const float* dy, const float* x, const float* mean, const float* rstd,
+                                      const float* gamma, const float* rowscale, const int32_t* order,
+                                      const int32_t* n_live, int64_t m, int32_t c, float* dx, void* workspace,
+                                      size_t workspace_bytes, int32_t* nblocks, void* stream);
+int seg3d_linear_wgrad_partials_rows(const float* x, const float* dy, int64_t m, const int32_t* n_live, int32_t cin,
+                                     int32_t cout, int32_t with_bias, void* workspace, size_t workspace_bytes,
+                                     int32_t* chunks, void* stream);
 int seg3d_affine_act(const float* x, const float* res, const float* scale, const float* shift, int32_t relu,
                      int64_t m, int32_t c, float* y, void* stream);
 int seg3d_batchnorm_bwd(const float* dy, const float* y, const float* x, const float* mean, const float* rstd,
diff --git a/openseg3d_amd/_lib.py b/openseg3d_amd/_lib.py
--- a/openseg3d_amd/_lib.py
+++ b/openseg3d_amd/_lib.py
@@ -8,7 +8,7 @@
 
 OK, EINVAL, EWORKSPACE, ELAUNCH = 0, -1, -2, -3
 REDUCE_SUM, REDUCE_MEAN, REDUCE_MAX = 0, 1, 2
-ABI_VERSION = 49
+ABI_VERSION = 50
 
 _p, _i32, _i64, _sz, _f = ctypes.c_void_p, ctypes.c_int32, ctypes.c_int64, ctypes.c_size_t, ctypes.c_float
 _u64 = ctypes.c_uint64
@@ -95,6 +95,13 @@
     "seg3d_batchnorm_stats": (ctypes.c_int, [_p, _i64, _i32, _f, _p, _p, _f, _p, _p, _p, _p, ctypes.c_size_t, _p]),
     "seg3d_affine_act": (ctypes.c_int, [_p, _p, _p, _p, _i32, _i64, _i32, _p, _p]),
     "seg3d_gelu_fwd": (ctypes.c_int, [_p, _i64, _p, _p, _p]),
+    "seg3d_row_partition_workspace_bytes": (_sz, [_i32, _i64]),
+    "seg3d_row_partition": (ctypes.c_int, [_p, _i32, _i64, _u64, _p, _p, _p, _p, _p, _sz, _p]),
+    "seg3d_linear_fwd_rows": (ctypes.c_int, [_p, _i64, _p, _p, _p, _p, _p, _i32, _i32, _i32, _p, _p]),
+    "seg3d_gelu_fwd_rows": (ctypes.c_int, [_p, _i64, _i32, _p, _p, _p, _p]),
+    "seg3d_layernorm_fwd_rows": (ctypes.c_int, [_p, _p, _p, _p, _p, _p, _p, _p, _f, _i64, _i32, _p, _p, _p, _p]),
+    "seg3d_layernorm_bwd_partials_rows": (ctypes.c_int, [_p, _p, _p, _p, _p, _p, _p, _p, _i64, _i32, _p, _p, _sz, _p, _p]),
+    "seg3d_linear_wgrad_partials_rows": (ctypes.c_int, [_p, _p, _i64, _p, _i32, _i32, _i32, _p, _sz, _p, _p]),
     "seg3d_batchnorm_bwd": (ctypes.c_int, [_p, _p, _p, _p, _p, _p, _i32, _i64, _i32, _p, _p, _p, _p, ctypes.c_size_t, _p]),
     "seg3d_batchnorm_bwd_reduce": (ctypes.c_int, [_p, _p, _p, _p, _p, _i32, _i64, _i32, _p, _p, ctypes.c_size_t, _p]),
     "seg3d_batchnorm_bwd_apply": (ctypes.c_int, [_p, _p, _p, _p, _p, _p, _p, _p, _i32, _i64, _i32, _p, _p, _p]),
diff --git a/openseg3d_amd/csrc/rownorm.hip b/openseg3d_amd/csrc/rownorm.hip
--- a/openseg3d_amd/csrc/rownorm.hip
+++ b/openseg3d_amd/csrc/rownorm.hip
@@ -32,7 +32,8 @@
                                                           const float* __restrict__ gamma, const float* __restrict__ beta,
                                                           const float* __restrict__ rowscale, float eps, int64_t m, int c,
                                                           RowMap rm, float* __restrict__ y, float* __restrict__ mean,
-                                                          float* __restrict__ rstd) {
+                                                          float* __restrict__ rstd, const int32_t* __restrict__ x_row,
+                                                          const int32_t* __restrict__ copy_row, float* __restrict__ y_copy) {
     const int lane = threadIdx.x & 63, wave = threadIdx.x >> 6;
     const int rows_per_wave = 64 / rm.p;
     const int lr = lane / rm.p, lq = lane % rm.p;
@@ -41,13 +42,15 @@
          base += (int64_t)gridDim.x * 4 * rows_per_wave) {
         const int64_t row = base + lr;
         const bool rok = row < m;
+        const int64_t xr = x_row ? (rok ? (int64_t)x_row[row] : -1) : row;
+        const bool live = rok && xr >= 0;
         float4 v[ITEMS];
         float s = 0.f;
 #pragma unroll
         for (int i = 0; i < ITEMS; ++i) {
             const int q = lq + i * rm.p;
             v[i] = make_float4(0.f, 0.f, 0.f, 0.f);
-            if (rok && q < rm.quads) v[i] = *reinterpret_cast<const float4*>(x + row * c + 4 * q);
+            if (live && q < rm.quads) v[i] = *reinterpret_cast<const float4*>(x + xr * c + 4 * q);
             s += (v[i].x + v[i].y) + (v[i].z + v[i].w);
         }
         const float mu = group_sum(s, rm.p) * inv_c;
@@ -62,27 +65,33 @@
         }
         const float rs = rsqrtf(group_sum(ss, rm.p) * inv_c + eps);
         const float sc = rowscale && rok ? rowscale[row] : 1.0f;
+        const int64_t cr = copy_row && rok ? (int64_t)copy_row[row] : -1;
 #pragma unroll
         for (int i = 0; i < ITEMS; ++i) {
             const int q = lq + i * rm.p;
             if (rok && q < rm.quads) {
-                const float4 g = *reinterpret_cast<const float4*>(gamma + 4 * q);
-                const float4 b = *reinterpret_cast<const float4*>(beta + 4 * q);
                 float4 o;
-                o.x = ((v[i].x - mu) * rs * g.x + b.x) * sc;
-                o.y = ((v[i].y - mu) * rs * g.y + b.y) * sc;
-                o.z = ((v[i].z - mu) * rs * g.z + b.z) * sc;
-                o.w = ((v[i].w - mu) * rs * g.w + b.w) * sc;
-                if (res) {
-                    const float4 r4 = *reinterpret_cast<const float4*>(res + row * c + 4 * q);
-                    o.x += r4.x; o.y += r4.y; o.z += r4.z; o.w += r4.w;
+                if (live) {
+                    const float4 g = *reinterpret_cast<const float4*>(gamma + 4 * q);
+                    const float4 b = *reinterpret_cast<const float4*>(beta + 4 * q);
+                    o.x = ((v[i].x - mu) * rs * g.x + b.x) * sc;
+                    o.y = ((v[i].y - mu) * rs * g.y + b.y) * sc;
+                    o.z = ((v[i].z - mu) * rs * g.z + b.z) * sc;
+                    o.w = ((v[i].w - mu) * rs * g.w + b.w) * sc;
+                    if (res) {
+                        const float4 r4 = *reinterpret_cast<const float4*>(res + row * c + 4 * q);
+                        o.x += r4.x; o.y += r4.y; o.z += r4.z; o.w += r4.w;
+                    }
+                } else {
+                    o = *reinterpret_cast<const float4*>(res + row * c + 4 * q);
                 }
                 *reinterpret_cast<float4*>(y + row * c + 4 * q) = o;
+                if (cr >= 0) *reinterpret_cast<float4*>(y_copy + cr * c + 4 * q) = o;
             }
         }
-        if (rok && lq == 0 && mean) {
-            mean[row] = mu;
-            rstd[row] = rs;
+        if (live && lq == 0 && mean) {
+            mean[xr] = mu;
+            rstd[xr] = rs;
         }
     }
 }
@@ -92,7 +101,9 @@
                                                           const float* __restrict__ mean, const float* __restrict__ rstd,
                                                           const float* __restrict__ gamma, const float* __restrict__ rowscale,
                                                           int64_t m, int c, RowMap rm, float* __restrict__ dx,
-                                                          float* __restrict__ part ) {
+                                                          float* __restrict__ part ,
+                                                          const int32_t* __restrict__ order,
+                                                          const int32_t* __restrict__ n_live) {
     extern __shared__ float red[];
     const int lane = threadIdx.x & 63, wave = threadIdx.x >> 6;
     const int rows_per_wave = 64 / rm.p;
@@ -102,12 +113,18 @@
 #pragma unroll
     for (int i = 0; i < ITEMS; ++i) ag[i] = ab[i] = make_float4(0.f, 0.f, 0.f, 0.f);
 
-    for (int64_t base = ((int64_t)blockIdx.x * 4 + wave) * rows_per_wave; base < m;
+    int64_t live = m, m_pad = m;
+    if (n_live) {
+        live = n_live[0] < 0 ? 0 : (n_live[0] < m ? (int64_t)n_live[0] : m);
+        m_pad = (live + 127) / 128 * 128 < m ? (live + 127) / 128 * 128 : m;
+    }
+    for (int64_t base = ((int64_t)blockIdx.x * 4 + wave) * rows_per_wave; base < m_pad;
          base += (int64_t)gridDim.x * 4 * rows_per_wave) {
         const int64_t row = base + lr;
-        const bool rok = row < m;
+        const bool rok = row < live;
+        const int64_t yrow = order && rok ? (int64_t)order[row] : row;
         const float mu = rok ? mean[row] : 0.f, rs = rok ? rstd[row] : 0.f;
-        const float sc = rowscale && rok ? rowscale[row] : 1.0f;
+        const float sc = rowscale && rok ? rowscale[yrow] : 1.0f;
         float4 xh[ITEMS], gy[ITEMS];
         float s1 = 0.f, s2 = 0.f;
 #pragma unroll
@@ -116,7 +133,7 @@
             xh[i] = gy[i] = make_float4(0.f, 0.f, 0.f, 0.f);
             if (rok && q < rm.quads) {
                 const float4 xv = *reinterpret_cast<const float4*>(x + row * c + 4 * q);
-                float4 dv = *reinterpret_cast<const float4*>(dy + row * c + 4 * q);
+                float4 dv = *reinterpret_cast<const float4*>(dy + yrow * c + 4 * q);
                 dv.x *= sc; dv.y *= sc; dv.z *= sc; dv.w *= sc;
                 const float4 g = *reinterpret_cast<const float4*>(gamma + 4 * q);
                 xh[i] = make_float4((xv.x - mu) * rs, (xv.y - mu) * rs, (xv.z - mu) * rs, (xv.w - mu) * rs);
@@ -138,6 +155,8 @@
                 o.z = rs * (gy[i].z - c1 - xh[i].z * c2);
                 o.w = rs * (gy[i].w - c1 - xh[i].w * c2);
                 *reinterpret_cast<float4*>(dx + row * c + 4 * q) = o;
+            } else if (row < m_pad && q < rm.quads) {
+                *reinterpret_cast<float4*>(dx + row * c + 4 * q) = make_float4(0.f, 0.f, 0.f, 0.f);
             }
         }
     }
@@ -267,7 +286,12 @@
 }
 
 __global__ __launch_bounds__(kThreads) void gelu_fwd_kernel(const float* __restrict__ h, int64_t quads, float* __restrict__ g,
-                                                            float* __restrict__ gp) {
+                                                            float* __restrict__ gp, const int32_t* __restrict__ n_live,
+                                                            int row_quads) {
+    if (n_live) {
+        const int64_t lq = (n_live[0] < 0 ? 0 : (int64_t)n_live[0]) * row_quads;
+        quads = lq < quads ? lq : quads;
+    }
     for (int64_t t = (int64_t)blockIdx.x * kThreads + threadIdx.x; t < quads; t += (int64_t)gridDim.x * kThreads) {
         const float4 v = reinterpret_cast<const float4*>(h)[t];
         const float in[4] = {v.x, v.y, v.z, v.w};
@@ -390,10 +414,10 @@
     const unsigned nb = blocks_for(m, 4 * (64 / rm.p));
     if (rm.items == 1)
         hipLaunchKernelGGL(ln_fwd_kernel<1>, dim3(nb), dim3(kThreads), 0, as_stream(stream), x, res, gamma, beta, rowscale,
-                           eps, m, c, rm, y, mean, rstd);
+                           eps, m, c, rm, y, mean, rstd, nullptr, nullptr, nullptr);
     else
         hipLaunchKernelGGL(ln_fwd_kernel<2>, dim3(nb), dim3(kThreads), 0, as_stream(stream), x, res, gamma, beta, rowscale,
-                           eps, m, c, rm, y, mean, rstd);
+                           eps, m, c, rm, y, mean, rstd, nullptr, nullptr, nullptr);
     SEG3D_CHECK_LAUNCH();
     return SEG3D_OK;
 }
@@ -419,10 +443,10 @@
     const size_t smem = (size_t)4 * (64 / rm.p) * 2 * c * sizeof(float);
     if (rm.items == 1)
         hipLaunchKernelGGL(ln_bwd_kernel<1>, dim3(nb), dim3(kThreads), smem, st, dy, x, mean, rstd, gamma, rowscale, m, c, rm,
-                           dx, part);
+                           dx, part, nullptr, nullptr);
     else
         hipLaunchKernelGGL(ln_bwd_kernel<2>, dim3(nb), dim3(kThreads), smem, st, dy, x, mean, rstd, gamma, rowscale, m, c, rm,
-                           dx, part);
+                           dx, part, nullptr, nullptr);
     SEG3D_CHECK_LAUNCH();
     *nblocks = (int32_t)nb;
     return SEG3D_OK;
@@ -444,10 +468,10 @@
         const size_t smem = (size_t)4 * (64 / rm.p) * 2 * c * sizeof(float);
         if (rm.items == 1)
             hipLaunchKernelGGL(ln_bwd_kernel<1>, dim3(nb), dim3(kThreads), smem, st, dy, x, mean, rstd, gamma, rowscale, m, c,
-                               rm, dx, part);
+                               rm, dx, part, nullptr, nullptr);
         else
             hipLaunchKernelGGL(ln_bwd_kernel<2>, dim3(nb), dim3(kThreads), smem, st, dy, x, mean, rstd, gamma, rowscale, m, c,
-                               rm, dx, part);
+                               rm, dx, part, nullptr, nullptr);
         SEG3D_CHECK_LAUNCH();
     }
     hipLaunchKernelGGL(ln_bwd_reduce, dim3((unsigned)((2 * c + 31) / 32)), dim3(1024), 0, st, part, (int)nb, c, dgamma,
@@ -504,8 +528,62 @@
     if (n == 0) return SEG3D_OK;
     if (!h || !g) return SEG3D_EINVAL;
     hipLaunchKernelGGL(gelu_fwd_kernel, dim3(blocks_for(n / 4, kThreads * 4)), dim3(kThreads), 0, as_stream(stream), h, n / 4, g,
-                       gp);
-    SEG3D_CHECK_LAUNCH();
+                       gp, nullptr, 0);
+    SEG3D_CHECK_LAUNCH();
+    return SEG3D_OK;
+}
+
+int seg3d_gelu_fwd_rows(const float* h, int64_t m, int32_t c, const int32_t* n_live, float* g, float* gp, void* stream) {
+    if (m < 0 || c <= 0 || (c & 3) || !n_live) return SEG3D_EINVAL;
+    if (m == 0) return SEG3D_OK;
+    if (!h || !g) return SEG3D_EINVAL;
+    const int64_t quads = m * (c / 4);
+    hipLaunchKernelGGL(gelu_fwd_kernel, dim3(blocks_for(quads, kThreads * 4)), dim3(kThreads), 0, as_stream(stream), h, quads, g,
+                       gp, n_live, c / 4);
+    SEG3D_CHECK_LAUNCH();
+    return SEG3D_OK;
+}
+
+int seg3d_layernorm_fwd_rows(const float* x, const float* res, const float* gamma, const float* beta, const float* rowscale,
+                             const int32_t* x_row, const int32_t* copy_row, float* y_copy, float eps, int64_t m, int32_t c,
+                             float* y, float* mean, float* rstd, void* stream) {
+    if (m < 0 || bad_c(c) || c > 512) return SEG3D_EINVAL;
+    if (m == 0) return SEG3D_OK;
+    if (!x || !gamma || !beta || !y || (x_row && !res) || (copy_row && !y_copy) || (mean && !rstd)) return SEG3D_EINVAL;
+    const RowMap rm = row_map(c);
+    const unsigned nb = blocks_for(m, 4 * (64 / rm.p));
+    if (rm.items == 1)
+        hipLaunchKernelGGL(ln_fwd_kernel<1>, dim3(nb), dim3(kThreads), 0, as_stream(stream), x, res, gamma, beta, rowscale,
+                           eps, m, c, rm, y, mean, rstd, x_row, copy_row, y_copy);
+    else
+        hipLaunchKernelGGL(ln_fwd_kernel<2>, dim3(nb), dim3(kThreads), 0, as_stream(stream), x, res, gamma, beta, rowscale,
+                           eps, m, c, rm, y, mean, rstd, x_row, copy_row, y_copy);
+    SEG3D_CHECK_LAUNCH();
+    return SEG3D_OK;
+}
+
+int seg3d_layernorm_bwd_partials_rows(const float* dy, const float* x, const float* mean, const float* rstd, const float* gamma,
+                                      const float* rowscale, const int32_t* order, const int32_t* n_live, int64_t m, int32_t c,
+                                      float* dx, void* workspace, size_t workspace_bytes, int32_t* nblocks, void* stream) {
+    if (m < 0 || bad_c(c) || c > 512 || !nblocks || !order || !n_live) return SEG3D_EINVAL;
+    if (workspace_bytes < seg3d_layernorm_bwd_workspace_bytes(m, c) || !workspace) return SEG3D_EWORKSPACE;
+    *nblocks = 0;
+    if (m == 0) return SEG3D_OK;
+    if (!dy || !x || !mean || !rstd || !gamma || !dx) return SEG3D_EINVAL;
+    hipStream_t st = as_stream(stream);
+    float* part = static_cast<float*>(workspace);
+    const RowMap rm = row_map(c);
+    unsigned nb = blocks_for(m, 4 * (64 / rm.p) * 4);
+    if (nb > (unsigned)kLnBwdMaxBlocks) nb = kLnBwdMaxBlocks;
+    const size_t smem = (size_t)4 * (64 / rm.p) * 2 * c * sizeof(float);
+    if (rm.items == 1)
+        hipLaunchKernelGGL(ln_bwd_kernel<1>, dim3(nb), dim3(kThreads), smem, st, dy, x, mean, rstd, gamma, rowscale, m, c, rm,
+                           dx, part, order, n_live);
+    else
+        hipLaunchKernelGGL(ln_bwd_kernel<2>, dim3(nb), dim3(kThreads), smem, st, dy, x, mean, rstd, gamma, rowscale, m, c, rm,
+                           dx, part, order, n_live);
+    SEG3D_CHECK_LAUNCH();
+    *nblocks = (int32_t)nb;
     return SEG3D_OK;
 }
 
diff --git a/openseg3d_amd/csrc/scan.hip b/openseg3d_amd/csrc/scan.hip
--- a/openseg3d_amd/csrc/scan.hip
+++ b/openseg3d_amd/csrc/scan.hip
@@ -97,6 +97,96 @@
     return SEG3D_OK;
 }
 
+__global__ __launch_bounds__(kThreads) void partition_totals(const float* __restrict__ scale, int64_t m, uint64_t skip_bits,
+                                                             uint32_t* __restrict__ sums ) {
+    __shared__ uint32_t lds[4];
+    const int r = blockIdx.y;
+    if ((skip_bits >> r) & 1ull) return;
+    const float* row = scale + (int64_t)r * m;
+    const int64_t base = (int64_t)blockIdx.x * kChunk + (int64_t)threadIdx.x * kItems;
+    uint32_t acc = 0u;
+#pragma unroll
+    for (int i = 0; i < kItems; ++i)
+        if (base + i < m) acc += row[base + i] != 0.0f ? 1u : 0u;
+    uint32_t tot;
+    block_inclusive(acc, lds, &tot);
+    if (threadIdx.x == 0) sums[(int64_t)r * gridDim.x + blockIdx.x] = tot;
+}
+
+__global__ __launch_bounds__(kThreads) void partition_scatter(const float* __restrict__ scale, int64_t m, uint64_t skip_bits,
+                                                              const uint32_t* __restrict__ sums, int32_t* __restrict__ order,
+                                                              int32_t* __restrict__ inv, int32_t* __restrict__ gather,
+                                                              int32_t* __restrict__ n_keep) {
+    __shared__ uint32_t lds[4];
+    const int r = blockIdx.y;
+    if ((skip_bits >> r) & 1ull) return;
+    const float* row = scale + (int64_t)r * m;
+    uint32_t before = 0u, all = 0u;
+    for (int j = threadIdx.x; j < (int)gridDim.x; j += kThreads) {
+        const uint32_t v = sums[(int64_t)r * gridDim.x + j];
+        all += v;
+        if (j < (int)blockIdx.x) before += v;
+    }
+    uint32_t chunk_base, kept_all;
+    block_inclusive(before, lds, &chunk_base);
+    block_inclusive(all, lds, &kept_all);
+
+    const int64_t base = (int64_t)blockIdx.x * kChunk + (int64_t)threadIdx.x * kItems;
+    bool keep[kItems];
+    uint32_t acc = 0u;
+#pragma unroll
+    for (int i = 0; i < kItems; ++i) {
+        keep[i] = base + i < m && row[base + i] != 0.0f;
+        acc += keep[i] ? 1u : 0u;
+    }
+    uint32_t tot;
+    const uint32_t incl = block_inclusive(acc, lds, &tot);
+    uint32_t kept = chunk_base + (incl - acc);
+    int32_t* o = order + (int64_t)r * m;
+    int32_t* iv = inv + (int64_t)r * m;
+    int32_t* ga = gather + (int64_t)r * m;
+#pragma unroll
+    for (int i = 0; i < kItems; ++i) {
+        const int64_t idx = base + i;
+        if (idx < m) {
+            if (keep[i]) {
+                o[kept] = (int32_t)idx;
+                ga[kept] = (int32_t)idx;
+                iv[idx] = (int32_t)kept;
+                kept += 1u;
+            } else {
+                const int64_t p = (int64_t)kept_all + (idx - (int64_t)kept);
+                o[p] = (int32_t)idx;
+                ga[p] = -1;
+                iv[idx] = -1;
+            }
+        }
+    }
+    if (blockIdx.x == 0 && threadIdx.x == 0) n_keep[r] = (int32_t)kept_all;
+}
+
+}
+
+extern "C" size_t seg3d_row_partition_workspace_bytes(int32_t n_masks, int64_t m) {
+    if (n_masks <= 0 || m < 0) return 0;
+    return (size_t)n_masks * (size_t)ceil_div64(m > 0 ? m : 1, kChunk) * sizeof(uint32_t);
+}
+
+extern "C" int seg3d_row_partition(const float* scale, int32_t n_masks, int64_t m, uint64_t skip_bits, int32_t* order,
+                                   int32_t* inv, int32_t* gather, int32_t* n_keep, void* workspace, size_t workspace_bytes,
+                                   void* stream) {
+    if (n_masks < 0 || n_masks > 64 || m < 0 || m > 0x7FFFFFFF) return SEG3D_EINVAL;
+    if (n_masks == 0) return SEG3D_OK;
+    if (!n_keep || (m > 0 && (!scale || !order || !inv || !gather))) return SEG3D_EINVAL;
+    if (!workspace || workspace_bytes < seg3d_row_partition_workspace_bytes(n_masks, m)) return SEG3D_EWORKSPACE;
+    const dim3 grid((unsigned)ceil_div64(m > 0 ? m : 1, kChunk), (unsigned)n_masks);
+    uint32_t* sums = static_cast<uint32_t*>(workspace);
+    hipStream_t st = as_stream(stream);
+    hipLaunchKernelGGL(partition_totals, grid, dim3(kThreads), 0, st, scale, m, skip_bits, sums);
+    SEG3D_CHECK_LAUNCH();
+    hipLaunchKernelGGL(partition_scatter, grid, dim3(kThreads), 0, st, scale, m, skip_bits, sums, order, inv, gather, n_keep);
+    SEG3D_CHECK_LAUNCH();
+    return SEG3D_OK;
 }
 
 int scan_exclusive_u32(const uint32_t* in, uint32_t* out, int64_t n, uint32_t* total, uint32_t* tmp,
diff --git a/openseg3d_amd/csrc/spconv_split.hip b/openseg3d_amd/csrc/spconv_split.hip
--- a/openseg3d_amd/csrc/spconv_split.hip
+++ b/openseg3d_amd/csrc/spconv_split.hip
@@ -113,14 +113,16 @@
     float eps;
 };
 
-template <int NBT, int RB, bool DENSE, int IO = 0, int DEPTH = 1>
+template <int NBT, int RB, bool DENSE, int IO = 0, int DEPTH = 1, bool CNT = false>
 __global__ __launch_bounds__(256, 2) void spconv_split_kernel(const void* __restrict__ x_v, const int32_t* __restrict__ nbr,
                                                               int64_t m_out, const uint4* __restrict__ wp,
                                                               const float* __restrict__ bias,
                                                               const void* __restrict__ addend_v,
                                                               const int32_t* __restrict__ row_order, int cin, int cout,
                                                               void* __restrict__ y_v, int relu_flags,
-                                                              const float* __restrict__ x_add, LnEpilogue ln) {
+                                                              const float* __restrict__ x_add, LnEpilogue ln,
+                                                              const int32_t* __restrict__ n_live) {
+    static_assert(!CNT || (DENSE && (IO == 0 || IO == 4) && DEPTH == 1), "the row count belongs to the Linear instantiations");
     const int relu = relu_flags & 1;
     const float* __restrict__ x = static_cast<const float*>(x_v);
     const float* __restrict__ addend = static_cast<const float*>(addend_v);
@@ -159,6 +161,12 @@
         if (tile_id >= n_tiles) return;
     }
     const int64_t row0 = tile_id * (kW * RB * 16) + wave * (RB * 16);
+    int64_t lim = m_out;
+    if constexpr (CNT) {
+        const int64_t nl = n_live[0];
+        lim = nl < 0 ? 0 : (nl < m_out ? nl : m_out);
+        if (!row_order && tile_id * (kW * RB * 16) >= lim) return;
+    }
     const int nb0 = col_group * NBT;
     const int cb_n = (cin + 31) >> 5, nb_n = cout >> 4;
     const int64_t last_row = m_out - 1;
@@ -169,7 +177,7 @@
         const bool ok = pos < m_out;
         const int64_t rc = ok ? (row_order ? (int64_t)row_order[pos] : pos) : last_row;
         if (DENSE) {
-            my_mask = 1u;
+            my_mask = CNT ? (row0 < lim ? 1u : 0u) : 1u;
         } else {
             int32_t v[27];
 #pragma unroll
@@ -200,7 +208,7 @@
 #pragma unroll
         for (int rb = 0; rb < RB; ++rb) {
             const int64_t pos = row0 + rb * 16 + c16;
-            grow_ok[rb] = pos < m_out;
+            grow_ok[rb] = pos < lim;
             grow[rb] = grow_ok[rb] ? pos : last_row;
         }
         auto fetch_idx = [&](int k, int32_t* idx) {
@@ -424,7 +432,7 @@
 #pragma unroll
         for (int r = 0; r < 4; ++r) {
             const int64_t opos = row0 + rb * 16 + g * 4 + r;
-            if (opos < m_out) {
+            if (opos < (CNT && !row_order ? lim : m_out)) {
                 const int64_t orow = row_order ? (int64_t)row_order[opos] : opos;
                 if constexpr (IO == 1 || IO == 2) {
                     __bf16* yb = static_cast<__bf16*>(y_v) + orow * cout + nb0 * 16 + c16;
@@ -475,7 +483,7 @@
 template <int NBT, int RB>
 int launch_split(const void* x, const int32_t* nbr, int64_t m_out, const void* wp, const float* bias, const void* addend,
                  const int32_t* row_order, int cin, int cout, void* y, int relu, int io, hipStream_t st,
-                 const float* x_add = nullptr, LnEpilogue ln = LnEpilogue{nullptr, nullptr, 0.f}) {
+                 const float* x_add = nullptr, LnEpilogue ln = LnEpilogue{nullptr, nullptr, 0.f}, const int32_t* n_live = nullptr) {
     dim3 grid((unsigned)ceil_div64(m_out, 4 * RB * 16), (unsigned)((cout / 16) / NBT));
     static const int xcd_run = [] {
         const char* e = getenv("SEG3D_CONV_XCD_RUN");
@@ -494,10 +502,21 @@
         grid.y = 1;
         relu |= 4;
     }
+    if (n_live) {
+        if (nbr != nullptr || (io != 0 && io != 4) || x_add || (relu & 3)) return SEG3D_EINVAL;
+        if (io == 4)
+            hipLaunchKernelGGL((spconv_split_kernel<NBT, RB, true, 4, 1, true>), grid, dim3(256), 0, st, x, nbr, m_out,
+                               reinterpret_cast<const uint4*>(wp), bias, addend, row_order, cin, cout, y, relu, nullptr, LnEpilogue{nullptr, nullptr, 0.f}, n_live);
+        else
+            hipLaunchKernelGGL((spconv_split_kernel<NBT, RB, true, 0, 1, true>), grid, dim3(256), 0, st, x, nbr, m_out,
+                               reinterpret_cast<const uint4*>(wp), bias, addend, row_order, cin, cout, y, relu, nullptr, LnEpilogue{nullptr, nullptr, 0.f}, n_live);
+        SEG3D_CHECK_LAUNCH();
+        return SEG3D_OK;
+    }
     if (io == 5) {
         if (nbr != nullptr || NBT * 16 != cout || !ln.gamma || !ln.beta) return SEG3D_EINVAL;
         hipLaunchKernelGGL((spconv_split_kernel<NBT, RB, true, 5>), grid, dim3(256), 0, st, x, nbr, m_out,
-                           reinterpret_cast<const uint4*>(wp), bias, addend, nullptr, cin, cout, y, 0, nullptr, ln);
+                           reinterpret_cast<const uint4*>(wp), bias, addend, nullptr, cin, cout, y, 0, nullptr, ln, nullptr);
         SEG3D_CHECK_LAUNCH();
         return SEG3D_OK;
     }
@@ -505,28 +524,28 @@
         if (nbr == nullptr) return SEG3D_EINVAL;
         if (io == 1)
             hipLaunchKernelGGL((spconv_split_kernel<NBT, RB, false, 1>), grid, dim3(256), 0, st, x, nbr, m_out,
-                               reinterpret_cast<const uint4*>(wp), bias, addend, row_order, cin, cout, y, relu, nullptr, LnEpilogue{nullptr, nullptr, 0.f});
+                               reinterpret_cast<const uint4*>(wp), bias, addend, row_order, cin, cout, y, relu, nullptr, LnEpilogue{nullptr, nullptr, 0.f}, nullptr);
         else
             hipLaunchKernelGGL((spconv_split_kernel<NBT, RB, false, 2>), grid, dim3(256), 0, st, x, nbr, m_out,
-                               reinterpret_cast<const uint4*>(wp), bias, addend, row_order, cin, cout, y, relu, nullptr, LnEpilogue{nullptr, nullptr, 0.f});
+                               reinterpret_cast<const uint4*>(wp), bias, addend, row_order, cin, cout, y, relu, nullptr, LnEpilogue{nullptr, nullptr, 0.f}, nullptr);
         SEG3D_CHECK_LAUNCH();
         return SEG3D_OK;
     }
     if (nbr == nullptr && io == 4)
         hipLaunchKernelGGL((spconv_split_kernel<NBT, RB, true, 4>), grid, dim3(256), 0, st, x, nbr, m_out,
-                           reinterpret_cast<const uint4*>(wp), bias, addend, nullptr, cin, cout, y, relu, nullptr, LnEpilogue{nullptr, nullptr, 0.f});
+                           reinterpret_cast<const uint4*>(wp), bias, addend, nullptr, cin, cout, y, relu, nullptr, LnEpilogue{nullptr, nullptr, 0.f}, nullptr);
     else if (nbr == nullptr && x_add)
         hipLaunchKernelGGL((spconv_split_kernel<NBT, RB, true, 3>), grid, dim3(256), 0, st, x, nbr, m_out,
-                           reinterpret_cast<const uint4*>(wp), bias, addend, nullptr, cin, cout, y, relu, x_add, LnEpilogue{nullptr, nullptr, 0.f});
+                           reinterpret_cast<const uint4*>(wp), bias, addend, nullptr, cin, cout, y, relu, x_add, LnEpilogue{nullptr, nullptr, 0.f}, nullptr);
     else if (nbr == nullptr)
         hipLaunchKernelGGL((spconv_split_kernel<NBT, RB, true>), grid, dim3(256), 0, st, x, nbr, m_out,
-                           reinterpret_cast<const uint4*>(wp), bias, addend, nullptr, cin, cout, y, relu, nullptr, LnEpilogue{nullptr, nullptr, 0.f});
+                           reinterpret_cast<const uint4*>(wp), bias, addend, nullptr, cin, cout, y, relu, nullptr, LnEpilogue{nullptr, nullptr, 0.f}, nullptr);
     else if (NBT <= kDeepMaxNbt && conv_depth2())
         hipLaunchKernelGGL((spconv_split_kernel<NBT, RB, false, 0, (NBT <= kDeepMaxNbt ? 2 : 1)>), grid, dim3(256), 0, st, x, nbr,
-                           m_out, reinterpret_cast<const uint4*>(wp), bias, addend, row_order, cin, cout, y, relu, nullptr, LnEpilogue{nullptr, nullptr, 0.f});
+                           m_out, reinterpret_cast<const uint4*>(wp), bias, addend, row_order, cin, cout, y, relu, nullptr, LnEpilogue{nullptr, nullptr, 0.f}, nullptr);
     else
         hipLaunchKernelGGL((spconv_split_kernel<NBT, RB, false>), grid, dim3(256), 0, st, x, nbr, m_out,
-                           reinterpret_cast<const uint4*>(wp), bias, addend, row_order, cin, cout, y, relu, nullptr, LnEpilogue{nullptr, nullptr, 0.f});
+                           reinterpret_cast<const uint4*>(wp), bias, addend, row_order, cin, cout, y, relu, nullptr, LnEpilogue{nullptr, nullptr, 0.f}, nullptr);
     SEG3D_CHECK_LAUNCH();
     return SEG3D_OK;
 }
@@ -563,10 +582,10 @@
 
 static int split_fwd_impl(const void* x, const int32_t* nbr, int64_t m_out, const void* wp, const float* bias,
                           const void* addend, const int32_t* row_order, int cin, int cout, void* y, int relu, int io,
-                          hipStream_t st, const float* x_add, LnEpilogue ln) {
+                          hipStream_t st, const float* x_add, LnEpilogue ln, const int32_t* n_live = nullptr) {
     if (x_add && (nbr || io != 0)) return SEG3D_EINVAL;
     if (io == 4 && (nbr || !addend)) return SEG3D_EINVAL;
-    if (!nbr && !row_order && !relu && !x_add && (io == 0 || io == 4) && g_forced_nbt.load(std::memory_order_relaxed) == 0) {
+    if (!nbr && !row_order && !relu && !x_add && !n_live && (io == 0 || io == 4) && g_forced_nbt.load(std::memory_order_relaxed) == 0) {
         const int rc = linear_stream_fwd(static_cast<const float*>(x), m_out, wp, bias, static_cast<const float*>(addend), cin,
                                          cout, static_cast<float*>(y), io, st);
         if (rc != 1) return rc;
@@ -585,13 +604,13 @@
         pick = nb;
     }
     switch (pick) {
-        case 12: return launch_split<12, 2>(x, nbr, m_out, wp, bias, addend, row_order, cin, cout, y, relu, io, st, x_add, ln);
-        case 8: return launch_split<8, 2>(x, nbr, m_out, wp, bias, addend, row_order, cin, cout, y, relu, io, st, x_add, ln);
-        case 6: return launch_split<6, 2>(x, nbr, m_out, wp, bias, addend, row_order, cin, cout, y, relu, io, st, x_add, ln);
-        case 4: return launch_split<4, 2>(x, nbr, m_out, wp, bias, addend, row_order, cin, cout, y, relu, io, st, x_add, ln);
-        case 3: return launch_split<3, 2>(x, nbr, m_out, wp, bias, addend, row_order, cin, cout, y, relu, io, st, x_add, ln);
-        case 2: return launch_split<2, 2>(x, nbr, m_out, wp, bias, addend, row_order, cin, cout, y, relu, io, st, x_add, ln);
-        default: return launch_split<1, 2>(x, nbr, m_out, wp, bias, addend, row_order, cin, cout, y, relu, io, st, x_add, ln);
+        case 12: return launch_split<12, 2>(x, nbr, m_out, wp, bias, addend, row_order, cin, cout, y, relu, io, st, x_add, ln, n_live);
+        case 8: return launch_split<8, 2>(x, nbr, m_out, wp, bias, addend, row_order, cin, cout, y, relu, io, st, x_add, ln, n_live);
+        case 6: return launch_split<6, 2>(x, nbr, m_out, wp, bias, addend, row_order, cin, cout, y, relu, io, st, x_add, ln, n_live);
+        case 4: return launch_split<4, 2>(x, nbr, m_out, wp, bias, addend, row_order, cin, cout, y, relu, io, st, x_add, ln, n_live);
+        case 3: return launch_split<3, 2>(x, nbr, m_out, wp, bias, addend, row_order, cin, cout, y, relu, io, st, x_add, ln, n_live);
+        case 2: return launch_split<2, 2>(x, nbr, m_out, wp, bias, addend, row_order, cin, cout, y, relu, io, st, x_add, ln, n_live);
+        default: return launch_split<1, 2>(x, nbr, m_out, wp, bias, addend, row_order, cin, cout, y, relu, io, st, x_add, ln, n_live);
     }
 }
 
@@ -599,7 +618,7 @@
                         const void* addend, const int32_t* row_order, int cin, int cout, void* y, int relu, int io,
                         hipStream_t st, const float* x_add) {
     return split_fwd_impl(x, nbr, m_out, wp, bias, addend, row_order, cin, cout, y, relu, io, st, x_add,
-                          LnEpilogue{nullptr, nullptr, 0.f});
+                          LnEpilogue{nullptr, nullptr, 0.f}, nullptr);
 }
 
 int spconv_split_fwd(const float* x, const int32_t* nbr, int64_t m_out, const void* wp, const float* bias,
@@ -658,6 +677,18 @@
     return spconv_split_fwd_io(x, nullptr, m, w_packed, nullptr, factor, nullptr, cin, cout, y, 0, 4, as_stream(stream), nullptr);
 }
 
+int seg3d_linear_fwd_rows(const float* x, int64_t m, const int32_t* n_live, const int32_t* row_out, const void* w_packed,
+                          const float* bias, const float* addend, int32_t mul, int32_t cin, int32_t cout, float* y,
+                          void* stream) {
+    if (m < 0 || cin <= 0 || cout <= 0 || (cin & 7) || (cout & 15) || !w_packed || !n_live) return SEG3D_EINVAL;
+    if (mul && (!addend || bias)) return SEG3D_EINVAL;
+    if (row_out && (!addend || bias || mul)) return SEG3D_EINVAL;
+    if (m == 0) return SEG3D_OK;
+    if (!x || !y) return SEG3D_EINVAL;
+    return split_fwd_impl(x, nullptr, m, w_packed, bias, addend, row_out, cin, cout, y, 0, mul ? 4 : 0, as_stream(stream), nullptr,
+                          LnEpilogue{nullptr, nullptr, 0.f}, n_live);
+}
+
 int seg3d_linear_fwd_sum(const float* x, const float* x_add, int64_t m, const void* w_packed, const float* bias, int32_t cin,
                          int32_t cout, float* y, void* stream) {
     if (m < 0 || cin <= 0 || cout <= 0 || (cin & 7) || (cout & 15) || !w_packed) return SEG3D_EINVAL;
diff --git a/openseg3d_amd/csrc/voxelize.hip b/openseg3d_amd/csrc/voxelize.hip
--- a/openseg3d_amd/csrc/voxelize.hip
+++ b/openseg3d_amd/csrc/voxelize.hip
@@ -273,7 +273,7 @@
     return cart2polar_impl<double>(points, n_points, row_stride, xyz_col, out, stream);
 }
 
-int seg3d_abi_version(void) { return 49; }
+int seg3d_abi_version(void) { return 50; }
 
 namespace {
 thread_local char g_last_error[320] = "";
diff --git a/openseg3d_amd/csrc/wgrad_dense.hip b/openseg3d_amd/csrc/wgrad_dense.hip
--- a/openseg3d_amd/csrc/wgrad_dense.hip
+++ b/openseg3d_amd/csrc/wgrad_dense.hip
@@ -91,11 +91,12 @@
     return acc;
 }
 
-template <bool XB, bool GROUP, int DEPTH = 1>
+template <bool XB, bool GROUP, int DEPTH = 1, bool CNT = false>
 __global__ __launch_bounds__(kThreads, (DEPTH > 1 ? 1 : 2)) void wgrad_dense_kernel(const void* __restrict__ x_v, const float* __restrict__ dy,
                                                                int64_t m_rows, int cin, int cout, int rows_per_chunk,
                                                                int nbi, int tiles, float* __restrict__ part,
-                                                               int want_bias, int group) {
+                                                               int want_bias, int group, const int32_t* __restrict__ n_live) {
+    static_assert(!CNT || (!XB && !GROUP && DEPTH == 1), "the row count belongs to the fp32 split-K form");
     const float* x = static_cast<const float*>(x_v);
     __shared__ __attribute__((aligned(16))) float red[GROUP ? 4 : 64 * 64];
     __shared__ float red_b[GROUP ? 1 : kWaves][64];
@@ -113,7 +114,11 @@
     const int ci0 = bi * 64, co0 = bo * 64;
     const int64_t r_begin = (int64_t)chunk * rows_per_chunk;
     if (r_begin >= m_rows) return;
-    const int64_t r_end = r_begin + rows_per_chunk < m_rows ? r_begin + rows_per_chunk : m_rows;
+    int64_t r_end = r_begin + rows_per_chunk < m_rows ? r_begin + rows_per_chunk : m_rows;
+    if constexpr (CNT) {
+        const int64_t nl = n_live[0];
+        if (nl < r_end) r_end = nl > r_begin ? nl : r_begin;
+    }
     const bool a_ok = co0 + 4 * cq < cout, b_ok = ci0 + 4 * cq < cin;
     const uint32_t yoff = (uint32_t)((8 * rg * cout + (a_ok ? co0 + 4 * cq : 0)) * 4);
     const uint32_t xoff = (uint32_t)((8 * rg * cin + (b_ok ? ci0 + 4 * cq : 0)) * (XB ? 2 : 4));
@@ -389,10 +394,10 @@
         const unsigned blocks = (unsigned)((p.chunks + 7) / 8 * 8) * (unsigned)groups;
         if (x_bf16)
             hipLaunchKernelGGL((wgrad_dense_kernel<true, true>), dim3(blocks), dim3(kThreads), 0, st, x, dy, m, cin, cout, (int)p.rows,
-                               nbi_g, groups, part, want_bias, p.group);
+                               nbi_g, groups, part, want_bias, p.group, nullptr);
         else
             hipLaunchKernelGGL((wgrad_dense_kernel<false, true>), dim3(blocks), dim3(kThreads), 0, st, x, dy, m, cin, cout, (int)p.rows,
-                               nbi_g, groups, part, want_bias, p.group);
+                               nbi_g, groups, part, want_bias, p.group, nullptr);
         return;
     }
     const int tiles = p.nbo * p.nbi;
@@ -403,15 +408,15 @@
     }();
     if (!x_bf16 && depth == 3) {
         hipLaunchKernelGGL((wgrad_dense_kernel<false, false, 3>), dim3(blocks), dim3(kThreads), 0, st, x, dy, m, cin, cout, (int)p.rows,
-                           p.nbi, tiles, part, want_bias, 0);
+                           p.nbi, tiles, part, want_bias, 0, nullptr);
         return;
     }
     if (x_bf16)
         hipLaunchKernelGGL((wgrad_dense_kernel<true, false>), dim3(blocks), dim3(kThreads), 0, st, x, dy, m, cin, cout, (int)p.rows,
-                           p.nbi, tiles, part, want_bias, 0);
+                           p.nbi, tiles, part, want_bias, 0, nullptr);
     else
         hipLaunchKernelGGL((wgrad_dense_kernel<false, false>), dim3(blocks), dim3(kThreads), 0, st, x, dy, m, cin, cout, (int)p.rows,
-                           p.nbi, tiles, part, want_bias, 0);
+                           p.nbi, tiles, part, want_bias, 0, nullptr);
 }
 
 static int linear_wgrad_partials(const void* x, bool x_bf16, const float* dy, int64_t m, int32_t cin, int32_t cout,
@@ -434,6 +439,25 @@
     return linear_wgrad_partials(x, false, dy, m, cin, cout, with_bias, workspace, workspace_bytes, chunks, stream);
 }
 
+extern "C" int seg3d_linear_wgrad_partials_rows(const float* x, const float* dy, int64_t m, const int32_t* n_live, int32_t cin,
+                                                int32_t cout, int32_t with_bias, void* workspace, size_t workspace_bytes,
+                                                int32_t* chunks, void* stream) {
+    if (m < 0 || cin <= 0 || cout <= 0 || (cin & 3) || (cout & 3) || !chunks || !n_live) return SEG3D_EINVAL;
+    if (m > 0 && (!x || !dy)) return SEG3D_EINVAL;
+    if (workspace_bytes < seg3d_linear_wgrad_workspace_bytes(m, cin, cout) || (m > 0 && !workspace)) return SEG3D_EINVAL;
+    *chunks = 0;
+    if (m == 0) return SEG3D_OK;
+    const Plan p = plan(m, cin, cout);
+    if (p.group) return SEG3D_EINVAL;
+    const int tiles = p.nbo * p.nbi;
+    const unsigned blocks = (unsigned)((p.chunks + 7) / 8 * 8) * (unsigned)tiles;
+    hipLaunchKernelGGL((wgrad_dense_kernel<false, false, 1, true>), dim3(blocks), dim3(kThreads), 0, as_stream(stream), x, dy, m, cin,
+                       cout, (int)p.rows, p.nbi, tiles, static_cast<float*>(workspace), with_bias ? 1 : 0, 0, n_live);
+    SEG3D_CHECK_LAUNCH();
+    *chunks = p.chunks;
+    return SEG3D_OK;
+}
+
 extern "C" int seg3d_linear_wgrad_partials_xbf16(const uint16_t* x_bf16, const float* dy, int64_t m, int32_t cin, int32_t cout,
                                                  int32_t with_bias, void* workspace, size_t workspace_bytes, int32_t* chunks,
                                                  void* stream) {
diff --git a/openseg3d_amd/ops.py b/openseg3d_amd/ops.py
--- a/openseg3d_amd/ops.py
+++ b/openseg3d_amd/ops.py
@@ -1517,11 +1517,16 @@
     return dw, db
 
 
-def _linear_wgrad_into(fk, x, dy, cin, cout, dw_ptr, db_ptr, *keep):
+def _linear_wgrad_into(fk, x, dy, cin, cout, dw_ptr, db_ptr, *keep, n_live=None):
     m = x.shape[0]
     ws_bytes = _lib.query("seg3d_linear_wgrad_workspace_bytes", m, cin, cout)
     ws = _workspace(ws_bytes, dy.device)
     chunks = ctypes.c_int32(0)
+    if n_live is not None:
+        _lib.call("seg3d_linear_wgrad_partials_rows", _ptr(x), _ptr(dy), m, _ptr(n_live), cin, cout, 1 if db_ptr else 0,
+                  _ptr(ws), ws_bytes, ctypes.byref(chunks), fk.fork(ws, x, dy, n_live, *keep))
+        fk.add_reduce(ws, chunks.value, cin * cout + cout, cin * cout, dw_ptr, db_ptr, *keep)
+        return
     _lib.call("seg3d_linear_wgrad_partials_xbf16" if x.dtype == torch.bfloat16 else "seg3d_linear_wgrad_partials",
               _ptr(x), _ptr(dy), m, cin, cout, 1 if db_ptr else 0, _ptr(ws), ws_bytes,
               ctypes.byref(chunks), fk.fork(ws, x, dy, *keep))
@@ -1540,12 +1545,49 @@
 
 GELU_SAVED_GRAD = os.environ.get("SEG3D_GELU_SAVED_GRAD", "1") != "0"
 
+DROPPATH_SKIP = os.environ.get("SEG3D_DROPPATH_SKIP", "0") == "1"
+
+
+class RowPartition:
+    __slots__ = ("order", "inv", "gather", "n_keep")
+
+    def row(self, r):
+        return self.order[r], self.inv[r], self.gather[r], self.n_keep[r:r + 1]
+
+
+def droppath_partition(scales, skip=()):
+    _need_gpu(scales)
+    scales = _f32c(scales)
+    r, m = scales.shape
+    if r > 64:
+        raise _lib.Seg3dError("droppath_partition: at most 64 masks per call")
+    part = RowPartition()
+    i32 = dict(dtype=torch.int32, device=scales.device)
+    part.order, part.inv, part.gather = (torch.empty((r, m), **i32) for _ in range(3))
+    part.n_keep = torch.empty((r,), **i32)
+    bits = 0
+    for k in skip:
+        bits |= 1 << int(k)
+    ws_bytes = _lib.query("seg3d_row_partition_workspace_bytes", r, m)
+    ws = _workspace(ws_bytes, scales.device)
+    _lib.call("seg3d_row_partition", _ptr(scales), r, m, ctypes.c_uint64(bits), _ptr(part.order), _ptr(part.inv),
+              _ptr(part.gather), _ptr(part.n_keep), _ptr(ws), ws.numel(), _stream())
+    return part
+
+
+def _linear_rows(x, n_live, packed, bias, cin, cout, addend=None, mul=False, row_out=None):
+    y = torch.empty((x.shape[0], cout), dtype=torch.float32, device=x.device)
+    _lib.call("seg3d_linear_fwd_rows", _ptr(x), x.shape[0], _ptr(n_live), _ptr(row_out), _ptr(packed), _ptr(bias), _ptr(addend),
+              int(bool(mul)), cin, cout, _ptr(y), _stream())
+    return y
+
 
 class _EncoderLayerFn(torch.autograd.Function):
 
     @staticmethod
     def forward(ctx, x, pos, w_in, b_in, tau, w_out, b_out, g1, be1, w1, b1, w2, b2, g2, be2, meta):
-        heads, tau_min, wi, eps1, eps2, s1, s2, drop_p, drop_seed = meta
+        heads, tau_min, wi, eps1, eps2, s1, s2, drop_p, drop_seed = meta[:9]
+        part2 = meta[9] if len(meta) > 9 else None
         x = _f32c(x)
         c = x.shape[1]
         live = any(ctx.needs_input_grad)
@@ -1556,12 +1598,16 @@
         fuse_ln = (LINEAR_LN_FUSED and not live and s1 is None and s2 is None and (c // 16) in (1, 2, 3, 4, 6, 8, 12)
                    and b_out is not None and b2 is not None)
         c_n1 = _Ctx(True, True, True, True, False, False)
+        hid = w1.shape[0]
+        if (DROPPATH_SKIP and live and s2 is not None and GELU_SAVED_GRAD and TRAIN_STORAGE != "bf16"
+                and b_out is not None and b1 is not None and b2 is not None):
+            return _EncoderLayerFn._forward_skip(ctx, c_in, c_at, c_n1, o, x, w_out, b_out, g1, be1, w1, b1, w2, b2, g2, be2,
+                                                 eps1, eps2, s1, s2, part2)
         if fuse_ln:
             x1 = _linear_layernorm(o, _linear_pack(w_out, 0), b_out, x, g1, be1, eps1, c, c)
         else:
             a = _linear_apply(o, _linear_pack(w_out, 0), b_out, c, c)
             x1 = _LayerNormResidualFn.forward(c_n1, a, x, g1, be1, eps1, s1)
-        hid = w1.shape[0]
         h = _linear_apply(x1, _linear_pack(w1, 0), b1, c, hid)
         if live and GELU_SAVED_GRAD:
             g, gp = torch.empty_like(h), torch.empty_like(h)
@@ -1576,29 +1622,95 @@
             m = _linear_apply(g, _linear_pack(w2, 0), b2, hid, c)
             x2 = _LayerNormResidualFn.forward(c_n2, m, x1, g2, be2, eps2, s2)
         ctx.parts = (c_in, c_at, c_n1, c_n2)
+        ctx.skip = None
         ctx.save_for_backward(_saved_rows(o), _saved_rows(x1), h, _saved_rows(g), w_out, w1, w2)
         ctx.bias_params = (b_out, b1, b2)
         ctx.norm_params = (g1, be1, g2, be2)
         return x2
 
     @staticmethod
+    def _forward_skip(ctx, c_in, c_at, c_n1, o, x, w_out, b_out, g1, be1, w1, b1, w2, b2, g2, be2, eps1, eps2, s1, s2, part2):
+        m, c = x.shape
+        hid = w1.shape[0]
+        dev = x.device
+        s2 = _f32c(s2.reshape(-1))
+        if part2 is None:
+            part2 = droppath_partition(s2.reshape(1, -1)).row(0)
+        order2, inv2, _, n2 = part2
+        f32 = dict(dtype=torch.float32, device=dev)
+        a = _linear_apply(o, _linear_pack(w_out, 0), b_out, c, c)
+        x1, x1_c = torch.empty((m, c), **f32), torch.empty((m, c), **f32)
+        mean1, rstd1 = torch.empty((m,), **f32), torch.empty((m,), **f32)
+        rs1 = None if s1 is None else _f32c(s1.reshape(-1))
+        _lib.call("seg3d_layernorm_fwd_rows", _ptr(a), _ptr(x), _ptr(g1), _ptr(be1), _ptr(rs1), None, _ptr(inv2), _ptr(x1_c),
+                  float(eps1), m, c, _ptr(x1), _ptr(mean1), _ptr(rstd1), _stream())
+        c_n1.save_for_backward(a, mean1, rstd1, g1, rs1)
+        c_n1.has_res = True
+        h_c = _linear_rows(x1_c, n2, _linear_pack(w1, 0), b1, c, hid)
+        g_c, gp_c = torch.empty_like(h_c), torch.empty_like(h_c)
+        _lib.call("seg3d_gelu_fwd_rows", _ptr(h_c), m, hid, _ptr(n2), _ptr(g_c), _ptr(gp_c), _stream())
+        m_c = _linear_rows(g_c, n2, _linear_pack(w2, 0), b2, hid, c)
+        x2 = torch.empty((m, c), **f32)
+        mean2, rstd2 = torch.empty((m,), **f32), torch.empty((m,), **f32)
+        _lib.call("seg3d_layernorm_fwd_rows", _ptr(m_c), _ptr(x1), _ptr(g2), _ptr(be2), _ptr(s2), _ptr(inv2), None, None,
+                  float(eps2), m, c, _ptr(x2), _ptr(mean2), _ptr(rstd2), _stream())
+        ctx.parts = (c_in, c_at, c_n1, None)
+        ctx.skip = (order2, n2, s2)
+        ctx.save_for_backward(o, x1_c, gp_c, g_c, w_out, w1, w2, m_c, mean2, rstd2)
+        ctx.bias_params = (b_out, b1, b2)
+        ctx.norm_params = (g1, be1, g2, be2)
+        return x2
+
+    @staticmethod
+    def _backward_mlp_skip(ctx, fk, dx2):
+        _, x1_c, gp_c, g_c, _, w1, w2, m_c, mean2, rstd2 = ctx.saved_tensors
+        order2, n2, s2 = ctx.skip
+        g2 = ctx.norm_params[2]
+        m, c = m_c.shape
+        hid = w1.shape[0]
+        dev = dx2.device
+        dm_c = torch.empty((m, c), dtype=torch.float32, device=dev)
+        dg2 = torch.empty((c,), dtype=torch.float32, device=dev)
+        dbe2 = torch.empty((c,), dtype=torch.float32, device=dev)
+        ws_bytes = _lib.query("seg3d_layernorm_bwd_workspace_bytes", m, c)
+        ws = torch.empty((ws_bytes,), dtype=torch.uint8, device=dev)
+        nb = ctypes.c_int32(0)
+        _lib.call("seg3d_layernorm_bwd_partials_rows", _ptr(dx2), _ptr(m_c), _ptr(mean2), _ptr(rstd2), _ptr(g2), _ptr(s2),
+                  _ptr(order2), _ptr(n2), m, c, _ptr(dm_c), _ptr(ws), ws_bytes, ctypes.byref(nb), _stream())
+        fk.add_reduce(ws, nb.value, 2 * c, c, dg2.data_ptr(), dbe2.data_ptr())
+        dw2 = torch.empty((c, hid), dtype=torch.float32, device=dev)
+        db2 = torch.empty((c,), dtype=torch.float32, device=dev)
+        _linear_wgrad_into(fk, g_c, dm_c, hid, c, dw2.data_ptr(), db2.data_ptr(), n_live=n2)
+        dh_c = _linear_rows(dm_c, n2, _linear_pack(w2, 1), None, c, hid, addend=gp_c, mul=True)
+        dw1 = torch.empty((hid, c), dtype=torch.float32, device=dev)
+        db1 = torch.empty((hid,), dtype=torch.float32, device=dev)
+        _linear_wgrad_into(fk, x1_c, dh_c, c, hid, dw1.data_ptr(), db1.data_ptr(), n_live=n2)
+        d_x1 = _linear_rows(dh_c, n2, _linear_pack(w1, 1), None, hid, c, addend=dx2, row_out=order2)
+        fk.hold(order2, n2, s2)
+        return d_x1, dw1, db1, dw2, db2, dg2, dbe2
+
+    @staticmethod
     def backward(ctx, dx2):
         c_in, c_at, c_n1, c_n2 = ctx.parts
-        o, x1, h, g, w_out, w1, w2 = ctx.saved_tensors
+        o, x1, h, g, w_out, w1, w2 = ctx.saved_tensors[:7]
         dx2 = _f32c(dx2)
         c, hid = x1.shape[1], w1.shape[0]
         fk = _WgradFork(dx2.device)
-        c_n1.fork = c_n2.fork = fk
-        dm, _, dg2, dbe2, _, _ = _LayerNormResidualFn.backward(c_n2, dx2)
-        dw2, db2 = _linear_wgrad(g, dm, hid, c, fork=fk)
-        if GELU_SAVED_GRAD:
-            dh = torch.empty((dm.shape[0], hid), dtype=torch.float32, device=dm.device)
-            _lib.call("seg3d_linear_fwd_mul", _ptr(dm), dm.shape[0], _ptr(_linear_pack(w2, 1)), _ptr(h), c, hid, _ptr(dh),
-                      _stream())
+        c_n1.fork = fk
+        if ctx.skip is not None:
+            d_x1, dw1, db1, dw2, db2, dg2, dbe2 = _EncoderLayerFn._backward_mlp_skip(ctx, fk, dx2)
         else:
-            dh = torch.ops.aten.gelu_backward(_linear_apply(dm, _linear_pack(w2, 1), None, c, hid), h)
-        dw1, db1 = _linear_wgrad(x1, dh, c, hid, fork=fk)
-        d_x1 = _linear_apply(dh, _linear_pack(w1, 1), None, hid, c, addend=dx2)
+            c_n2.fork = fk
+            dm, _, dg2, dbe2, _, _ = _LayerNormResidualFn.backward(c_n2, dx2)
+            dw2, db2 = _linear_wgrad(g, dm, hid, c, fork=fk)
+            if GELU_SAVED_GRAD:
+                dh = torch.empty((dm.shape[0], hid), dtype=torch.float32, device=dm.device)
+                _lib.call("seg3d_linear_fwd_mul", _ptr(dm), dm.shape[0], _ptr(_linear_pack(w2, 1)), _ptr(h), c, hid, _ptr(dh),
+                          _stream())
+            else:
+                dh = torch.ops.aten.gelu_backward(_linear_apply(dm, _linear_pack(w2, 1), None, c, hid), h)
+            dw1, db1 = _linear_wgrad(x1, dh, c, hid, fork=fk)
+            d_x1 = _linear_apply(dh, _linear_pack(w1, 1), None, hid, c, addend=dx2)
         da, _, dg1, dbe1, _, _ = _LayerNormResidualFn.backward(c_n1, d_x1)
         dw_out, db_out = _linear_wgrad(o, da, c, c, fork=fk)
         do = _linear_apply(da, _linear_pack(w_out, 1), None, c, c)
@@ -1609,7 +1721,9 @@
         g1, be1, g2, be2 = ctx.norm_params
         fk.join((w_out, dw_out), (w1, dw1), (w2, dw2), (b_out, db_out), (b1, db1), (b2, db2), (g1, dg1), (be1, dbe1),
                 (g2, dg2), (be2, dbe2))
-        c_n1.fork = c_n2.fork = None
+        c_n1.fork = None
+        if c_n2 is not None:
+            c_n2.fork = None
         ctx.parts = None
         return dx, None, dw_in, db_in, dtau, dw_out, db_out, dg1, dbe1, dw1, db1, dw2, db2, dg2, dbe2, None
 
diff --git a/openseg3d_amd/swformer.py b/openseg3d_amd/swformer.py
--- a/openseg3d_amd/swformer.py
+++ b/openseg3d_amd/swformer.py
@@ -176,7 +176,7 @@
         self.mlp = MLP(d_model, mlp_hidden_dim, drop=drop)
         self.drop_path_rate = float(drop_path_rate)
 
-    def forward(self, x, pos, wi, scales=None, seed=None):
+    def forward(self, x, pos, wi, scales=None, seed=None, part2=None):
         at, mlp = self.win_attn.self_attn, self.mlp
         if seed is None:
             seed = attention_dropout_seed() if self.training and at.dropout > 0.0 else 0
@@ -187,7 +187,7 @@
                                                         drop_path_scale(x, self.drop_path_rate))
         if (FUSED_LAYER and torch.is_grad_enabled() and x.requires_grad and not mlp.drop and at.in_proj_bias is not None
                 and ops.encoder_layer_fits(x, at.embed_dim, mlp.fc1.out_features, at.num_heads)):
-            meta = (at.num_heads, at.tau_min, wi, self.norm1.eps, self.norm2.eps, s1, s2) + at.drop_args(seed)
+            meta = (at.num_heads, at.tau_min, wi, self.norm1.eps, self.norm2.eps, s1, s2) + at.drop_args(seed) + (part2,)
             return ops._EncoderLayerFn.apply(x, pos, at.in_proj_weight, at.in_proj_bias, at.tau, at.out_proj.weight,
                                              at.out_proj.bias, self.norm1.weight, self.norm1.bias, mlp.fc1.weight,
                                              mlp.fc1.bias, mlp.fc2.weight, mlp.fc2.bias, self.norm2.weight,
@@ -214,9 +214,15 @@
         half = int(self.depth / 2)
         scales = self.drop_path_scales(x) if self.training else None
         seed = attention_dropout_seed() if self.training else 0
+        parts = None
+        if scales is not None and ops.DROPPATH_SKIP and FUSED_LAYER and x.is_cuda and torch.is_grad_enabled():
+            live = [2 * i + 1 for i, layer in enumerate(self.layers) if layer.drop_path_rate > 0.0]
+            parts = ops.droppath_partition(scales, skip=[r for r in range(2 * self.depth) if r not in live])
         for i, layer in enumerate(self.layers):
             s = 0 if i < half else 1
-            x = layer(x, plan.pos[s], plan.index[s], None if scales is None else (scales[2 * i], scales[2 * i + 1]), seed + i)
+            drop = scales is not None and layer.drop_path_rate > 0.0
+            x = layer(x, plan.pos[s], plan.index[s], None if scales is None else (scales[2 * i], scales[2 * i + 1]), seed + i,
+                      parts.row(2 * i + 1) if parts is not None and drop else None)
         return x
 
     def drop_path_scales(self, x):
```

After: 4.167 million points/s, median of 3. Within noise of the previous version (+0.0%).
